# shuwang127/SRCNN_Cpp

Measured on AMD Instinct MI355X. Metric: SRCNN Y-channel Mpixels/sec, higher is better.
Workload: dtype f32; 1 GPU; 1 x 3840x2160 luma plane per GPU per step (1920x1080 x2.0, BASELINE configs[1]), fused conv path, mfma arithmetic, inputs resident in HBM; frames_per_gpu=1, width=3840, height=2160, mode=mfma, seam_deferral=True, output_checksum=584152

## Files before the change

### include/srcnn_amd.h

```cpp
#ifndef SRCNN_AMD_H
#define SRCNN_AMD_H

#include <stddef.h>
#include <stdint.h>

#ifdef __cplusplus
extern "C" {
#endif

#define SRCNN_CONV1_FILTERS 64
#define SRCNN_CONV2_FILTERS 32

enum {
    SRCNN_OK = 0,
    SRCNN_ERR_INVALID = -1,
    SRCNN_ERR_HIP = -2,
    SRCNN_ERR_NOMEM = -3,
    SRCNN_ERR_NODEVICE = -4,
    SRCNN_ERR_STATE = -5
};

enum { SRCNN_MODE_MFMA = 0, SRCNN_MODE_EXACT = 1, SRCNN_MODE_SPLIT16 = 2, SRCNN_MODE_REFBYTES = 3, SRCNN_MODE_REFBYTES16 = 4,
       SRCNN_MODE_BANDED16 = 5 };

// ... 142 lines not shown
enum { SRCNN_METRIC_SSE = 1, SRCNN_METRIC_SSIM = 2 };
int srcnn_metrics_image_dev(srcnn_ctx *ctx, const srcnn_image *a, const srcnn_image *b, int width, int height, int channels,
                            int n_frames, int border, const float *luma , double data_range, int flags,
                            double *d_out );
double srcnn_metric_psnr(double sse, double n_px, double data_range);

int srcnn_forward_y(srcnn_ctx *ctx, const uint8_t *src, size_t src_stride,
                    uint8_t *dst, size_t dst_stride, int width, int height,
                    float *preclamp, size_t preclamp_stride);

int srcnn_forward_y_frames(srcnn_ctx *ctx, const uint8_t *const *src, size_t src_stride,
                           uint8_t *const *dst, size_t dst_stride, int width, int height, int n_frames);


int srcnn_stripe_rows(int height, int n_parts, int index, int *row_begin, int *row_end);

int srcnn_forward_y_frames_multi(srcnn_ctx *const *ctxs, int n_ctx,
                                 const uint8_t *const *src, size_t src_stride,
                                 uint8_t *const *dst, size_t dst_stride,
                                 int width, int height, int n_frames);

int srcnn_forward_y_lanes_dev(srcnn_ctx *const *ctxs, int n_ctx,
                              const uint8_t *const *d_src, size_t src_stride,
                              uint8_t *const *d_dst, size_t dst_stride,
                              int width, int height, int n_planes);

int srcnn_forward_y_striped(srcnn_ctx *const *ctxs, int n_ctx,
                            const uint8_t *src, size_t src_stride,
                            uint8_t *dst, size_t dst_stride, int width, int height);

int srcnn_forward_y_striped_frames(srcnn_ctx *const *ctxs, int n_ctx,
                                   const uint8_t *const *src, size_t src_stride,
                                   uint8_t *const *dst, size_t dst_stride,
                                   int width, int height, int n_planes);

int srcnn_forward_y_striped_dev(srcnn_ctx *const *ctxs, int n_ctx,
                                const uint8_t *const *d_stripes, size_t stripe_stride,
                                uint8_t *const *d_out, size_t out_stride, int width, int height);

int srcnn_halo_transport(const srcnn_ctx *ctx);


int srcnn_forward_y_dev(srcnn_ctx *ctx,
                        const uint8_t *d_src, size_t src_stride, size_t src_frame_pitch,
                        uint8_t *d_dst, size_t dst_stride, size_t dst_frame_pitch,
                        int width, int height, int n_frames,
                        float *d_preclamp );

int srcnn_forward_y_rows_dev(srcnn_ctx *ctx,
                             const uint8_t *d_src, size_t src_stride, int src_row0,
                             uint8_t *d_dst, size_t dst_stride, int dst_row0,
                             int width, int height, int row_begin, int row_end);

int srcnn_forward_y_rows_halo_dev(srcnn_ctx *ctx,
                                  const uint8_t *d_src, size_t src_stride, int src_row0, int src_rows,
                                  const uint8_t *d_halo_top, const uint8_t *d_halo_bot, size_t halo_stride,
                                  uint8_t *d_dst, size_t dst_stride, int dst_row0,
                                  int width, int height, int row_begin, int row_end);


int srcnn_model_halo_rows(const srcnn_ctx *ctx);

int srcnn_model_rows_dev(srcnn_ctx *ctx,
                         const uint8_t *d_src, size_t src_stride, int src_row0,
                         uint8_t *d_dst, size_t dst_stride, int dst_row0,
                         int width, int height, int row_begin, int row_end,
                         float *d_preclamp );

int srcnn_model_rows_halo_dev(srcnn_ctx *ctx,
                              const uint8_t *d_src, size_t src_stride, int src_row0, int src_rows,
                              const uint8_t *d_halo_top, const uint8_t *d_halo_bot, size_t halo_stride,
                              uint8_t *d_dst, size_t dst_stride, int dst_row0,
                              int width, int height, int row_begin, int row_end,
                              float *d_preclamp );

int srcnn_model_striped_dev(srcnn_ctx *const *ctxs, int n_ctx,
                            const uint8_t *const *d_stripes, size_t stripe_stride,
                            uint8_t *const *d_out, size_t out_stride, int width, int height);

int srcnn_model_striped(srcnn_ctx *const *ctxs, int n_ctx,
                        const uint8_t *src, size_t src_stride,
                        uint8_t *dst, size_t dst_stride, int width, int height);

int srcnn_model_color_rows_dev(srcnn_ctx *ctx,
                               const uint8_t *d_src, size_t src_stride, int src_row0,
                               uint8_t *d_dst, size_t dst_stride, int dst_row0,
                               int width, int height, int row_begin, int row_end,
                               float *d_preclamp );
int srcnn_model_color_rows_halo_dev(srcnn_ctx *ctx,
                                    const uint8_t *d_src, size_t src_stride, int src_row0, int src_rows,
                                    const uint8_t *d_halo_top, const uint8_t *d_halo_bot, size_t halo_stride,
                                    uint8_t *d_dst, size_t dst_stride, int dst_row0,
                                    int width, int height, int row_begin, int row_end,
                                    float *d_preclamp );
int srcnn_model_color_striped_dev(srcnn_ctx *const *ctxs, int n_ctx,
                                  const uint8_t *const *d_stripes, size_t stripe_stride,
                                  uint8_t *const *d_out, size_t out_stride, int width, int height);
int srcnn_model_color_striped(srcnn_ctx *const *ctxs, int n_ctx,
                              const uint8_t *src, size_t src_stride,
                              uint8_t *dst, size_t dst_stride, int width, int height);

int srcnn_model_rows_f32_dev(srcnn_ctx *ctx,
                             const float *d_src, size_t src_stride, size_t src_ch_pitch, int src_row0,
                             float *d_dst, size_t dst_stride, size_t dst_ch_pitch, int dst_row0,
                             int width, int height, int row_begin, int row_end);
int srcnn_model_rows_halo_f32_dev(srcnn_ctx *ctx,
                                  const float *d_src, size_t src_stride, size_t src_ch_pitch, int src_row0, int src_rows,
                                  const float *d_halo_top, const float *d_halo_bot, size_t halo_stride, size_t halo_ch_pitch,
                                  float *d_dst, size_t dst_stride, size_t dst_ch_pitch, int dst_row0,
                                  int width, int height, int row_begin, int row_end);
int srcnn_model_striped_f32_dev(srcnn_ctx *const *ctxs, int n_ctx,
                                const float *const *d_stripes, size_t stripe_stride, size_t stripe_ch_pitch,
                                float *const *d_out, size_t out_stride, size_t out_ch_pitch, int width, int height);
int srcnn_model_striped_f32(srcnn_ctx *const *ctxs, int n_ctx,
                            const float *src, size_t src_stride, size_t src_ch_pitch,
                            float *dst, size_t dst_stride, size_t dst_ch_pitch, int width, int height);

int srcnn_forward_y_unfused_dev(srcnn_ctx *ctx,
                                const uint8_t *d_src, size_t src_stride, size_t src_frame_pitch,
                                uint8_t *d_dst, size_t dst_stride, size_t dst_frame_pitch,
                                int width, int height, int n_frames, float *d_work);

int srcnn_conv99x11_dev(srcnn_ctx *ctx, const uint8_t *d_src, size_t src_stride,
                        float *d_planes, size_t plane_stride, size_t plane_pitch,
                        int width, int height);
int srcnn_conv55_dev(srcnn_ctx *ctx, const float *d_planes, size_t plane_stride, size_t plane_pitch,
                     uint8_t *d_dst, size_t dst_stride, int width, int height,
                     float *d_preclamp );


int srcnn_scaled_size(int width, int height, float scale, int *out_w, int *out_h);

int srcnn_bgr2ycrcb(srcnn_ctx *ctx, const uint8_t *bgr, size_t stride, int width, int height,
                    uint8_t *y, uint8_t *cr, uint8_t *cb, size_t plane_stride);
int srcnn_ycrcb2bgr(srcnn_ctx *ctx, const uint8_t *y, const uint8_t *cr, const uint8_t *cb,
                    size_t plane_stride, int width, int height, uint8_t *bgr, size_t stride);
int srcnn_resize_cubic(srcnn_ctx *ctx, const uint8_t *src, size_t src_stride, int src_w, int src_h,
                       uint8_t *dst, size_t dst_stride, int dst_w, int dst_h);

int srcnn_process_bgr(srcnn_ctx *ctx, const uint8_t *bgr, size_t stride, int width, int height,
                      float scale, uint8_t *out, size_t out_stride);
int srcnn_process_bgr_dev(srcnn_ctx *ctx, const uint8_t *d_bgr, size_t stride, int width, int height,
                          float scale, uint8_t *d_out, size_t out_stride);


int srcnn_fixup_stats(srcnn_ctx *ctx, unsigned long long out[4], float *delta, float *max_dev);
int srcnn_set_fixup_strict(srcnn_ctx *ctx, int on);
int srcnn_set_fixup_margin(srcnn_ctx *ctx, float factor);
int srcnn_set_fixup_local(srcnn_ctx *ctx, float k_local);
int srcnn_fixup_local_stats(srcnn_ctx *ctx, float *k, float *max_ratio);

int srcnn_query_plan(srcnn_ctx *ctx, int width, int height, int n_frames, int out[6]);

#ifdef __cplusplus
}
#endif
#endif
```

### srcnn_cpp_amd/__init__.py

```python
from __future__ import annotations

import ctypes as C
from pathlib import Path
from typing import Optional, Sequence

import numpy as np

__all__ = [
    "Context", "SrcnnError", "forward_y_striped_frames", "load_library", "library_path", "tuning_library_path", "use_library", "load_weights", "split_weights",
    "load_model", "split_model", "model_from_state_dict", "model_from_module", "MODEL_SIZES", "COLOR_MODEL_SIZES", "PAD_REPLICATE",
    "PAD_ZERO",
    "Convolution99", "Convolution11", "Convolution55", "Convolution99x11", "default_context",
    "MODE_MFMA", "MODE_EXACT", "MODE_SPLIT16", "MODE_REFBYTES", "MODE_REFBYTES16", "MODE_BANDED16", "FLOP_PER_PIXEL",
    "ERR_INVALID", "ERR_HIP", "ERR_NOMEM", "ERR_NODEVICE", "ERR_STATE",
    "stripe_rows", "forward_y_frames_multi", "forward_y_lanes_dev", "forward_y_striped", "forward_y_striped_dev",
    "model_striped", "model_striped_dev",
    "model_color_striped", "model_color_striped_dev", "model_striped_f32", "model_striped_f32_dev",
    "cubic_f32_taps", "cubic_aa_f32_taps", "luma_gain", "luma_for_order", "luma_bt601_studio", "LUMA_BT601",
    "ELEM_F32", "ELEM_F16", "ELEM_BF16", "ELEM_U8", "ELEM_SIZE", "Image", "image_check",
]

_PKG = Path(__file__).resolve().parent
_LIB_PATH = _PKG / "libsrcnn_amd.so"
_WEIGHTS_PATH = _PKG / "data" / "srcnn915_weights.f32"

MODE_MFMA = 0
MODE_EXACT = 1
MODE_SPLIT16 = 2
MODE_REFBYTES = 3
MODE_REFBYTES16 = 4
MODE_BANDED16 = 5
N_WEIGHTS = 8129
MODEL_SIZES = {8129: 1, 24513: 3, 57281: 5}
COLOR_MODEL_SIZES = {20099: 1, 36483: 3, 69251: 5}
PAD_REPLICATE = 0
PAD_ZERO = 1
_PADDINGS = {"replicate": PAD_REPLICATE, "zero": PAD_ZERO}
FLOP_PER_PIXEL = 16064
LUMA_BT601 = (0.299, 0.587, 0.114, 0.0)

ELEM_F32, ELEM_F16, ELEM_BF16, ELEM_U8 = 0, 1, 2, 3
ELEM_SIZE = {ELEM_F32: 4, ELEM_F16: 2, ELEM_BF16: 2, ELEM_U8: 1}
METRIC_SSE, METRIC_SSIM = 1, 2
METRIC_FIELDS = ("sse", "n_px", "ssim_sum", "n_win")

ERR_INVALID, ERR_HIP, ERR_NOMEM, ERR_NODEVICE, ERR_STATE = -1, -2, -3, -4, -5
_ERR = {-1: "invalid argument", -2: "HIP runtime error", -3: "out of memory",
        -4: "no gfx950 device", -5: "bad state"}

_u8p = C.POINTER(C.c_uint8)
_f32p = C.POINTER(C.c_float)
_f32pp = C.POINTER(_f32p)
_lib = None


class _CImage(C.Structure):
    _fields_ = [("data", C.c_void_p), ("elem", C.c_int), ("scale", C.c_float), ("px_step", C.c_size_t), ("stride", C.c_size_t),
                ("ch_pitch", C.c_size_t), ("frame_pitch", C.c_size_t)]


class SrcnnError(RuntimeError):
    def __init__(self, code: int, msg: str = ""):
        self.code = code
        super().__init__(f"srcnn error {code} ({_ERR.get(code, '?')}): {msg}")


def library_path() -> Path:
    return _LIB_PATH


def tuning_library_path() -> Path:
    return _PKG / "libsrcnn_amd_tuning.so"


def use_library(path) -> None:
    global _LIB_PATH
    if _lib is not None:
        raise RuntimeError("the library is already loaded")
    _LIB_PATH = Path(path)


def load_library() -> C.CDLL:
    global _lib
    if _lib is not None:
        return _lib
    if not _LIB_PATH.exists():
        raise SrcnnError(-4, f"{_LIB_PATH} not built: run `python -m srcnn_cpp_amd.build` "
                             "(there is no CPU fallback)")
    import importlib.util
    import sys
    if "torch" not in sys.modules and importlib.util.find_spec("torch") is not None:
        import torch
    lib = C.CDLL(str(_LIB_PATH))
    sz, i, vp, imp = C.c_size_t, C.c_int, C.c_void_p, C.POINTER(_CImage)
    sigs = {
        "srcnn_abi_version": ([], i),
        "srcnn_create": ([C.POINTER(vp), i], i),
        "srcnn_destroy": ([vp], None),
        "srcnn_last_error": ([vp], C.c_char_p),
        "srcnn_set_mode": ([vp, i], i),
        "srcnn_get_mode": ([vp], i),
        "srcnn_set_stream": ([vp, vp], i),
        "srcnn_synchronize": ([vp], i),
        "srcnn_kernel_variant": ([vp], i),
        "srcnn_conv99": ([vp, _u8p, sz, _f32p, sz, i, i, _f32p, C.c_float], i),
        "srcnn_conv11": ([vp, _f32pp, sz, _f32p, sz, i, i, _f32p, C.c_float], i),
        "srcnn_conv55": ([vp, _f32pp, sz, _u8p, sz, i, i, _f32p, C.c_float], i),
        "srcnn_conv99x11": ([vp, _u8p, sz, _f32pp, sz, i, i, _f32p, _f32p, _f32p, _f32p], i),
        "srcnn_set_weights": ([vp, _f32p, _f32p, _f32p, _f32p, _f32p, C.c_float], i),
        "srcnn_set_model": ([vp, i, _f32p, _f32p, _f32p, _f32p, _f32p, C.c_float], i),
        "srcnn_get_model_f2": ([vp], i),
        "srcnn_set_padding": ([vp, i], i),
        "srcnn_get_padding": ([vp], i),
        "srcnn_set_model_color": ([vp, i, _f32p, _f32p, _f32p, _f32p, _f32p, _f32p], i),
        "srcnn_get_model_channels": ([vp], i),
        "srcnn_forward_color": ([vp, _u8p, sz, _u8p, sz, i, i, _f32p, sz], i),
        "srcnn_forward_color_dev": ([vp, vp, sz, sz, vp, sz, sz, i, i, i, vp], i),
        "srcnn_forward_f32": ([vp, _f32p, sz, sz, _f32p, sz, sz, i, i], i),
        "srcnn_forward_f32_dev": ([vp, vp, sz, sz, sz, vp, sz, sz, sz, i, i, i], i),
        "srcnn_cubic_f32_taps": ([i, i, C.POINTER(i), _f32p], i),
        "srcnn_resize_cubic_f32": ([vp, _f32p, sz, sz, i, i, _f32p, sz, sz, i, i, i], i),
        "srcnn_resize_cubic_f32_dev": ([vp, vp, sz, sz, sz, i, i, vp, sz, sz, sz, i, i, i, i], i),
        "srcnn_cubic_aa_f32_taps": ([i, i, C.POINTER(i), C.POINTER(i), _f32p, i], i),
        "srcnn_resize_cubic_aa_f32": ([vp, _f32p, sz, sz, i, i, _f32p, sz, sz, i, i, i], i),
        "srcnn_resize_cubic_aa_f32_dev": ([vp, vp, sz, sz, sz, i, i, vp, sz, sz, sz, i, i, i, i], i),
        "srcnn_resize_cubic_aa_image_dev": ([vp, imp, i, i, imp, i, i, i, i], i),
        "srcnn_metrics_image_dev": ([vp, imp, imp, i, i, i, i, i, _f32p, C.c_double, i, vp], i),
        "srcnn_metric_psnr": ([C.c_double, C.c_double, C.c_double], C.c_double),
        "srcnn_process_f32": ([vp, _f32p, sz, sz, i, i, _f32p, sz, sz, i, i], i),
        "srcnn_process_f32_dev": ([vp, vp, sz, sz, sz, i, i, vp, sz, sz, sz, i, i, i], i),
        "srcnn_luma_gain": ([_f32p, _f32p], i),
        "srcnn_process_rgb_f32": ([vp, _f32p, sz, sz, i, i, _f32p, sz, sz, i, i, _f32p, _f32p], i),
        "srcnn_process_rgb_f32_dev": ([vp, vp, sz, sz, sz, i, i, vp, sz, sz, sz, i, i, _f32p, _f32p, i], i),
        "srcnn_image_check": ([imp, i, i, i, i, i], i),
        "srcnn_forward_image_dev": ([vp, imp, imp, i, i, i], i),
        "srcnn_resize_cubic_image_dev": ([vp, imp, i, i, imp, i, i, i, i], i),
        "srcnn_process_image_dev": ([vp, imp, i, i, imp, i, i, i], i),
        "srcnn_process_rgb_image_dev": ([vp, imp, i, i, imp, i, i, _f32p, _f32p, i], i),
        "srcnn_set_input_range": ([vp, C.c_float], i),
        "srcnn_get_input_range": ([vp], C.c_float),
        "srcnn_forward_y": ([vp, _u8p, sz, _u8p, sz, i, i, _f32p, sz], i),
        "srcnn_forward_y_frames": ([vp, C.POINTER(_u8p), sz, C.POINTER(_u8p), sz, i, i, i], i),
        "srcnn_forward_y_dev": ([vp, vp, sz, sz, vp, sz, sz, i, i, i, vp], i),
        "srcnn_forward_y_rows_dev": ([vp, vp, sz, i, vp, sz, i, i, i, i, i], i),
        "srcnn_forward_y_rows_halo_dev": ([vp, vp, sz, i, i, vp, vp, sz, vp, sz, i, i, i, i, i], i),
        "srcnn_halo_transport": ([vp], i),
        "srcnn_forward_y_unfused_dev": ([vp, vp, sz, sz, vp, sz, sz, i, i, i, vp], i),
        "srcnn_conv99x11_dev": ([vp, vp, sz, vp, sz, sz, i, i], i),
        "srcnn_conv55_dev": ([vp, vp, sz, sz, vp, sz, i, i, vp], i),
        "srcnn_conv99x11_to_dev": ([vp, _u8p, sz, vp, sz, sz, i, i, _f32p, _f32p, _f32p, _f32p], i),
        "srcnn_conv55_from_dev": ([vp, vp, sz, sz, _u8p, sz, i, i, _f32p, C.c_float], i),
        "srcnn_dev_alloc": ([vp, sz, C.POINTER(vp)], i),
        "srcnn_dev_free": ([vp, vp], i),
        "srcnn_dev_download": ([vp, vp, vp, sz], i),
        "srcnn_dev_upload": ([vp, vp, vp, sz], i),
        "srcnn_ipc_export": ([vp, vp, C.POINTER(C.c_ubyte * 64)], i),
        "srcnn_ipc_open": ([vp, C.POINTER(C.c_ubyte * 64), C.POINTER(vp)], i),
        "srcnn_ipc_close": ([vp, vp], i),
        "srcnn_query_plan": ([vp, i, i, i, C.POINTER(i * 6)], i),
        "srcnn_fixup_stats": ([vp, C.POINTER(C.c_ulonglong * 4), C.POINTER(C.c_float), C.POINTER(C.c_float)], i),
        "srcnn_set_fixup_strict": ([vp, i], i),
        "srcnn_set_seam_deferral": ([vp, i], i),
        "srcnn_flush": ([vp], i),
        "srcnn_set_fixup_margin": ([vp, C.c_float], i),
        "srcnn_set_kernel_variant": ([vp, i], i),
        "srcnn_set_fixup_local": ([vp, C.c_float], i),
        "srcnn_fixup_local_stats": ([vp, C.POINTER(C.c_float), C.POINTER(C.c_float)], i),
        "srcnn_scaled_size": ([i, i, C.c_float, C.POINTER(i), C.POINTER(i)], i),
        "srcnn_bgr2ycrcb": ([vp, _u8p, sz, i, i, _u8p, _u8p, _u8p, sz], i),
        "srcnn_ycrcb2bgr": ([vp, _u8p, _u8p, _u8p, sz, i, i, _u8p, sz], i),
        "srcnn_resize_cubic": ([vp, _u8p, sz, i, i, _u8p, sz, i, i], i),
        "srcnn_process_bgr": ([vp, _u8p, sz, i, i, C.c_float, _u8p, sz], i),
        "srcnn_process_bgr_dev": ([vp, vp, sz, i, i, C.c_float, vp, sz], i),
        "srcnn_stripe_rows": ([i, i, i, C.POINTER(i), C.POINTER(i)], i),
        "srcnn_forward_y_frames_multi": ([C.POINTER(vp), i, C.POINTER(_u8p), sz, C.POINTER(_u8p), sz, i, i, i], i),
        "srcnn_forward_y_lanes_dev": ([C.POINTER(vp), i, C.POINTER(vp), sz, C.POINTER(vp), sz, i, i, i], i),
        "srcnn_forward_y_striped": ([C.POINTER(vp), i, _u8p, sz, _u8p, sz, i, i], i),
        "srcnn_forward_y_striped_frames": ([C.POINTER(vp), i, C.POINTER(_u8p), sz, C.POINTER(_u8p), sz, i, i, i], i),
        "srcnn_forward_y_striped_dev": ([C.POINTER(vp), i, C.POINTER(vp), sz, C.POINTER(vp), sz, i, i], i),
        "srcnn_model_halo_rows": ([vp], i),
        "srcnn_model_rows_dev": ([vp, vp, sz, i, vp, sz, i, i, i, i, i, vp], i),
        "srcnn_model_rows_halo_dev": ([vp, vp, sz, i, i, vp, vp, sz, vp, sz, i, i, i, i, i, vp], i),
        "srcnn_model_striped": ([C.POINTER(vp), i, _u8p, sz, _u8p, sz, i, i], i),
        "srcnn_model_striped_dev": ([C.POINTER(vp), i, C.POINTER(vp), sz, C.POINTER(vp), sz, i, i], i),
        "srcnn_model_color_rows_dev": ([vp, vp, sz, i, vp, sz, i, i, i, i, i, vp], i),
        "srcnn_model_color_rows_halo_dev": ([vp, vp, sz, i, i, vp, vp, sz, vp, sz, i, i, i, i, i, vp], i),
        "srcnn_model_color_striped": ([C.POINTER(vp), i, _u8p, sz, _u8p, sz, i, i], i),
        "srcnn_model_color_striped_dev": ([C.POINTER(vp), i, C.POINTER(vp), sz, C.POINTER(vp), sz, i, i], i),
        "srcnn_model_rows_f32_dev": ([vp, vp, sz, sz, i, vp, sz, sz, i, i, i, i, i], i),
        "srcnn_model_rows_halo_f32_dev": ([vp, vp, sz, sz, i, i, vp, vp, sz, sz, vp, sz, sz, i, i, i, i, i], i),
        "srcnn_model_striped_f32": ([C.POINTER(vp), i, _f32p, sz, sz, _f32p, sz, sz, i, i], i),
        "srcnn_model_striped_f32_dev": ([C.POINTER(vp), i, C.POINTER(vp), sz, sz, C.POINTER(vp), sz, sz, i, i], i),
    }
    for name, (args, res) in sigs.items():
        fn = getattr(lib, name)
        fn.argtypes = args
        fn.restype = res
    _lib = lib
    return lib


ABI_SYMBOLS = (
    "srcnn_abi_version", "srcnn_create", "srcnn_destroy", "srcnn_last_error", "srcnn_set_mode",
    "srcnn_get_mode", "srcnn_set_stream", "srcnn_synchronize", "srcnn_kernel_variant", "srcnn_set_kernel_variant", "srcnn_conv99", "srcnn_conv11",
    "srcnn_conv55", "srcnn_conv99x11", "srcnn_set_weights", "srcnn_forward_y", "srcnn_forward_y_frames",
    "srcnn_forward_y_dev",
    "srcnn_forward_y_rows_dev", "srcnn_forward_y_rows_halo_dev", "srcnn_halo_transport", "srcnn_forward_y_unfused_dev", "srcnn_conv99x11_dev",
    "srcnn_conv55_dev", "srcnn_conv99x11_to_dev", "srcnn_conv55_from_dev", "srcnn_dev_alloc", "srcnn_dev_free",
    "srcnn_dev_download", "srcnn_dev_upload", "srcnn_ipc_export", "srcnn_ipc_open", "srcnn_ipc_close", "srcnn_query_plan", "srcnn_fixup_stats", "srcnn_set_fixup_strict", "srcnn_set_fixup_margin", "srcnn_set_fixup_local", "srcnn_fixup_local_stats", "srcnn_set_seam_deferral", "srcnn_flush", "srcnn_scaled_size", "srcnn_bgr2ycrcb", "srcnn_ycrcb2bgr",
    "srcnn_resize_cubic", "srcnn_process_bgr", "srcnn_process_bgr_dev",
    "srcnn_stripe_rows", "srcnn_forward_y_frames_multi", "srcnn_forward_y_lanes_dev", "srcnn_forward_y_striped", "srcnn_forward_y_striped_frames", "srcnn_forward_y_striped_dev",
    "srcnn_set_model", "srcnn_get_model_f2", "srcnn_set_padding", "srcnn_get_padding",
    "srcnn_set_model_color", "srcnn_get_model_channels", "srcnn_forward_color", "srcnn_forward_color_dev",
    "srcnn_forward_f32", "srcnn_forward_f32_dev", "srcnn_set_input_range", "srcnn_get_input_range",
    "srcnn_cubic_f32_taps", "srcnn_resize_cubic_f32", "srcnn_resize_cubic_f32_dev", "srcnn_process_f32", "srcnn_process_f32_dev",
    "srcnn_luma_gain", "srcnn_process_rgb_f32", "srcnn_process_rgb_f32_dev",
    "srcnn_image_check", "srcnn_forward_image_dev", "srcnn_resize_cubic_image_dev", "srcnn_process_image_dev",
    "srcnn_process_rgb_image_dev",
    "srcnn_cubic_aa_f32_taps", "srcnn_resize_cubic_aa_f32", "srcnn_resize_cubic_aa_f32_dev", "srcnn_resize_cubic_aa_image_dev",
    "srcnn_metrics_image_dev", "srcnn_metric_psnr",
    "srcnn_model_halo_rows", "srcnn_model_rows_dev", "srcnn_model_rows_halo_dev", "srcnn_model_striped", "srcnn_model_striped_dev",
    "srcnn_model_color_rows_dev", "srcnn_model_color_rows_halo_dev", "srcnn_model_color_striped", "srcnn_model_color_striped_dev",
    "srcnn_model_rows_f32_dev", "srcnn_model_rows_halo_f32_dev", "srcnn_model_striped_f32", "srcnn_model_striped_f32_dev",
)


def load_weights(path: Optional[Path] = None) -> np.ndarray:
    blob = np.fromfile(str(path or _WEIGHTS_PATH), dtype="<f4")
    if blob.size != N_WEIGHTS:
        raise ValueError(f"weight blob has {blob.size} floats, expected {N_WEIGHTS}")
    return blob


def split_weights(blob: np.ndarray):
    blob = np.ascontiguousarray(blob, dtype=np.float32)
    return (blob[64:5248].reshape(64, 9, 9), blob[0:64], blob[5280:7328].reshape(32, 64),
            blob[5248:5280], blob[7329:8129].reshape(32, 5, 5), float(blob[7328]))


def split_model(blob: np.ndarray):
    blob = np.ascontiguousarray(blob, dtype=np.float32).ravel()
    if blob.size in COLOR_MODEL_SIZES:
        f2 = COLOR_MODEL_SIZES[blob.size]
        o2 = 64 + 15552
        o3 = o2 + 32 + 2048 * f2 * f2
        return (blob[64:o2].reshape(64, 3, 9, 9), blob[0:64], blob[o2 + 32:o3].reshape(32, 64, f2, f2),
                blob[o2:o2 + 32], blob[o3 + 3:o3 + 2403].reshape(3, 32, 5, 5), blob[o3:o3 + 3].copy())
    f2 = MODEL_SIZES.get(blob.size)
    if f2 is None:
        raise ValueError(f"model blob has {blob.size} floats, expected one of {sorted(MODEL_SIZES)} "
                         f"(colour: {sorted(COLOR_MODEL_SIZES)})")
    if f2 == 1:
        return split_weights(blob)
    n2 = 2048 * f2 * f2
    o3 = 5280 + n2
    return (blob[64:5248].reshape(64, 9, 9), blob[0:64], blob[5280:o3].reshape(32, 64, f2, f2),
            blob[5248:5280], blob[o3 + 1:o3 + 801].reshape(32, 5, 5), float(blob[o3]))


def load_model(path) -> np.ndarray:
    blob = np.fromfile(str(path), dtype="<f4")
    if blob.size not in MODEL_SIZES and blob.size not in COLOR_MODEL_SIZES:
        raise ValueError(f"model blob has {blob.size} floats, expected one of {sorted(MODEL_SIZES)} "
                         f"(colour: {sorted(COLOR_MODEL_SIZES)})")
    return blob


def model_from_state_dict(sd, input_scale: float = 255.0, image_order: Optional[str] = None):
    def arr(key, shape=None):
        if key not in sd:
            raise KeyError(f"state dict has no {key!r}")
        v = sd[key]
        v = v.detach().cpu().numpy() if hasattr(v, "detach") else np.asarray(v)
        v = np.asarray(v, dtype=np.float64)
        if shape is not None and v.shape != shape:
            raise ValueError(f"{key}: shape {v.shape}, expected {shape}")
        return v
    w2 = arr("conv2.weight")
    if w2.ndim != 4 or w2.shape[:2] != (32, 64) or w2.shape[2] != w2.shape[3] or w2.shape[2] not in (1, 3, 5):
        raise ValueError(f"conv2.weight: shape {w2.shape}, expected (32, 64, f2, f2) with f2 in 1, 3, 5")
    s = float(input_scale)
    f32 = lambda a: np.ascontiguousarray(a, dtype=np.float32)
    c_in, c_out = arr("conv1.weight").shape[1:2], arr("conv3.weight").shape[:1]
    if c_in == (3,) or c_out == (3,):
        if c_in != c_out:
            raise ValueError(f"conv1 reads {c_in[0] if c_in else '?'} channels and conv3 writes {c_out[0] if c_out else '?'}: "
                             "a model has 1 channel in and out, or 3")
        if image_order not in ("rgb", "bgr"):
            raise ValueError(f"image_order={image_order!r}: a 3-channel model needs image_order='rgb' or 'bgr' (the channel "
                             "order of the images it will run on)")
        w1, w3, b3 = arr("conv1.weight", (64, 3, 9, 9)), arr("conv3.weight", (3, 32, 5, 5)), arr("conv3.bias", (3,))
        if image_order == "bgr":
            w1, w3, b3 = w1[:, ::-1], w3[::-1], b3[::-1]
        return (f32(w1), f32(arr("conv1.bias", (64,)) * s), f32(w2.reshape(32, 64, w2.shape[2], w2.shape[2])),
                f32(arr("conv2.bias", (32,)) * s), f32(w3), f32(b3 * s))
    return (f32(arr("conv1.weight", (64, 1, 9, 9)).reshape(64, 9, 9)), f32(arr("conv1.bias", (64,)) * s),
            f32(w2 if w2.shape[2] > 1 else w2.reshape(32, 64)), f32(arr("conv2.bias", (32,)) * s),
            f32(arr("conv3.weight", (1, 32, 5, 5)).reshape(32, 5, 5)), float(arr("conv3.bias", (1,))[0] * s))


def model_from_module(module, input_scale: float = 255.0, image_order: Optional[str] = None):
    modes = set()
    for name in ("conv1", "conv2", "conv3"):
        conv = getattr(module, name, None)
        if conv is None:
            raise ValueError(f"module has no {name}")
        k = tuple(conv.kernel_size)
        pad = conv.padding
        if isinstance(pad, str):
            if pad == "valid":
                raise ValueError(f"{name}: padding='valid' (unpadded layers are not supported)")
            pad = tuple(kk // 2 for kk in k)
        pad = tuple(pad) if isinstance(pad, (tuple, list)) else (pad, pad)
        if pad != tuple(kk // 2 for kk in k):
            raise ValueError(f"{name}: padding {pad} for kernel {k}, expected {tuple(kk // 2 for kk in k)}"
                             + (" (unpadded layers are not supported)" if pad == (0, 0) else ""))
        mode = conv.padding_mode
        if mode == "zeros":
            modes.add("zero")
        elif mode == "replicate":
            modes.add("replicate")
        else:
            raise ValueError(f"{name}: padding_mode={mode!r} (only 'zeros' and 'replicate' are supported)")
    if len(modes) != 1:
        raise ValueError(f"the layers mix padding modes {sorted(modes)}: one mode for all three layers is supported")
    return model_from_state_dict(module.state_dict(), input_scale, image_order), modes.pop()


def _plane(a, dtype, name, writable=False):
    if not isinstance(a, np.ndarray) or a.ndim != 2 or a.dtype != dtype:
        raise TypeError(f"{name}: expected a 2-D numpy array of {np.dtype(dtype).name}")
    if a.strides[1] != a.itemsize or a.strides[0] % a.itemsize or a.strides[0] < a.shape[1] * a.itemsize:
        raise ValueError(f"{name}: rows must be contiguous (row stride may be padded)")
    if writable and not a.flags.writeable:
        raise ValueError(f"{name}: output plane is read-only")
    return a, a.strides[0] // a.itemsize


def _f32_planes(a, name, writable=False):
    if not isinstance(a, np.ndarray) or a.dtype != np.float32 or a.ndim not in (2, 3, 4):
        raise TypeError(f"{name}: expected a float32 numpy array of shape (H, W), (C, H, W) or (N, C, H, W)")
    if 0 in a.shape:
        raise ValueError(f"{name}: empty array of shape {tuple(a.shape)}")
    a4 = a[(None,) * (4 - a.ndim)]
    w = a4.shape[3]
    if a4.strides[3] != 4 or (a4.shape[2] > 1 and (a4.strides[2] % 4 or a4.strides[2] < 4 * w)):
        raise ValueError(f"{name}: rows must be contiguous (row, channel and frame strides may be padded)")
    if any(a4.shape[d] > 1 and (a4.strides[d] % 4 or a4.strides[d] <= 0) for d in (0, 1)):
        raise ValueError(f"{name}: channel and frame strides must be positive multiples of 4 bytes")
    if writable and not a.flags.writeable:
        raise ValueError(f"{name}: output array is read-only")
    return a4


def _f32_image(a, name, dst_w, dst_h):
    if not isinstance(a, np.ndarray) or a.dtype != np.float32 or a.ndim not in (2, 3):
        raise TypeError(f"{name}: expected a float32 numpy array of shape (H, W) or (C, H, W)")
    a3 = _f32_planes(a, name)[0]
    for what, v in (("dst_w", dst_w), ("dst_h", dst_h)):
        if isinstance(v, bool) or not isinstance(v, (int, np.integer)) or v <= 0:
            raise ValueError(f"{what}: expected a positive integer, got {v!r}")
    return a3, int(dst_w), int(dst_h)
# ... 139 lines not shown
        self._check(self._lib.srcnn_forward_color(self._h, img.ctypes.data_as(_u8p), ss, dst.ctypes.data_as(_u8p), ds, w, h,
                                                  pp, ps))
        return dst

    def forward_color_dev(self, d_src, src_stride, src_frame_pitch, d_dst, dst_stride, dst_frame_pitch,
                          width, height, n_frames=1, d_preclamp=0):
        self._check(self._lib.srcnn_forward_color_dev(self._h, d_src, src_stride, src_frame_pitch, d_dst, dst_stride,
                                                      dst_frame_pitch, width, height, n_frames, d_preclamp or None))

    def forward_f32(self, x, out=None):
        x4 = _f32_planes(x, "x")
        if out is None:
            out = np.empty(x.shape, np.float32)
        o4 = _f32_planes(out, "out", True)
        _same_shape("out", out.shape, x.shape)
        n, c, h, w = x4.shape
        if c not in (1, 3):
            raise ValueError(f"x: shape {tuple(x.shape)}: a model has 1 channel or 3")
        channels = self.model_channels()
        if c != channels:
            raise ValueError(f"x: shape {tuple(x.shape)} for a model of {channels} channel(s): expected (N, {channels}, H, W), "
                             f"({channels}, H, W)" + (" or (H, W)" if channels == 1 else ""))
        stride = lambda a4: a4.strides[2] // 4 if h > 1 else w
        for k in range(n):
            self._check(self._lib.srcnn_forward_f32(self._h, _fp(x4[k]), stride(x4), x4.strides[1] // 4 if c > 1 else 0, _fp(o4[k]),
                                                    stride(o4), o4.strides[1] // 4 if c > 1 else 0, w, h))
        return out

    def forward_f32_dev(self, d_src, src_stride, src_ch_pitch, src_frame_pitch, d_dst, dst_stride, dst_ch_pitch,
                        dst_frame_pitch, width, height, n_frames=1):
        self._check(self._lib.srcnn_forward_f32_dev(self._h, d_src, src_stride, src_ch_pitch, src_frame_pitch, d_dst, dst_stride,
                                                    dst_ch_pitch, dst_frame_pitch, width, height, n_frames))

    def resize_cubic_f32(self, x, dst_w, dst_h):
        x3, dst_w, dst_h = _f32_image(x, "x", dst_w, dst_h)
        c, h, w = x3.shape
        out = np.empty((c, dst_h, dst_w), np.float32)
        self._check(self._lib.srcnn_resize_cubic_f32(self._h, _fp(x3), x3.strides[1] // 4 if h > 1 else w,
                                                     x3.strides[0] // 4 if c > 1 else 0, w, h, _fp(out), dst_w, dst_w * dst_h,
                                                     dst_w, dst_h, c))
        return out if x.ndim == 3 else out[0]

    def resize_cubic_f32_dev(self, d_src, src_stride, src_ch_pitch, src_frame_pitch, src_w, src_h, d_dst, dst_stride,
                             dst_ch_pitch, dst_frame_pitch, dst_w, dst_h, channels=1, n_frames=1):
        self._check(self._lib.srcnn_resize_cubic_f32_dev(self._h, d_src, src_stride, src_ch_pitch, src_frame_pitch, src_w, src_h,
                                                         d_dst, dst_stride, dst_ch_pitch, dst_frame_pitch, dst_w, dst_h, channels,
                                                         n_frames))

    def resize_cubic_aa_f32(self, x, dst_w, dst_h):
        x3, dst_w, dst_h = _f32_image(x, "x", dst_w, dst_h)
        c, h, w = x3.shape
        out = np.empty((c, dst_h, dst_w), np.float32)
        self._check(self._lib.srcnn_resize_cubic_aa_f32(self._h, _fp(x3), x3.strides[1] // 4 if h > 1 else w,
                                                        x3.strides[0] // 4 if c > 1 else 0, w, h, _fp(out), dst_w, dst_w * dst_h,
                                                        dst_w, dst_h, c))
        return out if x.ndim == 3 else out[0]

    def resize_cubic_aa_f32_dev(self, d_src, src_stride, src_ch_pitch, src_frame_pitch, src_w, src_h, d_dst, dst_stride,
                                dst_ch_pitch, dst_frame_pitch, dst_w, dst_h, channels=1, n_frames=1):
        self._check(self._lib.srcnn_resize_cubic_aa_f32_dev(self._h, d_src, src_stride, src_ch_pitch, src_frame_pitch, src_w, src_h,
                                                            d_dst, dst_stride, dst_ch_pitch, dst_frame_pitch, dst_w, dst_h, channels,
                                                            n_frames))

    def process_f32(self, x, dst_w, dst_h):
        x3, dst_w, dst_h = _f32_image(x, "x", dst_w, dst_h)
        c, h, w = x3.shape
        channels = self.model_channels()
        if c != channels:
            raise ValueError(f"x: shape {tuple(x.shape)} for a model of {channels} channel(s): expected ({channels}, H, W)"
                             + (" or (H, W)" if channels == 1 else ""))
        out = np.empty((c, dst_h, dst_w), np.float32)
        self._check(self._lib.srcnn_process_f32(self._h, _fp(x3), x3.strides[1] // 4 if h > 1 else w,
                                                x3.strides[0] // 4 if c > 1 else 0, w, h, _fp(out), dst_w, dst_w * dst_h, dst_w,
                                                dst_h))
        return out if x.ndim == 3 else out[0]

    def process_f32_dev(self, d_src, src_stride, src_ch_pitch, src_frame_pitch, src_w, src_h, d_dst, dst_stride, dst_ch_pitch,
                        dst_frame_pitch, dst_w, dst_h, n_frames=1):
        self._check(self._lib.srcnn_process_f32_dev(self._h, d_src, src_stride, src_ch_pitch, src_frame_pitch, src_w, src_h, d_dst,
                                                    dst_stride, dst_ch_pitch, dst_frame_pitch, dst_w, dst_h, n_frames))

    def process_rgb_f32(self, x, dst_w, dst_h, luma=LUMA_BT601, clamp=None):
        x3, dst_w, dst_h = _f32_image(x, "x", dst_w, dst_h)
        if x.ndim != 3 or x3.shape[0] != 3:
            raise ValueError(f"x: shape {tuple(x.shape)}: expected (3, H, W)")
        _, h, w = x3.shape
        _not_shrinking(w, h, dst_w, dst_h)
        luma4, clamp2 = _luma4(luma), _clamp2(clamp)
        out = np.empty((3, dst_h, dst_w), np.float32)
        self._check(self._lib.srcnn_process_rgb_f32(self._h, _fp(x3), x3.strides[1] // 4 if h > 1 else w, x3.strides[0] // 4, w, h,
                                                    _fp(out), dst_w, dst_w * dst_h, dst_w, dst_h, luma4, clamp2))
        return out

    def process_rgb_f32_dev(self, d_src, src_stride, src_ch_pitch, src_frame_pitch, src_w, src_h, d_dst, dst_stride, dst_ch_pitch,
                            dst_frame_pitch, dst_w, dst_h, luma=LUMA_BT601, clamp=None, n_frames=1):
        _not_shrinking(src_w, src_h, dst_w, dst_h)
        luma4, clamp2 = _luma4(luma), _clamp2(clamp)
        self._check(self._lib.srcnn_process_rgb_f32_dev(self._h, d_src, src_stride, src_ch_pitch, src_frame_pitch, src_w, src_h, d_dst,
                                                        dst_stride, dst_ch_pitch, dst_frame_pitch, dst_w, dst_h, luma4, clamp2,
                                                        n_frames))

    def forward_image_dev(self, src: "Image", dst: "Image", width, height, n_frames=1):
        self._check(self._lib.srcnn_forward_image_dev(self._h, C.byref(src.c()), C.byref(dst.c()), width, height, n_frames))

    def resize_cubic_image_dev(self, src: "Image", src_w, src_h, dst: "Image", dst_w, dst_h, channels, n_frames=1):
        self._check(self._lib.srcnn_resize_cubic_image_dev(self._h, C.byref(src.c()), src_w, src_h, C.byref(dst.c()), dst_w, dst_h,
                                                           channels, n_frames))

    def resize_cubic_aa_image_dev(self, src: "Image", src_w, src_h, dst: "Image", dst_w, dst_h, channels, n_frames=1):
        self._check(self._lib.srcnn_resize_cubic_aa_image_dev(self._h, C.byref(src.c()), src_w, src_h, C.byref(dst.c()), dst_w,
                                                              dst_h, channels, n_frames))

    def metrics_image_dev(self, a: "Image", b: "Image", width, height, channels, n_frames, border, luma, data_range, flags, d_out):
        luma4, ca, cb = _metric_luma4(luma), a.c(), b.c()
        self._check(self._lib.srcnn_metrics_image_dev(self._h, C.byref(ca), C.byref(cb), int(width), int(height), int(channels),
                                                      int(n_frames), int(border), luma4, float(data_range), int(flags), d_out))

    def process_image_dev(self, src: "Image", src_w, src_h, dst: "Image", dst_w, dst_h, n_frames=1):
        self._check(self._lib.srcnn_process_image_dev(self._h, C.byref(src.c()), src_w, src_h, C.byref(dst.c()), dst_w, dst_h,
                                                      n_frames))

    def process_rgb_image_dev(self, src: "Image", src_w, src_h, dst: "Image", dst_w, dst_h, luma=LUMA_BT601, clamp=None, n_frames=1):
        _not_shrinking(src_w, src_h, dst_w, dst_h)
        luma4, clamp2 = _luma4(luma), _clamp2(clamp)
        self._check(self._lib.srcnn_process_rgb_image_dev(self._h, C.byref(src.c()), src_w, src_h, C.byref(dst.c()), dst_w, dst_h,
                                                          luma4, clamp2, n_frames))

    def set_input_range(self, r: float):
        self._check(self._lib.srcnn_set_input_range(self._h, float(r)))

    def input_range(self) -> float:
        return float(self._lib.srcnn_get_input_range(self._h))

    def model_f2(self) -> int:
        return int(self._lib.srcnn_get_model_f2(self._h))

    def set_padding(self, padding):
        if isinstance(padding, str):
            if padding not in _PADDINGS:
                raise ValueError(f"padding {padding!r}: expected 'zero' or 'replicate'")
            padding = _PADDINGS[padding]
        self._check(self._lib.srcnn_set_padding(self._h, int(padding)))

    def padding(self) -> str:
        v = int(self._lib.srcnn_get_padding(self._h))
        return {PAD_REPLICATE: "replicate", PAD_ZERO: "zero"}[v]

    def query_plan(self, width, height, n_frames=1):
        out = (C.c_int * 6)()
        self._check(self._lib.srcnn_query_plan(self._h, width, height, n_frames, C.byref(out)))
        return dict(workgroups=out[0], seg_rows=out[1], strips=out[2], segments=out[3],
                    lds_bytes=out[4], threads=out[5])

    def conv99(self, src, dst, kernel, bias):
        src, ss = _plane(src, np.uint8, "src")
        dst, ds = _plane(dst, np.float32, "dst", True)
        k = _wt(kernel, 81, "kernel")
        h, w = dst.shape
        _same_shape("src", src.shape, dst.shape)
        self._check(self._lib.srcnn_conv99(self._h, src.ctypes.data_as(_u8p), ss, _fp(dst), ds, w, h,
                                           _fp(k), float(bias)))

    def conv11(self, src, dst, kernel, bias):
        arr, ss, shape = _ptr_array(src, 64, "src")
        dst, ds = _plane(dst, np.float32, "dst", True)
        k = _wt(kernel, 64, "kernel")
        h, w = dst.shape
        _same_shape("src planes", shape, dst.shape)
        self._check(self._lib.srcnn_conv11(self._h, arr, ss, _fp(dst), ds, w, h, _fp(k), float(bias)))

    def conv55(self, src, dst, kernel, bias):
        arr, ss, shape = _ptr_array(src, 32, "src")
        dst, ds = _plane(dst, np.uint8, "dst", True)
        k = _wt(kernel, 800, "kernel")
        h, w = dst.shape
        _same_shape("src planes", shape, dst.shape)
        self._check(self._lib.srcnn_conv55(self._h, arr, ss, dst.ctypes.data_as(_u8p), ds, w, h,
                                           _fp(k), float(bias)))

    def conv99x11(self, src, dst, k99, b99, k11, b11):
        src, ss = _plane(src, np.uint8, "src")
        arr, ds, shape = _ptr_array(dst, 32, "dst", True)
        k99, b99 = _wt(k99, 5184, "kernel99"), _wt(b99, 64, "bias99")
        k11, b11 = _wt(k11, 2048, "kernel11"), _wt(b11, 32, "bias11")
        h, w = src.shape
        _same_shape("dst planes", shape, src.shape)
        self._check(self._lib.srcnn_conv99x11(self._h, src.ctypes.data_as(_u8p), ss, arr, ds, w, h,
                                              _fp(k99), _fp(b99), _fp(k11), _fp(b11)))

    def fixup_stats(self):
        out, delta, dev = (C.c_ulonglong * 4)(), C.c_float(), C.c_float()
        self._check(self._lib.srcnn_fixup_stats(self._h, C.byref(out), C.byref(delta), C.byref(dev)))
        return {"scattered_pixels": int(out[0]), "dense_tiles": int(out[1]), "bytes_changed": int(out[2]),
                "exact_reruns": int(out[3]), "delta": float(delta.value), "max_dev": float(dev.value)}

    def set_fixup_strict(self, on: bool = True):
        self._check(self._lib.srcnn_set_fixup_strict(self._h, int(bool(on))))

    def set_seam_deferral(self, on: bool = True):
        self._check(self._lib.srcnn_set_seam_deferral(self._h, int(bool(on))))

    def flush(self):
        self._check(self._lib.srcnn_flush(self._h))

    def set_fixup_margin(self, factor: float):
        self._check(self._lib.srcnn_set_fixup_margin(self._h, float(factor)))

    def set_fixup_local(self, k_local: float):
        self._check(self._lib.srcnn_set_fixup_local(self._h, float(k_local)))

    def fixup_local_stats(self):
        k, r = C.c_float(), C.c_float()
        self._check(self._lib.srcnn_fixup_local_stats(self._h, C.byref(k), C.byref(r)))
        return float(k.value), float(r.value)

    def dev_alloc(self, nbytes: int) -> int:
        p = C.c_void_p()
        self._check(self._lib.srcnn_dev_alloc(self._h, nbytes, C.byref(p)))
        return p.value

    def dev_free(self, d_ptr: int):
        self._check(self._lib.srcnn_dev_free(self._h, d_ptr))

    def dev_download(self, dst: np.ndarray, d_src: int):
        if not (isinstance(dst, np.ndarray) and dst.flags.c_contiguous and dst.flags.writeable):
            raise ValueError("dst: expected a writeable C-contiguous numpy array")
        self._check(self._lib.srcnn_dev_download(self._h, dst.ctypes.data_as(C.c_void_p), d_src, dst.nbytes))
        return dst

    def dev_upload(self, d_dst: int, src: np.ndarray):
        src = np.ascontiguousarray(src)
        self._check(self._lib.srcnn_dev_upload(self._h, d_dst, src.ctypes.data_as(C.c_void_p), src.nbytes))

    def ipc_export(self, d_ptr: int) -> bytes:
        h = (C.c_ubyte * 64)()
        self._check(self._lib.srcnn_ipc_export(self._h, d_ptr, C.byref(h)))
        return bytes(h)

    def ipc_open(self, handle: bytes) -> int:
        if len(handle) != 64:
            raise ValueError("an IPC handle is 64 bytes")
        h = (C.c_ubyte * 64).from_buffer_copy(handle)
        p = C.c_void_p()
        self._check(self._lib.srcnn_ipc_open(self._h, C.byref(h), C.byref(p)))
        return p.value

    def ipc_close(self, d_ptr: int):
        self._check(self._lib.srcnn_ipc_close(self._h, d_ptr))

    def conv99x11_to_dev(self, src, d_planes, plane_stride, plane_pitch, k99, b99, k11, b11):
        src, ss = _plane(src, np.uint8, "src")
        k99, b99 = _wt(k99, 5184, "kernel99"), _wt(b99, 64, "bias99")
        k11, b11 = _wt(k11, 2048, "kernel11"), _wt(b11, 32, "bias11")
        h, w = src.shape
        self._check(self._lib.srcnn_conv99x11_to_dev(self._h, src.ctypes.data_as(_u8p), ss, d_planes, plane_stride, plane_pitch,
                                                     w, h, _fp(k99), _fp(b99), _fp(k11), _fp(b11)))

    def conv55_from_dev(self, d_planes, plane_stride, plane_pitch, dst, kernel, bias):
        dst, ds = _plane(dst, np.uint8, "dst", True)
        k = _wt(kernel, 800, "kernel")
        h, w = dst.shape
        self._check(self._lib.srcnn_conv55_from_dev(self._h, d_planes, plane_stride, plane_pitch, dst.ctypes.data_as(_u8p), ds,
                                                    w, h, _fp(k), float(bias)))

    def forward_y(self, src, dst=None, preclamp=None):
        src, ss = _plane(src, np.uint8, "src")
        h, w = src.shape
        if dst is None:
            dst = np.empty((h, w), np.uint8)
        dst, ds = _plane(dst, np.uint8, "dst", True)
        _same_shape("dst", dst.shape, src.shape)
        pp, ps = None, 0
        if preclamp is not None:
            preclamp, ps = _plane(preclamp, np.float32, "preclamp", True)
            _same_shape("preclamp", preclamp.shape, src.shape)
            pp = _fp(preclamp)
        self._check(self._lib.srcnn_forward_y(self._h, src.ctypes.data_as(_u8p), ss,
                                              dst.ctypes.data_as(_u8p), ds, w, h, pp, ps))
        return dst

    def forward_y_frames(self, frames, out=None):
        frames = np.ascontiguousarray(frames, dtype=np.uint8)
        if frames.ndim != 3 or 0 in frames.shape:
            raise ValueError("frames: expected a non-empty [n, h, w] uint8 array")
        n, h, w = frames.shape
        if out is None:
            out = np.empty_like(frames)
        if not isinstance(out, np.ndarray) or out.dtype != np.uint8:
            raise TypeError("out: expected a uint8 numpy array")
        _same_shape("out", out.shape, frames.shape)
        if not out.flags.c_contiguous or not out.flags.writeable:
            raise ValueError("out: must be C-contiguous and writeable")
        srcs = (_u8p * n)(*[frames[k].ctypes.data_as(_u8p) for k in range(n)])
        dsts = (_u8p * n)(*[out[k].ctypes.data_as(_u8p) for k in range(n)])
        self._check(self._lib.srcnn_forward_y_frames(self._h, srcs, w, dsts, w, w, h, n))
        return out

    def forward_y_dev(self, d_src, src_stride, src_frame_pitch, d_dst, dst_stride, dst_frame_pitch,
                      width, height, n_frames=1, d_preclamp=0):
        self._check(self._lib.srcnn_forward_y_dev(self._h, d_src, src_stride, src_frame_pitch, d_dst,
                                                  dst_stride, dst_frame_pitch, width, height, n_frames,
                                                  d_preclamp or None))

    def forward_y_rows_dev(self, d_src, src_stride, src_row0, d_dst, dst_stride, dst_row0,
                           width, height, row_begin, row_end):
        self._check(self._lib.srcnn_forward_y_rows_dev(self._h, d_src, src_stride, src_row0, d_dst,
# ... 478 lines not shown
```

### srcnn_cpp_amd/csrc/srcnn_api.cpp

```cpp
#include "srcnn_ctx.h"

using namespace srcnn;
using namespace srcnn::host;

namespace srcnn {
namespace host {

int fail(srcnn_ctx *c, int code, const char *fmt, ...)
{
    if (c) {
        va_list ap;
        va_start(ap, fmt);
        vsnprintf(c->err, sizeof(c->err), fmt, ap);
        va_end(ap);
    }
    return code;
}

int reserve(srcnn_ctx *c, DevBuf &b, size_t bytes)
{
    if (bytes <= b.cap) return SRCNN_OK;
    if (b.p) {
        if (int rc = flush_seams(c)) return rc;
        HIP_TRY(c, hipDeviceSynchronize());
        HIP_TRY(c, hipFree(b.p));
        b.p = nullptr;
        b.cap = 0;
    }
    HIP_TRY(c, hipMalloc(&b.p, bytes));
    b.cap = bytes;
    return SRCNN_OK;
}

void release(DevBuf &b)
{
    if (b.p) (void)hipFree(b.p);
    b.p = nullptr;
    b.cap = 0;
}

}
}

static long probe_verdict(int device, int n_devices, hipStream_t stream)
{
    static std::mutex probe_mutex;
    static std::vector<long> probe_result;
    std::lock_guard<std::mutex> lk(probe_mutex);
    if ((int)probe_result.size() < n_devices) probe_result.resize((size_t)n_devices, -2);
    if (device < 0 || device >= (int)probe_result.size()) return -1;
    if (probe_result[(size_t)device] == -2) probe_result[(size_t)device] = srcnn::interlock_probe_mismatches(device, stream);
    return probe_result[(size_t)device];
}

extern "C" {

int srcnn_abi_version(void) { return 1; }

int srcnn_create(srcnn_ctx **out, int device)
{
    if (!out) return SRCNN_ERR_INVALID;
    *out = nullptr;
    int n = 0;
    if (hipGetDeviceCount(&n) != hipSuccess || n <= 0 || device < 0 || device >= n) return SRCNN_ERR_NODEVICE;
    hipDeviceProp_t prop;
    if (hipGetDeviceProperties(&prop, device) != hipSuccess) return SRCNN_ERR_NODEVICE;
    if (std::strncmp(prop.gcnArchName, "gfx950", 6) != 0) return SRCNN_ERR_NODEVICE;
    srcnn_ctx *c = new (std::nothrow) srcnn_ctx();
    if (!c) return SRCNN_ERR_NOMEM;
    c->device = device;
    c->n_cu = prop.multiProcessorCount > 0 ? prop.multiProcessorCount : 256;
    DeviceScope dev_scope_(c);
    if (dev_scope_.rc != SRCNN_OK || hipStreamCreateWithFlags(&c->own_stream, hipStreamNonBlocking) != hipSuccess) {
        delete c;
        return SRCNN_ERR_HIP;
    }
    c->stream = c->own_stream;
    long bad = probe_verdict(device, n, c->own_stream);
    const char *force = SRCNN_DEBUG_ENV("SRCNN_DEBUG_FORCE_SAFE");
    if (force && std::atoi(force)) bad = 1;
    if (bad != 0) {
        c->safe_hazards = true;
        (void)fail(c, SRCNN_OK, "the MFMA interlock probe %s on device %d: this context launches the hazard-safe strip kernels",
                   bad < 0 ? "could not run" : "found differing results", device);
    }
    *out = c;
    return SRCNN_OK;
}

int srcnn_kernel_variant(const srcnn_ctx *c) { return c ? (c->safe_hazards ? 1 : 0) : SRCNN_ERR_INVALID; }

int srcnn_set_kernel_variant(srcnn_ctx *c, int variant)
{
    BIND(c);
    if (variant != 0 && variant != 1) return fail(c, SRCNN_ERR_INVALID, "set_kernel_variant: 0 (what the interlock probe allows) or 1 (hazard-safe)");
    if (variant == 1) {
        c->safe_hazards = true;
        return SRCNN_OK;
    }
    int n = 0;
    HIP_TRY(c, hipGetDeviceCount(&n));
    c->safe_hazards = probe_verdict(c->device, n, c->own_stream) != 0;
    return SRCNN_OK;
}

void srcnn_destroy(srcnn_ctx *c)
{
    if (!c) return;
    c->pool.reset();
    DeviceScope dev_scope_(c);
    (void)flush_seams(c);
    (void)hipStreamSynchronize(c->stream);
    (void)hipDeviceSynchronize();
    for (DevBuf *b : {&c->wfrag, &c->wraw, &c->in_u8, &c->out_u8, &c->pre_f32, &c->planes, &c->plane1, &c->kern, &c->sink,
                      &c->bgr_in, &c->bgr_out, &c->ycc_lo, &c->ycc_hi, &c->y_sr, &c->tables, &c->wfrag16,
                      &c->band_top, &c->band_bot, &c->stripe_ext, &c->sp_table, &c->sp16_table, &c->sp_map64, &c->sp_map32,
                      &c->f32_tables, &c->f32_lo, &c->f32_hi, &c->f32_work, &c->aa_tables, &c->aa_work, &c->metric_work})
        release(*b);
    if (c->sp_done) (void)hipEventDestroy(c->sp_done);
    for (int k = 0; k < srcnn_ctx::kHaloSets; ++k) {
        release(c->halo_top[k]);
        release(c->halo_bot[k]);
        if (c->halo_free[k]) (void)hipEventDestroy(c->halo_free[k]);
    }
    for (int k = 0; k < 2; ++k)
        if (c->pin_plane[k]) (void)hipHostFree(c->pin_plane[k]);
    if (c->halo_ready) (void)hipEventDestroy(c->halo_ready);
    if (c->bands_done) (void)hipEventDestroy(c->bands_done);
    if (c->halo_stream) (void)hipStreamDestroy(c->halo_stream);
    for (auto &sc : c->seam_scratch) {
        release(sc.buf);
        release(sc.cbuf);
        release(sc.buf2);
        release(sc.cbuf2);
        release(sc.flag);
        release(sc.fix_lists);
        release(sc.fix_counters);
    }
    release(c->fix_totals);
    for (auto &t : c->item_tables) {
        release(t.dev);
        release(t.dev_seams);
        release(t.dev_winmap);
    }
    for (int k = 0; k < 2; ++k) {
        for (hipEvent_t e : {c->sf_up[k], c->sf_k[k], c->sf_down[k]})
            if (e) (void)hipEventDestroy(e);
        release(c->lane_in[k]);
        release(c->lane_out[k]);
        if (c->pin_in[k]) (void)hipHostFree(c->pin_in[k]);
        if (c->pin_out[k]) (void)hipHostFree(c->pin_out[k]);
        if (c->lane_stream[k]) (void)hipStreamDestroy(c->lane_stream[k]);
    }
    if (c->own_stream) (void)hipStreamDestroy(c->own_stream);
    delete c;
}

const char *srcnn_last_error(const srcnn_ctx *c) { return c ? c->err : "null context"; }

int srcnn_set_mode(srcnn_ctx *c, int mode)
{
    if (!c || (mode != SRCNN_MODE_MFMA && mode != SRCNN_MODE_EXACT && mode != SRCNN_MODE_SPLIT16 && mode != SRCNN_MODE_REFBYTES &&
               mode != SRCNN_MODE_REFBYTES16 && mode != SRCNN_MODE_BANDED16))
        return SRCNN_ERR_INVALID;
    BIND(c);
    c->mode = mode;
    return SRCNN_OK;
}

int srcnn_get_mode(const srcnn_ctx *c) { return c ? c->mode : SRCNN_ERR_INVALID; }

int srcnn_set_stream(srcnn_ctx *c, void *hip_stream)
{
    BIND(c);
    c->stream = hip_stream ? static_cast<hipStream_t>(hip_stream) : c->own_stream;
    return SRCNN_OK;
}

int srcnn_set_seam_deferral(srcnn_ctx *c, int on)
{
    BIND(c);
    c->defer_seams = on != 0;
    return SRCNN_OK;
}

int srcnn_flush(srcnn_ctx *c)
{
    BIND(c);
    return SRCNN_OK;
}

int srcnn_synchronize(srcnn_ctx *c)
{
    BIND(c);
    int rc = SRCNN_OK;
    (void)rc;
    HIP_TRY(c, hipStreamSynchronize(c->stream));
    return SRCNN_OK;
}

int srcnn_fixup_stats(srcnn_ctx *c, unsigned long long out[4], float *delta, float *max_dev)
{
    BIND(c);
    if (!out) return fail(c, SRCNN_ERR_INVALID, "fixup_stats: null output");
    unsigned long long t[FIX_TOTALS] = {0, 0, 0, 0, 0, 0};
    if (c->fix_totals.p) {
        HIP_TRY(c, hipStreamSynchronize(c->stream));
        HIP_TRY(c, hipMemcpy(t, c->fix_totals.p, sizeof(t), hipMemcpyDeviceToHost));
    }
    out[0] = t[FIX_N_SCAT];
    out[1] = t[FIX_N_DENSE];
    out[2] = t[FIX_N_CHANGED];
    out[3] = t[FIX_N_RERUN];
    if (delta) *delta = c->mode == SRCNN_MODE_REFBYTES16 ? c->fix_delta * (8.f / 6.f) : c->fix_delta;
    if (max_dev) {
        const unsigned bits = (unsigned)t[FIX_MAX_DEV];
        std::memcpy(max_dev, &bits, sizeof(float));
    }
    return SRCNN_OK;
}

int srcnn_set_fixup_local(srcnn_ctx *c, float k_local)
{
    BIND(c);
    if (!(k_local >= 0.f && k_local <= 64.f)) return fail(c, SRCNN_ERR_INVALID, "set_fixup_local: the factor must lie in [0, 64]");
    c->fix_local = k_local;
    c->fix_local16 = k_local * (kFixLocal16 / kFixLocal);
    return SRCNN_OK;
}

int srcnn_fixup_local_stats(srcnn_ctx *c, float *k, float *max_ratio)
{
    BIND(c);
    if (k) *k = (c->mode == SRCNN_MODE_REFBYTES16 ? c->fix_local16 : c->fix_local) * c->fix_margin;
    if (max_ratio) {
        unsigned long long t[FIX_TOTALS] = {0, 0, 0, 0, 0, 0};
        if (c->fix_totals.p) {
            HIP_TRY(c, hipStreamSynchronize(c->stream));
            HIP_TRY(c, hipMemcpy(t, c->fix_totals.p, sizeof(t), hipMemcpyDeviceToHost));
        }
        const unsigned bits = (unsigned)t[FIX_MAX_RATIO];
        std::memcpy(max_ratio, &bits, sizeof(float));
    }
    return SRCNN_OK;
}

int srcnn_set_fixup_margin(srcnn_ctx *c, float factor)
{
    BIND(c);
    if (!(factor >= 0.25f && factor <= 64.f)) return fail(c, SRCNN_ERR_INVALID, "set_fixup_margin: factor must lie in [0.25, 64]");
    c->fix_margin = factor;
    if (c->has_l12 || c->has_l3) {
        const float *hr = c->host_raw.data();
        c->fix_delta = fixup_delta(hr + 64, hr, hr + 5280, hr + 5248, hr + 7329, factor);
    }
    return SRCNN_OK;
}

int srcnn_set_fixup_strict(srcnn_ctx *c, int on)
{
    if (!c) return SRCNN_ERR_INVALID;
    c->fix_strict = on != 0;
    return SRCNN_OK;
}

int srcnn_dev_alloc(srcnn_ctx *c, size_t bytes, void **out)
{
    BIND(c);
    if (!out || bytes == 0) return fail(c, SRCNN_ERR_INVALID, "dev_alloc: bad arguments");
    *out = nullptr;
    HIP_TRY(c, hipMalloc(out, bytes));
    return SRCNN_OK;
}

int srcnn_dev_free(srcnn_ctx *c, void *p)
{
    BIND(c);
    if (!p) return SRCNN_OK;
    HIP_TRY(c, hipDeviceSynchronize());
    HIP_TRY(c, hipFree(p));
    return SRCNN_OK;
}

int srcnn_dev_download(srcnn_ctx *c, void *dst, const void *d_src, size_t bytes)
{
    BIND(c);
    if (!dst || !d_src) return fail(c, SRCNN_ERR_INVALID, "dev_download: null pointer");
    HIP_TRY(c, hipStreamSynchronize(c->stream));
    HIP_TRY(c, hipMemcpy(dst, d_src, bytes, hipMemcpyDeviceToHost));
    return SRCNN_OK;
}

int srcnn_dev_upload(srcnn_ctx *c, void *d_dst, const void *src, size_t bytes)
{
    BIND(c);
    if (!d_dst || !src) return fail(c, SRCNN_ERR_INVALID, "dev_upload: null pointer");
    HIP_TRY(c, hipStreamSynchronize(c->stream));
    HIP_TRY(c, hipMemcpy(d_dst, src, bytes, hipMemcpyHostToDevice));
    return SRCNN_OK;
}

int srcnn_ipc_export(srcnn_ctx *c, void *d_ptr, unsigned char handle[64])
{
    BIND(c);
    if (!d_ptr || !handle) return fail(c, SRCNN_ERR_INVALID, "ipc_export: null pointer");
    static_assert(sizeof(hipIpcMemHandle_t) == 64, "the ABI carries the handle as 64 bytes");
    hipIpcMemHandle_t h;
    HIP_TRY(c, hipIpcGetMemHandle(&h, d_ptr));
    std::memcpy(handle, &h, sizeof(h));
    return SRCNN_OK;
}

int srcnn_ipc_open(srcnn_ctx *c, const unsigned char handle[64], void **d_ptr)
{
    BIND(c);
    if (!d_ptr || !handle) return fail(c, SRCNN_ERR_INVALID, "ipc_open: null pointer");
    *d_ptr = nullptr;
    hipIpcMemHandle_t h;
    std::memcpy(&h, handle, sizeof(h));
    HIP_TRY(c, hipIpcOpenMemHandle(d_ptr, h, hipIpcMemLazyEnablePeerAccess));
    return SRCNN_OK;
}

int srcnn_ipc_close(srcnn_ctx *c, void *d_ptr)
{
    BIND(c);
    if (!d_ptr) return SRCNN_OK;
    HIP_TRY(c, hipDeviceSynchronize());
    HIP_TRY(c, hipIpcCloseMemHandle(d_ptr));
    return SRCNN_OK;
}

#ifdef SRCNN_TUNING_BUILD

int srcnn_debug_read_sink(srcnn_ctx *c, void *dst, size_t bytes)
{
    BIND(c);
    int rc = SRCNN_OK;
    (void)rc;
    if (!dst || bytes > c->sink.cap) return SRCNN_ERR_INVALID;
    HIP_TRY(c, hipStreamSynchronize(c->stream));
    HIP_TRY(c, hipMemcpy(dst, c->sink.p, bytes, hipMemcpyDeviceToHost));
    return SRCNN_OK;
}

int srcnn_debug_pack_fragments(const float *blob8129, float *frag , uint8_t *frag16 ,
                               int *frag_floats, int *frag16_bytes)
{
    if (frag_floats) *frag_floats = NFRAG * 64;
    if (frag16_bytes) *frag16_bytes = (int)S16_TABLE_BYTES;
    if (!blob8129) return SRCNN_ERR_INVALID;
    const float *b1 = blob8129, *w1 = blob8129 + 64, *b2 = blob8129 + 5248, *w2 = blob8129 + 5280, *w3 = blob8129 + 7329;
    if (frag) pack_fragments(w1, b1, w2, b2, w3, frag);
    if (frag16) pack_fragments16(w1, b1, w2, b2, w3, frag16);
    return split16_range_ok(w1, b1, w2, b2, w3) ? 1 : 0;
}

int srcnn_debug_worker_pool(int n, int rounds)
{
    if (n < 1 || n > 64 || rounds < 1) return SRCNN_ERR_INVALID;
    WorkerPool pool;
    std::vector<long> hits((size_t)n, 0);
    for (int r = 0; r < rounds; ++r) {
        const int m = 1 + r % n;
        const int fail_at = (r % 7 == 3 && m > 1) ? m - 1 : -1;
        const int rc = pool.run(m, [&](int k) -> int {
            ++hits[(size_t)k];
            return k == fail_at ? -100 - k : 0;
        });
        if (rc != (fail_at >= 0 ? -100 - fail_at : 0)) return -1;
    }
    for (int k = 0; k < n; ++k) {
        long want = 0;
        for (int r = 0; r < rounds; ++r) want += (1 + r % n) > k;
        if (hits[(size_t)k] != want) return -2;
    }
    return pool.size() == n - 1 ? 0 : -3;
}

int srcnn_debug_cubic_table(int n_src, int n_dst, int *ofs, short *coef)
{
    if (n_src <= 0 || n_dst <= 0 || !ofs || !coef) return SRCNN_ERR_INVALID;
    cubic_table(n_src, n_dst, ofs, coef);
    return SRCNN_OK;
}

int srcnn_debug_resize_variant(int sw, int sh, int dw, int dh, int dword_ok)
{
    if (sw <= 0 || sh <= 0 || dw <= 0 || dh <= 0) return SRCNN_ERR_INVALID;
    return resize_variant(sw, sh, dw, dh, dword_ok != 0);
}

int srcnn_debug_resize_f32_variant(int sw, int sh, int dw, int dh)
{
    if (sw <= 0 || sh <= 0 || dw <= 0 || dh <= 0) return SRCNN_ERR_INVALID;
    return resize_f32_variant(sw, sh, dw, dh);
}

int srcnn_debug_resize_f32_limits(int *out4)
{
    if (!out4) return SRCNN_ERR_INVALID;
    const int v[4] = {F32_RT, F32_RMAX, F32_SMAX, 256};
    for (int k = 0; k < 4; ++k) out4[k] = v[k];
    return SRCNN_OK;
}

int srcnn_debug_resize_limits(int *out6)
{
    if (!out6) return SRCNN_ERR_INVALID;
    const int v[6] = {RT, RMAX, RT4, RMAX4, SMAX, 256};
    for (int k = 0; k < 6; ++k) out6[k] = v[k];
    return SRCNN_OK;
}
#endif

}
```

### srcnn_cpp_amd/csrc/srcnn_ctx.h

```cpp
#pragma once
#include "../../include/srcnn_amd.h"
#include "srcnn_kernels.h"

#include <algorithm>
#include <atomic>
#include <cstdarg>
#include <cstdio>
#include <cstdlib>
#include <cmath>
#include <condition_variable>
#include <cstring>
#include <functional>
#include <memory>
#include <mutex>
#include <new>
#include <thread>
#include <vector>

#ifdef SRCNN_TUNING_BUILD
#define SRCNN_DEBUG_ENV(name) std::getenv(name)
#else
#define SRCNN_DEBUG_ENV(name) static_cast<const char *>(nullptr)
#endif

namespace srcnn {
namespace host {

struct DevBuf {
    void *p = nullptr;
    size_t cap = 0;
};

class WorkerPool {
    struct Worker {
        std::thread th;
        std::mutex m;
        std::condition_variable cv;
        std::function<int()> task;
        bool has_task = false, done = false, stop = false;
        int rc = 0;
    };
    std::vector<std::unique_ptr<Worker>> workers_;

    static void loop(Worker *w)
    {
        std::unique_lock<std::mutex> lk(w->m);
        for (;;) {
            w->cv.wait(lk, [w] { return w->has_task || w->stop; });
            if (w->stop) return;
            std::function<int()> t = std::move(w->task);
            w->has_task = false;
            lk.unlock();
            const int rc = t();
            lk.lock();
            w->rc = rc;
            w->done = true;
            w->cv.notify_all();
        }
    }

public:
    WorkerPool() = default;
    WorkerPool(const WorkerPool &) = delete;
    WorkerPool &operator=(const WorkerPool &) = delete;
    ~WorkerPool()
    {
        for (auto &w : workers_) {
            { std::lock_guard<std::mutex> lk(w->m); w->stop = true; }
            w->cv.notify_all();
            if (w->th.joinable()) w->th.join();
        }
    }
    template <typename Fn>
    int run(int n, Fn fn, int nomem = SRCNN_ERR_NOMEM) { return run(n, fn, nomem, [] {}); }
    template <typename Fn, typename Abort>
    int run(int n, Fn fn, int nomem, Abort on_incomplete)
    {
        try {
            while ((int)workers_.size() < n - 1) {
                std::unique_ptr<Worker> w(new Worker());
                w->th = std::thread(loop, w.get());
                workers_.push_back(std::move(w));
            }
        } catch (...) {
            return nomem;
        }
        int posted = 0, first = 0;
        try {
            for (int k = 1; k < n; ++k) {
                Worker *w = workers_[(size_t)k - 1].get();
                { std::lock_guard<std::mutex> lk(w->m); w->task = [&fn, k] { return fn(k); }; w->has_task = true; w->done = false; }
                w->cv.notify_all();
                posted = k;
            }
            first = fn(0);
        } catch (...) {
            first = nomem;
            on_incomplete();
        }
        for (int k = 1; k <= posted; ++k) {
            Worker *w = workers_[(size_t)k - 1].get();
            std::unique_lock<std::mutex> lk(w->m);
            w->cv.wait(lk, [w] { return w->done; });
            if (!first && w->rc) first = w->rc;
        }
        return first;
    }
    int size() const { return (int)workers_.size(); }
};

}
}

constexpr float kFixMargin = 4.f;
constexpr float kFixAbsTerm = 4.f * 256.f / 16777216.f;
constexpr float kFixAbsLocal = 16.f * 256.f / 16777216.f;
constexpr float kFixLocal = 0.4f;
constexpr float kFixLocal16 = 0.5375f;

struct srcnn_ctx {
    int device = 0;
    int n_cu = 256;
    int mode = SRCNN_MODE_MFMA;
    bool safe_hazards = false;
    hipStream_t own_stream = nullptr;
    hipStream_t stream = nullptr;
    char err[512] = "no error";
    bool has_l12 = false, has_l3 = false;
    float b3 = 0.f;
    srcnn::host::DevBuf wfrag;
    srcnn::host::DevBuf wfrag16;
    bool split16_ok = false;
    srcnn::host::DevBuf wraw;
    int channels = 1;
    int f2 = 1;
    srcnn::host::DevBuf sp_table, sp_map64, sp_map32;
    float sp_b3[3] = {0.f, 0.f, 0.f};
    int sp_f2 = 0;
    std::vector<float> sp_w2;
    double sp_l1_bound = 0.0;
    srcnn::host::DevBuf sp16_table;
    int sp16_f2 = 0;
    float sp16_scale1 = 1.f, sp16_unscale = 1.f;
    float input_range = 255.f;
    double sp_l1_sum[64] = {}, sp_l1_absb[64] = {};
    int sp16_e2 = 0;
    hipEvent_t sp_done = nullptr;
    hipStream_t sp_stream = nullptr;
    int padding = SRCNN_PAD_REPLICATE;
    bool whole_model = false;
    bool per_filter = false;
    srcnn::host::DevBuf in_u8, out_u8, pre_f32, planes, plane1, kern, sink;
    struct SeamScratch {
        hipStream_t stream = nullptr;
        bool used = false;
        srcnn::host::DevBuf buf, cbuf;
        srcnn::host::DevBuf buf2, cbuf2;
        int flip = 0;
        srcnn::host::DevBuf flag, fix_lists, fix_counters;
    };
    SeamScratch seam_scratch[4];
    srcnn::host::DevBuf bgr_in, bgr_out, ycc_lo, ycc_hi, y_sr, tables;
    int tab_sw = 0, tab_sh = 0, tab_dw = 0, tab_dh = 0;
    srcnn::host::DevBuf f32_tables, f32_lo, f32_hi, f32_work;
    int ftab_sw = 0, ftab_sh = 0, ftab_dw = 0, ftab_dh = 0;
    hipStream_t ftab_stream = nullptr;
    srcnn::host::DevBuf aa_tables, aa_work;
    int atab_sw = 0, atab_sh = 0, atab_dw = 0, atab_dh = 0, atab_kx = 0, atab_ky = 0;
    hipStream_t aa_stream = nullptr;
    srcnn::host::DevBuf metric_work;
    hipStream_t metric_stream = nullptr;
    struct ItemTable {
        int key[8] = {0, 0, 0, 0, 0, 0, 0, 0};
        int count = 0;
        int n_seams = 0;
        srcnn::host::DevBuf dev, dev_seams;
        srcnn::host::DevBuf dev_winmap;
        bool separated = false;
        unsigned long stamp = 0;
    };
    static constexpr int kItemTables = 32;
    ItemTable item_tables[kItemTables];
    unsigned long item_clock = 0;
    std::vector<float> host_raw = std::vector<float>(8129, 0.f);
    void *pin_plane[2] = {nullptr, nullptr};
    size_t pin_plane_cap = 0;
    hipStream_t halo_stream = nullptr;
    hipEvent_t halo_ready = nullptr, bands_done = nullptr;
    bool bands_pending = false;
    srcnn::host::DevBuf band_top, band_bot, stripe_ext;
    static constexpr int kHaloSets = 4;
    srcnn::host::DevBuf halo_top[kHaloSets], halo_bot[kHaloSets];
    hipEvent_t halo_free[kHaloSets] = {nullptr, nullptr, nullptr, nullptr};
    bool halo_free_set[kHaloSets] = {false, false, false, false};
    unsigned long stripe_steps = 0;
    int halo_transport = 0;
    std::vector<int> peer_state;
    hipEvent_t sf_up[2] = {nullptr, nullptr}, sf_k[2] = {nullptr, nullptr}, sf_down[2] = {nullptr, nullptr};
    std::atomic<int> sf_gen_up{0}, sf_gen_k{0}, sf_abort{0};
    hipStream_t lane_stream[2] = {nullptr, nullptr};
    srcnn::host::DevBuf lane_in[2], lane_out[2];
    void *pin_in[2] = {nullptr, nullptr}, *pin_out[2] = {nullptr, nullptr};
    size_t pin_cap = 0;
    bool defer_seams = false;
    int defer_block = 0;
    struct PendingSeams {
        bool valid = false;
        hipStream_t stream = nullptr;
        srcnn::FoldParams f{};
    } pending;
    float fix_delta = 0.f;
    float fix_margin = kFixMargin;
    float fix_local = kFixLocal;
    float fix_local16 = kFixLocal16;
    bool fix_strict = true;
    srcnn::host::DevBuf fix_totals;
    std::unique_ptr<srcnn::host::WorkerPool> pool;
};

namespace srcnn {
namespace host {

int fail(srcnn_ctx *c, int code, const char *fmt, ...);

#define HIP_TRY(ctx, expr)                                                                      \
    do {                                                                                        \
        hipError_t e_ = (expr);                                                                 \
        if (e_ != hipSuccess)                                                                   \
            return fail((ctx), e_ == hipErrorOutOfMemory ? SRCNN_ERR_NOMEM : SRCNN_ERR_HIP,     \
                        "%s failed: %s", #expr, hipGetErrorString(e_));                         \
    } while (0)

struct DeviceScope {
    int prev = -1, rc = SRCNN_OK;
    explicit DeviceScope(srcnn_ctx *c)
    {
        if (!c) { rc = SRCNN_ERR_INVALID; return; }
        if (hipGetDevice(&prev) != hipSuccess) prev = -1;
        if (prev != c->device) {
            const hipError_t e = hipSetDevice(c->device);
            if (e != hipSuccess) {
                rc = fail(c, SRCNN_ERR_HIP, "hipSetDevice(%d) failed: %s", c->device, hipGetErrorString(e));
                prev = -1;
            }
        } else {
            prev = -1;
        }
    }
    ~DeviceScope() { if (prev >= 0) (void)hipSetDevice(prev); }
    DeviceScope(const DeviceScope &) = delete;
    DeviceScope &operator=(const DeviceScope &) = delete;
};
struct DeferBlock {
    srcnn_ctx *c;
    explicit DeferBlock(srcnn_ctx *ctx) : c(ctx) { ++c->defer_block; }
    ~DeferBlock() { --c->defer_block; }
    DeferBlock(const DeferBlock &) = delete;
    DeferBlock &operator=(const DeferBlock &) = delete;
};
#define BIND_KEEP(c)            \
    DeviceScope dev_scope_(c);  \
    if (dev_scope_.rc) return dev_scope_.rc
#define BIND(c)                                                        \
    BIND_KEEP(c);                                                      \
    if (int flush_rc_ = srcnn::host::flush_seams(c)) return flush_rc_; \
    srcnn::host::DeferBlock defer_block_(c)

int reserve(srcnn_ctx *c, DevBuf &b, size_t bytes);
void release(DevBuf &b);

constexpr int kHaloRows = 6;

float fixup_delta(const float *w1, const float *b1, const float *w2, const float *b2, const float *w3, double margin = kFixMargin);
void pack_fragments(const float *w1, const float *b1, const float *w2, const float *b2, const float *w3, float *out);
void pack_fragments16(const float *w1, const float *b1, const float *w2, const float *b2, const float *w3, uint8_t *out);
void split16(float w, float scale, uint16_t *hi, uint16_t *lo);
double banded16_l1_bound(int C, const float *w1, const float *b1, double range = 255.0);
bool banded16_exponent(double bound, int *e);
bool banded16_pack_w2(int f2, const float *w2, uint16_t *table, int *e2);
bool split16_range_ok(const float *w1, const float *b1, const float *w2, const float *b2, const float *w3);
int upload_weights(srcnn_ctx *c, const float *k99, const float *b99, const float *k11, const float *b11, const float *k55, float b55);
int use_layers12(srcnn_ctx *c, const float *kernel99, const float *bias99, const float *kernel11, const float *bias11);
int use_layer3(srcnn_ctx *c, const float *kernel, float bias);
inline bool has_model(const srcnn_ctx *c) { return c->has_l12 && c->has_l3; }
inline bool luma_path_ok(const srcnn_ctx *c)
{
    return c->channels == 1 && c->f2 == 1 && c->padding != SRCNN_PAD_ZERO && (c->mode != SRCNN_MODE_BANDED16 || c->per_filter);
}
void drop_spatial_model(srcnn_ctx *c);

int refuse_spatial(srcnn_ctx *c, const char *what, bool banded_entry = false);
struct BandedPlanes {
    bool f32 = false;
    const void *src = nullptr;
    size_t src_stride = 0, ch_step = 0, src_frame_pitch = 0;
    int px_step = 1;
    void *dst = nullptr;
    size_t dst_stride = 0, dst_ch_pitch = 0, dst_frame_pitch = 0;
    float *pre = nullptr;
    bool rows = false;
    int row_begin = 0, row_end = 0, src_row0 = 0, src_rows = 0, dst_row0 = 0;
    const void *halo_top = nullptr, *halo_bot = nullptr;
    size_t halo_stride = 0, halo_ch_pitch = 0;
};
int forward_banded(srcnn_ctx *c, const BandedPlanes &io, int width, int height, int n_frames);
int forward_banded(srcnn_ctx *c, const uint8_t *src, size_t src_stride, int px_step, size_t ch_step, size_t src_frame_pitch,
                   uint8_t *dst, size_t dst_stride, size_t dst_frame_pitch, int width, int height, int n_frames, float *pre);
enum StripeKind { STRIPE_Y = 0, STRIPE_COLOR = 1, STRIPE_F32 = 2 };
int model_rows_refusal(srcnn_ctx *c, StripeKind kind = STRIPE_Y);
size_t f32_span(int C, size_t stride, size_t ch_pitch, size_t frame_pitch, int width, int height, int n_frames);
bool f32_planes_disjoint(int C, size_t stride, size_t ch_pitch, size_t frame_pitch, int width, int height, int n_frames);
int forward_f32_refusal(srcnn_ctx *c);
constexpr size_t kSpatialWorkBytes = (size_t)512 << 20;
extern const char *const kNoModel;

struct Plan {
    int seg_rows, n_strips, n_segs;
};
Plan make_plan(const srcnn_ctx *c, int width, int rows, int n_frames, int halo, int wgs_per_cu = 2, int col_halo = -1);
struct ItemPlan {
    std::vector<int> items, seams;
    bool separated = false;
    int count() const { return (int)items.size() / ITEM_INTS; }
    int n_seams() const { return (int)seams.size() / 2; }
};
ItemPlan plan_items(int n_cu, int n_strips, int row_begin, int row_end, int skew_pct, int wgs_per_cu = 2, bool want_seams = false,
                    int extra_top = 0, int extra_bot = 0);
int skew_percent();
int build_items(srcnn_ctx *c, int n_strips, int row_begin, int row_end, int height, int wgs_per_cu, bool want_seams,
                const srcnn_ctx::ItemTable **table);
int split16_wgs_per_cu(bool split16, int tune);
int seam_scratch_for_stream(srcnn_ctx *c, srcnn_ctx::SeamScratch **out);
bool cseam_pays(int width);
constexpr int kItemBatchMax = 32, kItemBatchChunk = 8, kGridBatchChunk = 64;
bool f32_mfma(const srcnn_ctx *c);
int frames_per_launch(const srcnn_ctx *c, int width, int height, int n_frames);

bool ranges_overlap(const void *a, size_t a_bytes, const void *b, size_t b_bytes);
size_t span_elems(size_t stride, size_t frame_pitch, int width, int height, int n_frames);
bool bad_plane(const void *p, size_t stride, int w, int h);
bool bad_pitch(size_t plane_pitch);
int run_strip(srcnn_ctx *c, int mode, StripParams p, int n_frames, int fix_frame = 0, int fix_frames = 1, bool may_defer = false);
int flush_seams(srcnn_ctx *c);

void cubic_f32_taps(int n_src, int n_dst, int *first, float *coef);
struct ResizeTablesF32 {
    const int *xfirst, *yfirst;
    const float *xcoef, *ycoef;
};
int ensure_tables_f32(srcnn_ctx *c, int sw, int sh, int dw, int dh, ResizeTablesF32 *t);
int cubic_aa_f32_taps(int n_src, int n_dst, int *first, int *count, float *coef, int max_taps);

void cubic_table(int n_src, int n_dst, int *ofs, short *coef);
int ensure_lanes(srcnn_ctx *c, size_t bytes);

template <typename T>
void copy_rows_mt(T *dst, size_t dst_stride, const T *src, size_t src_stride, int width, int height)
{
    static const int n_thr = [] {
        const char *e = SRCNN_DEBUG_ENV("SRCNN_HOST_COPY_THREADS");
        const int hw = (int)std::thread::hardware_concurrency();
        return std::max(1, e ? std::atoi(e) : std::min(8, hw > 0 ? hw / 2 : 4));
    }();
    auto part = [=](int y0, int y1) {
        if (dst_stride == (size_t)width && src_stride == (size_t)width)
            std::memcpy(dst + (size_t)y0 * width, src + (size_t)y0 * width, (size_t)(y1 - y0) * width * sizeof(T));
        else
            for (int y = y0; y < y1; ++y) std::memcpy(dst + (size_t)y * dst_stride, src + (size_t)y * src_stride, (size_t)width * sizeof(T));
    };
    const int nt = (int)std::min<size_t>((size_t)n_thr, std::max<size_t>(1, (size_t)width * height * sizeof(T) >> 20));
    if (nt <= 1) { part(0, height); return; }
    std::vector<std::thread> pool;
    for (int t = 1; t < nt; ++t) pool.emplace_back(part, (int)((long)height * t / nt), (int)((long)height * (t + 1) / nt));
    part(0, height / nt);
    for (auto &th : pool) th.join();
}

}
}
```

### srcnn_cpp_amd/csrc/srcnn_kernels.h

```cpp
#pragma once
#include <hip/hip_runtime.h>
#include <stddef.h>
#include <stdint.h>

namespace srcnn {

constexpr int FW = 128;
constexpr int YP = FW + 8;
constexpr int YR = 16;
constexpr int NWAVES = FW / 32;
constexpr int NTHREADS = NWAVES * 64;

enum StripMode { MODE_FUSED = 0, MODE_L12 = 1, MODE_L3 = 2 };

constexpr int NFRAG_L1 = 82;
constexpr int NFRAG_L2 = 32;
constexpr int NFRAG_L3 = 16;
constexpr int NFRAG_B2 = 16;
constexpr int NFRAG_L2U = 32;
constexpr int NFRAG_B2U = 16;
constexpr int NFRAG_L3U = 16;
constexpr int FRAG_L2 = NFRAG_L1, FRAG_L3 = FRAG_L2 + NFRAG_L2, FRAG_B2 = FRAG_L3 + NFRAG_L3,
              FRAG_L2U = FRAG_B2 + NFRAG_B2, FRAG_B2U = FRAG_L2U + NFRAG_L2U, FRAG_L3U = FRAG_B2U + NFRAG_B2U;
constexpr int NFRAG = FRAG_L3U + NFRAG_L3U;

__host__ __device__ constexpr int acc_row(int r, int h) { return (r & 3) + 8 * (r >> 2) + 4 * h; }
__host__ __device__ constexpr int row_chan(int i) { return 2 * ((i & 3) + 4 * (i >> 3)) + ((i >> 2) & 1); }

__host__ __device__ constexpr int l3_row_tap(int i)
{
    const int r = (i & 3) + 4 * (i >> 3), h = (i >> 2) & 1, s = r / 5, m = r % 5, n = h ? 3 + s : s;
    return (r < 15 && n < 5) ? 5 * m + n : -1;
}
__host__ __device__ constexpr bool l3_row_is_scale(int i)
{
    const int r = (i & 3) + 4 * (i >> 3), h = (i >> 2) & 1;
    return h == 1 && r >= 10 && r < 15;
}

constexpr int S16_FRAG_L2 = 24, S16_FRAG_L3 = 32, S16_NFRAG = 36;
constexpr size_t S16_TABLE_BYTES = (size_t)S16_NFRAG * 64 * 16 + 2 * 16 * sizeof(float);
__host__ __device__ constexpr int l1s_tap(int b, int h, int e)
{
    const int n = 4 * b + e / 2, u = e & 1;
    if (n < 20) return (2 * (n % 5) + u < 9) ? 9 * (n / 5 + 5 * h) + 2 * (n % 5) + u : -1;
    if (n < 23) {
        const int jj = 4 * h + 2 * (n - 20) + u;
        return (h == 0 ? jj <= 3 : (jj >= 4 && jj <= 8)) ? 36 + jj : -1;
    }
    return (u == 0 && h == 0) ? 81 : -1;
}

struct StripParams {
    const uint8_t *src;
    long src_stride, src_frame_pitch;
    int src_row0;
    const uint8_t *src_top, *src_bot;
    long halo_stride;
    int src_row1;
    const float *planes_in;
    float *planes_out;
    long pl_stride, pl_pitch, pl_frame_pitch;
    uint8_t *dst;
    float *pre;
    long dst_stride, dst_frame_pitch;
    int dst_row0;
    const float *wfrag;
    const uint32_t *wfrag16;
    float *sink;
    float b3;
    int width, height;
    int row_begin, row_end;
    int seg_rows, n_strips, n_segs;
    const int *items;
    int items_per_frame;
    int seams_per_frame;
    float *seam;
    float *cseam;
    int strips_total;
    int tune;
    uint8_t *flag;
    float fix_delta, fix_scale;
    float fix_kl, fix_abs;
    unsigned *fix_counters;
};

enum { FIX_N_SCAT = 0, FIX_N_DENSE = 1, FIX_N_CHANGED = 2, FIX_MAX_DEV = 3, FIX_N_RERUN = 4,
       FIX_MAX_RATIO = 5,
       FIX_TOTALS = 6,
       FIX_WORD_STRIDE = 64,
       FIX_NEXT_ITEM = 6,
       FIX_NEXT_RERUN = 7,
       FIX_REGIONS = 8, FIX_REGION0 = 8 * FIX_WORD_STRIDE,
       FIX_COUNTERS = FIX_REGION0 + FIX_REGIONS * FIX_WORD_STRIDE };
struct FixParams {
    const uint8_t *src;
    long src_stride;
    int src_row0;
    const uint8_t *src_top, *src_bot;
    long halo_stride;
    int src_row1;
    uint8_t *dst;
    const uint8_t *flag;
    long dst_stride;
    int dst_row0;
    int width, height, row_begin, row_end;
    const float *wraw;
    unsigned *counters;
    unsigned long long *totals;
    unsigned *scat, *dense;
    float delta, code_step;
    float kl, abs_term;
    float rerun_above;
    int n_frames;
    long src_frame_pitch, dst_frame_pitch, flag_frame_pitch;
};
__device__ __forceinline__ float fix_threshold(float s1, float delta, float kl, float abs_term)
{
    return __builtin_fminf(delta, __builtin_fmaf(s1, kl, abs_term));
}
__device__ __forceinline__ uint8_t fix_code(float v, float thr, float delta, float scale)
{
    const float dist = v - __builtin_rintf(v);
    const bool live = (__builtin_fabsf(dist) <= thr) & ((__builtin_bit_cast(unsigned, v) - 0x3f000000u) < (0x437f8000u - 0x3f000000u));
    const unsigned code = (unsigned)((dist + delta) * scale + 1.5f);
    return live ? (uint8_t)code : (uint8_t)0;
}

__device__ __forceinline__ uint8_t fix_src_at(const FixParams &p, int frame, int yy, int xx)
{
    if (p.src_top && yy < p.src_row0) return p.src_top[(long)(yy - (p.src_row0 - 6)) * p.halo_stride + xx];
    if (p.src_bot && yy >= p.src_row1) return p.src_bot[(long)(yy - p.src_row1) * p.halo_stride + xx];
    return p.src[(long)frame * p.src_frame_pitch + (long)(yy - p.src_row0) * p.src_stride + xx];
}

hipError_t launch_fixup(const FixParams &p, int n_cu, bool with_rerun, bool lds_weights, hipStream_t st);
constexpr int FIX_BATCH_FRAMES = 16;
size_t fixup_list_entries(int width, int rows, int n_frames, size_t *dense_entries);

constexpr int ITEM_INTS = 5;
constexpr int SEAM_R = 12, SEAM_ROWS = 4;
__host__ __device__ constexpr int seam_t_off(int r) { return SEAM_R + 3 * (r * 4 - r * (r - 1) / 2); }
constexpr int SEAM_FLOATS = SEAM_R + 3 * (4 + 3 + 2 + 1);

size_t strip_lds_bytes(int mode);
hipError_t launch_seams(const StripParams &p, int n_seams, const int *d_seams, hipStream_t stream);

constexpr int CSEAM_FLOATS = 16;
hipError_t launch_cseams(const StripParams &p, int n_frames, hipStream_t stream);
hipError_t launch_seams_merged(const StripParams &p, int n_seams, const int *d_seams, const unsigned char *d_winmap, int n_frames,
                               hipStream_t stream);
hipError_t launch_strip(int mode, const StripParams &p, int n_frames, hipStream_t stream, size_t lds_pad = 0);
struct FoldParams {
    StripParams prev;
    const int *seams;
    const unsigned char *winmap;
    int n_seams, cblocks, first_block;
};
hipError_t launch_strip_fold(const StripParams &p, const FoldParams &f, hipStream_t stream, size_t lds_pad = 0);
hipError_t launch_strip_safe(int mode, const StripParams &p, int n_frames, hipStream_t stream, size_t lds_pad = 0);
long interlock_probe_mismatches(int device, hipStream_t stream);

size_t split16_lds_bytes();
hipError_t launch_split16(const StripParams &p, int n_frames, hipStream_t stream, size_t lds_pad = 0);

hipError_t launch_conv99_exact(const uint8_t *src, long sstride, float *dst, long dstride,
                               int w, int h, const float *d_kernel81, float bias, hipStream_t st);
hipError_t launch_conv11_exact(const float *planes, long stride, long pitch, float *dst, long dstride,
                               int w, int h, const float *d_kernel64, float bias, hipStream_t st);
hipError_t launch_conv99x11_exact(const uint8_t *src, long sstride, long src_frame_pitch,
                                  float *planes, long stride, long pitch, long frame_pitch,
                                  int w, int h, int n_frames, const float *d_weights, hipStream_t st);
hipError_t launch_conv55_exact(const float *planes, long stride, long pitch, long frame_pitch,
                               uint8_t *dst, float *pre, long dstride, long dst_frame_pitch,
                               int w, int h, int n_frames, const float *d_kernel800, float bias,
                               hipStream_t st);

constexpr int SPATIAL_NFRAG_L1 = 82, SPATIAL_NFRAG_L3 = 16;
__host__ __device__ constexpr size_t spatial_l2_offset(int C) { return (size_t)C * SPATIAL_NFRAG_L1 * 64; }
__host__ __device__ constexpr size_t spatial_l3_offset(int C, int f2) { return spatial_l2_offset(C) + (size_t)f2 * f2 * 2048 + 32; }
__host__ __device__ constexpr size_t spatial_table_floats(int C, int f2) { return spatial_l3_offset(C, f2) + (size_t)C * SPATIAL_NFRAG_L3 * 64; }
size_t spatial_l2_lds_bytes(int f2);
__host__ __device__ constexpr int spatial_l2h_channel(int step, int h, int e) { return 32 * (step >> 1) + acc_row(8 * (step & 1) + e, h); }
__host__ __device__ constexpr size_t spatial_l2h_table_bytes(int f2) { return (size_t)4 * f2 * f2 * 2 * 64 * 16; }
struct L1Input {
    const void *src;
    bool f32;
    int channels;
    long sstride;
    int px_step;
    long ch_step;
    bool rows;
    const void *top, *bot;
    long halo_stride, halo_ch_pitch;
    int src_row0, src_row1, halo_rows;
};
hipError_t launch_spatial_l1(const L1Input &in, bool zero, bool split, float scale, int W, int H, int m0, int m1, const float *frag,
                             void *map, long mpitch, hipStream_t st);
hipError_t launch_spatial_l2(int f2, bool zero, bool split, const void *map, long mpitch, int m0, int m1, int W, int H, int o0, int o1,
                             const void *frag, const float *bias, float unscale, float *out, long opitch, hipStream_t st);
struct L3Output {
    void *dst;
    bool f32;
    long dstride, ch_pitch;
    float *pre;
};
hipError_t launch_spatial_l3(int channels, bool zero, const float *map, long mpitch, int o0, int o1, int W, int H, int b0, int b1,
                             const float *frag, const float *b3, const L3Output &out, hipStream_t st);
hipError_t launch_split3(const uint8_t *src, long sstride, int W, int H, uint8_t *planes, long ppitch, hipStream_t st);

constexpr int RT = 8;
constexpr int RMAX = 16;
constexpr int SMAX = 288;
#ifndef SRCNN_RT4
#define SRCNN_RT4 32
#endif
constexpr int RT4 = SRCNN_RT4;
constexpr int RPT = RT4 / 4;
constexpr int RMAX4 = RT4 == 32 ? 28 : 20;
enum { RESIZE_DIRECT = 0, RESIZE_TILED = 1, RESIZE_TILED4 = 2 };
inline int resize_variant(int sw, int sh, int dw, int dh, bool dword_ok)
{
    const long span = ((long)RT * sh + dh - 1) / dh + 4;
    const long cspan = (256L * sw + dw - 1) / dw + 5;
    const long span4 = ((long)RT4 * sh + dh - 1) / dh + 4;
    if (span4 <= RMAX4 && cspan <= SMAX && dword_ok) return RESIZE_TILED4;
    if (span <= RMAX && cspan <= SMAX) return RESIZE_TILED;
    return RESIZE_DIRECT;
}
constexpr int kMaxGridYZ = 65535;
inline long resize_grid_rows(int variant, int dh)
{
    return variant == RESIZE_TILED4 ? ((long)dh + RT4 - 1) / RT4 : variant == RESIZE_TILED ? ((long)dh + RT - 1) / RT : (long)dh;
}

constexpr int F32_RT = 16;
constexpr int F32_RPT = F32_RT / 4;
constexpr int F32_RMAX = 20;
// ... 39 lines not shown
```

### srcnn_cpp_amd/csrc/srcnn_launch.cpp

```cpp
#include "srcnn_ctx.h"

using namespace srcnn;
using namespace srcnn::host;

namespace srcnn {
namespace host {

bool ranges_overlap(const void *a, size_t a_bytes, const void *b, size_t b_bytes)
{
    const uintptr_t a0 = (uintptr_t)a, b0 = (uintptr_t)b;
    return a0 < b0 + b_bytes && b0 < a0 + a_bytes;
}
size_t span_elems(size_t stride, size_t frame_pitch, int width, int height, int n_frames)
{
    return (size_t)(n_frames - 1) * frame_pitch + (size_t)(height - 1) * stride + (size_t)width;
}

bool bad_plane(const void *p, size_t stride, int w, int h)
{
    return !p || w <= 0 || h <= 0 || stride < (size_t)w || stride >= ((size_t)1 << 30);
}
bool bad_pitch(size_t plane_pitch) { return plane_pitch >= ((size_t)1 << 29); }

int flush_seams(srcnn_ctx *c)
{
    if (!c || !c->pending.valid) return SRCNN_OK;
    c->pending.valid = false;
    const FoldParams &f = c->pending.f;
    if (f.winmap) HIP_TRY(c, launch_seams_merged(f.prev, f.n_seams, f.seams, f.winmap, 1, c->pending.stream));
    else HIP_TRY(c, launch_seams(f.prev, f.n_seams, f.seams, c->pending.stream));
    return SRCNN_OK;
}

static bool fold_is_safe(const StripParams &a, const StripParams &b)
{
    auto span = [](const StripParams &q, const uint8_t **lo, size_t *bytes) {
        *lo = q.dst + (long)(q.row_begin - q.dst_row0) * q.dst_stride;
        *bytes = (size_t)(q.row_end - q.row_begin - 1) * (size_t)q.dst_stride + (size_t)q.width;
    };
    const uint8_t *alo, *blo;
    size_t ab, bb;
    span(a, &alo, &ab);
    span(b, &blo, &bb);
    {
        const int r0 = std::max(0, b.row_begin - kHaloRows), r1 = std::min(b.height, b.row_end + kHaloRows);
        const int s0 = b.src_top ? std::max(r0, b.src_row0) : r0, s1 = b.src_bot ? std::min(r1, b.src_row1) : r1;
        if (s1 > s0 && ranges_overlap(alo, ab, b.src + (long)(s0 - b.src_row0) * b.src_stride,
                                      (size_t)(s1 - s0 - 1) * (size_t)b.src_stride + (size_t)b.width))
            return false;
        const size_t halo_bytes = (size_t)(kHaloRows - 1) * (size_t)b.halo_stride + (size_t)b.width;
        if (b.src_top && ranges_overlap(alo, ab, b.src_top, halo_bytes)) return false;
        if (b.src_bot && ranges_overlap(alo, ab, b.src_bot, halo_bytes)) return false;
    }
    if (!ranges_overlap(alo, ab, blo, bb)) return true;
    return a.dst == b.dst && a.dst_stride == b.dst_stride && a.dst_row0 == b.dst_row0 && a.width == b.width && a.height == b.height &&
           a.row_begin == b.row_begin && a.row_end == b.row_end && a.items == b.items && a.strips_total == b.strips_total;
}

static float r16_kl(const srcnn_ctx *c, float strip_kl) { return c->mode == SRCNN_MODE_REFBYTES16 ? strip_kl * 1024.f : strip_kl; }

int run_strip(srcnn_ctx *c, int mode, StripParams p, int n_frames, int fix_frame, int fix_frames, bool may_defer)
{
    const int halo = (mode == MODE_L12) ? 0 : 2;
    static const char *env_tune = SRCNN_DEBUG_ENV("SRCNN_DEBUG_TUNE");
    static const char *env_pad = SRCNN_DEBUG_ENV("SRCNN_DEBUG_LDS_PAD");
    constexpr int kTuneHarmless = 2 | 8 | 16 | 128;
    p.tune = (env_tune ? std::atoi(env_tune) : 0) & kTuneHarmless;
    const size_t pad = env_pad ? (size_t)std::atol(env_pad) : 0;
    const bool split16 = mode == MODE_FUSED && (c->mode == SRCNN_MODE_SPLIT16 || c->mode == SRCNN_MODE_REFBYTES16);
    const int wgs_per_cu = split16_wgs_per_cu(split16, p.tune);
    Plan pl = make_plan(c, p.width, p.row_end - p.row_begin, n_frames, halo, wgs_per_cu);
    static const char *env_segs = SRCNN_DEBUG_ENV("SRCNN_DEBUG_SEGS");
    if (env_segs && std::atoi(env_segs) > 0) {
        const int rows = p.row_end - p.row_begin, ns = std::min(rows, std::atoi(env_segs));
        pl.seg_rows = (rows + ns - 1) / ns;
        pl.n_segs = (rows + pl.seg_rows - 1) / pl.seg_rows;
    }
    p.seg_rows = pl.seg_rows;
    p.n_strips = pl.n_strips;
    p.n_segs = pl.n_segs;
    p.items = nullptr;
    p.seam = nullptr;
    p.cseam = nullptr;
    p.strips_total = pl.n_strips;
    int grid_items = 0;
    bool defer = false;
    const srcnn_ctx::ItemTable *table = nullptr;
    static const char *env_l3 = SRCNN_DEBUG_ENV("SRCNN_DEBUG_L3");
    const int ns_l3 = (p.width + FW - 1) / FW;
    const bool l3_aligned = mode == MODE_L3 && !(env_l3 && std::atoi(env_l3) == 0) &&
                            (p.width - (ns_l3 - 1) * FW >= 4 || ns_l3 == 1);
    if (l3_aligned) {
        pl = make_plan(c, p.width, p.row_end - p.row_begin, n_frames, halo, 4, 0);
        p.seg_rows = pl.seg_rows;
        p.n_strips = pl.n_strips;
        p.n_segs = pl.n_segs;
        p.strips_total = pl.n_strips;
        srcnn_ctx::SeamScratch *sc = nullptr;
        int rc;
        if ((rc = seam_scratch_for_stream(c, &sc))) return rc;
        const size_t n = (size_t)n_frames * p.strips_total * (p.row_end - p.row_begin) * CSEAM_FLOATS * sizeof(float);
        if ((rc = reserve(c, sc->cbuf, n))) return rc;
        p.cseam = static_cast<float *>(sc->cbuf.p);
    }
    const bool fused32 = mode == MODE_FUSED && !split16;
    if (mode != MODE_L12 && (n_frames == 1 || (fused32 && n_frames < kItemBatchMax && !(p.tune & 128))) && !l3_aligned) {
        static const char *env_seams = SRCNN_DEBUG_ENV("SRCNN_DEBUG_SEAMS");
        const int seam_knob = env_seams ? std::atoi(env_seams) : 3;
        const bool want_seams = mode == MODE_FUSED && !split16 && (seam_knob & 1);
        int rc;
        auto items_for = [&](int n_strips_, bool seams_) -> int {
            int rc2 = build_items(c, n_strips_, p.row_begin, p.row_end, p.height, wgs_per_cu, seams_, &table);
            if (!rc2 && table->count == 0 && wgs_per_cu == 2 && seams_)
                rc2 = build_items(c, n_strips_, p.row_begin, p.row_end, p.height, 1, seams_, &table);
            return rc2;
        };
        bool col_seams = false;
        if (want_seams && (seam_knob & 2) && cseam_pays(p.width)) {
            const int ns_cs = (p.width + FW - 1) / FW;
            if ((rc = items_for(ns_cs, true))) return rc;
            if (table->count > 0) {
                p.strips_total = ns_cs;
                col_seams = true;
            } else {
                table = nullptr;
            }
        }
        if (!table && (rc = items_for(pl.n_strips, want_seams))) return rc;
        grid_items = table->count;
        if (grid_items > 0) {
            p.items = static_cast<const int *>(table->dev.p);
            if (table->n_seams > 0 || col_seams) {
                srcnn_ctx::SeamScratch *sc = nullptr;
                for (auto &e : c->seam_scratch)
                    if (e.used && e.stream == c->stream) sc = &e;
                for (auto &e : c->seam_scratch)
                    if (!sc && !e.used) sc = &e;
                if (!sc) {
                    HIP_TRY(c, hipDeviceSynchronize());
                    for (auto &e : c->seam_scratch) e.used = false;
                    sc = &c->seam_scratch[0];
                }
                sc->used = true;
                sc->stream = c->stream;
                defer = may_defer && c->defer_seams && c->defer_block == 0 && !c->safe_hazards && fused32 && n_frames == 1 && !p.pre && !(p.tune & 16) &&
                        table->n_seams > 0 && (col_seams ? table->separated : true) &&
                        !(c->mode == SRCNN_MODE_REFBYTES || c->mode == SRCNN_MODE_REFBYTES16);
                if (defer) sc->flip ^= 1;
                DevBuf &rbuf = defer && sc->flip ? sc->buf2 : sc->buf, &cbuf = defer && sc->flip ? sc->cbuf2 : sc->cbuf;
                if (table->n_seams > 0) {
                    if ((rc = reserve(c, rbuf, (size_t)n_frames * table->n_seams * SEAM_FLOATS * NTHREADS * sizeof(float)))) return rc;
                    p.seam = static_cast<float *>(rbuf.p);
                }
                if (col_seams) {
                    const size_t n = (size_t)n_frames * p.strips_total * (p.row_end - p.row_begin) * CSEAM_FLOATS * sizeof(float);
                    if ((rc = reserve(c, cbuf, n))) return rc;
                    p.cseam = static_cast<float *>(cbuf.p);
                }
            }
            p.n_strips = 1;
            p.n_segs = grid_items;
            p.items_per_frame = grid_items;
            p.seams_per_frame = std::max(1, table->n_seams);
        }
    }
    if (fused32 && n_frames > 1 && grid_items == 0) {
        static const char *env_seams = SRCNN_DEBUG_ENV("SRCNN_DEBUG_SEAMS");
        const int ns_cs = (p.width + FW - 1) / FW;
        (void)ns_cs;
        if ((!env_seams || (std::atoi(env_seams) & 2)) && cseam_pays(p.width)) {
            pl = make_plan(c, p.width, p.row_end - p.row_begin, n_frames, halo, wgs_per_cu, 0);
            p.seg_rows = pl.seg_rows;
            p.n_strips = pl.n_strips;
            p.n_segs = pl.n_segs;
            p.strips_total = pl.n_strips;
            srcnn_ctx::SeamScratch *sc = nullptr;
            for (auto &e : c->seam_scratch)
                if (e.used && e.stream == c->stream) sc = &e;
            for (auto &e : c->seam_scratch)
                if (!sc && !e.used) sc = &e;
            if (!sc) {
                HIP_TRY(c, hipDeviceSynchronize());
                for (auto &e : c->seam_scratch) e.used = false;
                sc = &c->seam_scratch[0];
            }
            sc->used = true;
            sc->stream = c->stream;
            const size_t n = (size_t)n_frames * p.strips_total * (p.row_end - p.row_begin) * CSEAM_FLOATS * sizeof(float);
            int rc;
            if ((rc = reserve(c, sc->cbuf, n))) return rc;
            p.cseam = static_cast<float *>(sc->cbuf.p);
        }
    }
    const bool fix = mode == MODE_FUSED && (c->mode == SRCNN_MODE_REFBYTES || c->mode == SRCNN_MODE_REFBYTES16) && !p.pre;
    srcnn_ctx::SeamScratch *fsc = nullptr;
    size_t fix_scat_cap = 0, fix_dense_cap = 0, fix_flag_pitch = 0;
    float fix_delta_used = 0.f;
    if (fix) {
        if (n_frames != 1 || fix_frame < 0 || fix_frame >= fix_frames || fix_frames > FIX_BATCH_FRAMES)
            return fail(c, SRCNN_ERR_STATE, "REFBYTES strip launches hold one frame");
        int rc;
        if ((rc = seam_scratch_for_stream(c, &fsc))) return rc;
        const int rows = p.row_end - p.row_begin;
        fix_scat_cap = fixup_list_entries(p.width, rows, fix_frames, &fix_dense_cap);
        fix_flag_pitch = (size_t)rows * (size_t)p.dst_stride;
        if ((rc = reserve(c, fsc->flag, fix_flag_pitch * (size_t)fix_frames))) return rc;
        if ((rc = reserve(c, fsc->fix_lists, (fix_scat_cap + fix_dense_cap) * sizeof(unsigned)))) return rc;
        if ((rc = reserve(c, fsc->fix_counters, FIX_COUNTERS * sizeof(unsigned)))) return rc;
        if (!c->fix_totals.p) {
            if ((rc = reserve(c, c->fix_totals, FIX_TOTALS * sizeof(unsigned long long)))) return rc;
            HIP_TRY(c, hipMemsetAsync(c->fix_totals.p, 0, FIX_TOTALS * sizeof(unsigned long long), c->stream));
        }
        p.flag = static_cast<uint8_t *>(fsc->flag.p) + (size_t)fix_frame * fix_flag_pitch - (long)(p.row_begin - p.dst_row0) * p.dst_stride;
        fix_delta_used = c->mode == SRCNN_MODE_REFBYTES16 ? c->fix_delta * (8.f / 6.f) : c->fix_delta;
        p.fix_delta = fix_delta_used;
        p.fix_scale = 253.f / (2.f * fix_delta_used);
        const bool r16 = c->mode == SRCNN_MODE_REFBYTES16;
        const bool local = (r16 ? c->fix_local16 : c->fix_local) > 0.f;
        p.fix_kl = local ? (r16 ? c->fix_local16 * std::ldexp(1.f, -10) : c->fix_local) * c->fix_margin * std::ldexp(1.f, -24) : 0.f;
        p.fix_abs = local ? kFixAbsLocal : fix_delta_used;
        p.fix_counters = static_cast<unsigned *>(fsc->fix_counters.p);
    }
    p.wfrag = static_cast<const float *>(c->wfrag.p);
    p.wfrag16 = static_cast<const uint32_t *>(c->wfrag16.p);
    p.sink = static_cast<float *>(c->sink.p);
    p.b3 = c->b3;
    if (split16) {
        if (!c->split16_ok)
            return fail(c, SRCNN_ERR_STATE, "SRCNN_MODE_SPLIT16: these weights exceed the f16 ranges of the mode "
                                            "(layer maps must stay below 8192 / 16384 for 8-bit input); use SRCNN_MODE_MFMA");
        int rc;
        if ((rc = flush_seams(c))) return rc;
        HIP_TRY(c, launch_split16(p, n_frames, c->stream, pad));
    }
    else if (c->pending.valid && defer && c->pending.stream == c->stream && grid_items > 0 && fold_is_safe(c->pending.f.prev, p)) {
        c->pending.f.first_block = grid_items;
        c->pending.valid = false;
        HIP_TRY(c, launch_strip_fold(p, c->pending.f, c->stream, pad));
    } else {
        int rc;
        if ((rc = flush_seams(c))) return rc;
        HIP_TRY(c, (c->safe_hazards ? launch_strip_safe : launch_strip)(mode, p, n_frames, c->stream, pad));
    }
    static const char *env_merge = SRCNN_DEBUG_ENV("SRCNN_DEBUG_SEAM_MERGE");
    if (defer && !(env_merge && std::atoi(env_merge) == 0)) {
        FoldParams &f = c->pending.f;
        f.prev = p;
        f.seams = static_cast<const int *>(table->dev_seams.p);
        f.winmap = p.cseam ? static_cast<const unsigned char *>(table->dev_winmap.p) : nullptr;
        f.n_seams = table->n_seams;
        f.cblocks = p.cseam ? (int)(((long)(p.strips_total - 1) * (p.row_end - p.row_begin) + 255) / 256) : 0;
        f.first_block = 0;
        c->pending.stream = c->stream;
        c->pending.valid = true;
    } else if (p.seam && p.cseam && table->separated && !(env_merge && std::atoi(env_merge) == 0)) {
        HIP_TRY(c, launch_seams_merged(p, table->n_seams * n_frames, static_cast<const int *>(table->dev_seams.p),
                                       static_cast<const unsigned char *>(table->dev_winmap.p), n_frames, c->stream));
    } else {
        if (p.seam) HIP_TRY(c, launch_seams(p, table->n_seams * n_frames, static_cast<const int *>(table->dev_seams.p), c->stream));
        if (p.cseam) HIP_TRY(c, launch_cseams(p, n_frames, c->stream));
    }
    if (fix && fix_frame == fix_frames - 1) {
        FixParams f{};
        f.n_frames = fix_frames;
        f.src_frame_pitch = p.src_frame_pitch;
        f.dst_frame_pitch = p.dst_frame_pitch;
        f.flag_frame_pitch = (long)fix_flag_pitch;
        f.src = p.src - (long)fix_frame * p.src_frame_pitch;
        f.src_stride = p.src_stride;
        f.src_row0 = p.src_row0;
        f.src_top = p.src_top;
        f.src_bot = p.src_bot;
        f.halo_stride = p.halo_stride;
        f.src_row1 = p.src_row1;
        f.dst = p.dst - (long)fix_frame * p.dst_frame_pitch;
        f.flag = p.flag - (long)fix_frame * (long)fix_flag_pitch;
        f.dst_stride = p.dst_stride;
        f.dst_row0 = p.dst_row0;
        f.width = p.width;
        f.height = p.height;
        f.row_begin = p.row_begin;
        f.row_end = p.row_end;
        f.wraw = static_cast<const float *>(c->wraw.p);
        f.counters = p.fix_counters;
        f.totals = static_cast<unsigned long long *>(c->fix_totals.p);
        f.scat = static_cast<unsigned *>(fsc->fix_lists.p);
        f.dense = f.scat + fix_scat_cap;
        f.delta = fix_delta_used;
        f.code_step = 2.f * fix_delta_used / 253.f;
        f.kl = r16_kl(c, p.fix_kl);
        f.abs_term = p.fix_abs;
        static const char *env_rerun = SRCNN_DEBUG_ENV("SRCNN_DEBUG_FORCE_RERUN");
        f.rerun_above = (env_rerun && std::atoi(env_rerun)) ? -1.f : c->fix_strict ? 0.5f : INFINITY;
        static const char *env_lds = SRCNN_DEBUG_ENV("SRCNN_DEBUG_FIX_LDS");
        const bool lds_weights = env_lds ? std::atoi(env_lds) == 1
                                         : (long)p.width * (p.row_end - p.row_begin) * fix_frames <= 2400000L;
        HIP_TRY(c, launch_fixup(f, c->n_cu, c->fix_strict, lds_weights, c->stream));
    }
    return SRCNN_OK;
}

}
}

extern "C" {


int srcnn_conv99x11_dev(srcnn_ctx *c, const uint8_t *d_src, size_t src_stride, float *d_planes,
                        size_t plane_stride, size_t plane_pitch, int width, int height)
{
    BIND(c);
    int rc = SRCNN_OK;
    (void)rc;
    if (!luma_path_ok(c)) return refuse_spatial(c, "srcnn_conv99x11_dev");
    if (!c->has_l12) return fail(c, SRCNN_ERR_STATE, "layers 1-2 not loaded (srcnn_set_weights / srcnn_conv99x11)");
    if (bad_plane(d_src, src_stride, width, height) || bad_plane(d_planes, plane_stride, width, height) ||
        plane_pitch < plane_stride * (size_t)height || bad_pitch(plane_pitch))
        return fail(c, SRCNN_ERR_INVALID, "conv99x11_dev: bad plane geometry");
    if (c->mode == SRCNN_MODE_EXACT) {
        HIP_TRY(c, launch_conv99x11_exact(d_src, (long)src_stride, 0, d_planes, (long)plane_stride,
                                          (long)plane_pitch, 0, width, height, 1,
                                          static_cast<const float *>(c->wraw.p), c->stream));
        return SRCNN_OK;
    }
    StripParams p{};
    p.src = d_src;
    p.src_stride = (long)src_stride;
    p.planes_out = d_planes;
    p.pl_stride = (long)plane_stride;
    p.pl_pitch = (long)plane_pitch;
    p.width = width;
    p.height = height;
    p.row_begin = 0;
    p.row_end = height;
    return run_strip(c, MODE_L12, p, 1);
}

int srcnn_conv55_dev(srcnn_ctx *c, const float *d_planes, size_t plane_stride, size_t plane_pitch,
                     uint8_t *d_dst, size_t dst_stride, int width, int height, float *d_preclamp)
{
    BIND(c);
    int rc = SRCNN_OK;
    (void)rc;
    if (!luma_path_ok(c)) return refuse_spatial(c, "srcnn_conv55_dev");
    if (!c->has_l3) return fail(c, SRCNN_ERR_STATE, "layer 3 not loaded (srcnn_set_weights / srcnn_conv55)");
    if (bad_plane(d_planes, plane_stride, width, height) || bad_plane(d_dst, dst_stride, width, height) ||
        plane_pitch < plane_stride * (size_t)height || bad_pitch(plane_pitch))
        return fail(c, SRCNN_ERR_INVALID, "conv55_dev: bad plane geometry");
    if (c->mode == SRCNN_MODE_EXACT) {
        HIP_TRY(c, launch_conv55_exact(d_planes, (long)plane_stride, (long)plane_pitch, 0, d_dst, d_preclamp,
                                       (long)dst_stride, 0, width, height, 1,
                                       static_cast<const float *>(c->wraw.p) + 7329, c->b3, c->stream));
        return SRCNN_OK;
    }
    StripParams p{};
    p.planes_in = d_planes;
    p.pl_stride = (long)plane_stride;
    p.pl_pitch = (long)plane_pitch;
    p.dst = d_dst;
    p.pre = d_preclamp;
    p.dst_stride = (long)dst_stride;
    p.width = width;
    p.height = height;
    p.row_begin = 0;
    p.row_end = height;
    return run_strip(c, MODE_L3, p, 1);
}

int srcnn_forward_y_unfused_dev(srcnn_ctx *c, const uint8_t *d_src, size_t src_stride, size_t src_frame_pitch,
                                uint8_t *d_dst, size_t dst_stride, size_t dst_frame_pitch, int width,
                                int height, int n_frames, float *d_work)
{
    BIND(c);
    int rc = SRCNN_OK;
    (void)rc;
    if (!luma_path_ok(c)) return refuse_spatial(c, "srcnn_forward_y_unfused_dev");
    if (!has_model(c)) return fail(c, SRCNN_ERR_STATE, "%s", kNoModel);
    if (bad_plane(d_src, src_stride, width, height) || bad_plane(d_dst, dst_stride, width, height) || !d_work ||
        n_frames <= 0)
        return fail(c, SRCNN_ERR_INVALID, "forward_y_unfused_dev: bad arguments");
    static const char *env_plpad = SRCNN_DEBUG_ENV("SRCNN_DEBUG_PLPAD");
    const long pitch = (long)width * height + (env_plpad ? std::atol(env_plpad) : 0);
    if (bad_pitch((size_t)pitch)) return fail(c, SRCNN_ERR_INVALID, "forward_y_unfused_dev: plane too large");
    if (c->mode == SRCNN_MODE_EXACT) {
        HIP_TRY(c, launch_conv99x11_exact(d_src, (long)src_stride, (long)src_frame_pitch, d_work, width, pitch,
                                          32 * pitch, width, height, n_frames,
                                          static_cast<const float *>(c->wraw.p), c->stream));
        HIP_TRY(c, launch_conv55_exact(d_work, width, pitch, 32 * pitch, d_dst, nullptr, (long)dst_stride,
                                       (long)dst_frame_pitch, width, height, n_frames,
                                       static_cast<const float *>(c->wraw.p) + 7329, c->b3, c->stream));
        return SRCNN_OK;
    }
    StripParams p{};
    p.src = d_src;
    p.src_stride = (long)src_stride;
// ... 173 lines not shown
```

### srcnn_cpp_amd/csrc/srcnn_mfma.hip

```cpp
#include "srcnn_kernels.h"

#include <type_traits>

#ifndef SRCNN_SAFE_HAZARDS
#define SRCNN_SAFE_HAZARDS 0
#endif
#if SRCNN_SAFE_HAZARDS
#define SRCNN_KNS safe
#else
#define SRCNN_KNS fast
#endif

namespace srcnn {
namespace SRCNN_KNS {

typedef float f32x16 __attribute__((ext_vector_type(16)));
typedef float f32x2 __attribute__((ext_vector_type(2)));

#define MFMA(a, b, c) __builtin_amdgcn_mfma_f32_32x32x2f32((a), (b), (c), 0, 0, 0)

__device__ __forceinline__ f32x16 mfma_first(float a, float b, const f32x16 &c)
{
#if SRCNN_SAFE_HAZARDS
    return MFMA(a, b, c);
#endif
    f32x16 d;
    asm volatile("v_mfma_f32_32x32x2_f32 %0, %1, %2, %3" : "=&v"(d) : "v"(a), "v"(b), "v"(c));
    return d;
}
__device__ __forceinline__ f32x16 mfma_first0(float a, float b)
{
#if SRCNN_SAFE_HAZARDS
    const f32x16 z = {0};
    return MFMA(a, b, z);
#endif
    f32x16 d;
    asm volatile("v_mfma_f32_32x32x2_f32 %0, %1, %2, 0" : "=&v"(d) : "v"(a), "v"(b));
    return d;
}


__device__ __forceinline__ int clampi(int v, int lo, int hi) { return min(max(v, lo), hi); }

__device__ __forceinline__ unsigned lane_off(unsigned x)
{
    asm volatile("" : "+v"(x));
    return x;
}
template <typename T>
__device__ __forceinline__ __attribute__((address_space(1))) T *scalar_base(T *p)
{
    __attribute__((address_space(1))) T *g = (__attribute__((address_space(1))) T *)p;
    asm volatile("" : "+s"(g));
    return g;
}

template <typename T>
__device__ __forceinline__ T *uniform_ptr(T *p)
{
    const unsigned long long a = (unsigned long long)p;
    const unsigned lo = __builtin_amdgcn_readfirstlane((unsigned)a), hi = __builtin_amdgcn_readfirstlane((unsigned)(a >> 32));
    return (T *)(((unsigned long long)hi << 32) | lo);
}

__device__ __forceinline__ void lds_barrier()
{
    asm volatile("s_waitcnt lgkmcnt(0)\n\ts_barrier" ::: "memory");
}

__device__ __forceinline__ float relu(float x)
{
    float r;
    asm("v_max_f32 %0, 0, %1" : "=v"(r) : "v"(x));
    return r;
}

__device__ const signed char CSEAM_TERMS[15][9] = {
    {4, 0, 124, 1, 125, 2, 126, 3, 127}, {3, 0, 125, 1, 126, 2, 127, 0, 0}, {1, 0, 126, 0, 0, 0, 0, 0, 0},
    {1, 0, 127, 0, 0, 0, 0, 0, 0},       {1, 1, 127, 0, 0, 0, 0, 0, 0},     {1, 2, 0, 0, 0, 0, 0, 0, 0},
    {1, 3, 1, 0, 0, 0, 0, 0, 0},         {1, 4, 2, 0, 0, 0, 0, 0, 0},       {1, 1, 0, 0, 0, 0, 0, 0, 0},
    {1, 2, 1, 0, 0, 0, 0, 0, 0},         {1, 3, 2, 0, 0, 0, 0, 0, 0},       {1, 4, 3, 0, 0, 0, 0, 0, 0},
    {1, 3, 0, 0, 0, 0, 0, 0, 0},         {1, 4, 0, 0, 0, 0, 0, 0, 0},       {1, 4, 1, 0, 0, 0, 0, 0, 0}};

struct CseamLane {
    int cnt, off[4];
};
__device__ __forceinline__ CseamLane cseam_lane(int e)
{
    CseamLane cl = {0, {0, 0, 0, 0}};
    if (e < 15) {
        const signed char *t = CSEAM_TERMS[e];
        cl.cnt = t[0];
#pragma unroll
        for (int i = 0; i < 4; ++i) cl.off[i] = i < t[0] ? t[1 + 2 * i] * FW + t[2 + 2 * i] : 0;
    }
    return cl;
}
__device__ __forceinline__ void cseam_export(const float *tile, float *dst, int e, const CseamLane &cl)
{
    const float a = tile[cl.off[0]], b = tile[cl.off[1]], c = tile[cl.off[2]], d = tile[cl.off[3]];
    float v = a;
    v = cl.cnt > 1 ? v + b : v;
    v = cl.cnt > 2 ? v + c : v;
    v = cl.cnt > 3 ? v + d : v;
    if (cl.cnt > 0) dst[(unsigned)e] = v;
}

__device__ __forceinline__ void relu_pairs(f32x16 &a, const f32x2 ones)
{
#if SRCNN_SAFE_HAZARDS
#pragma unroll
    for (int q = 0; q < 16; ++q) a[q] = __builtin_fmaxf(a[q], 0.f);
    return;
#endif
#pragma unroll
    for (int q = 0; q < 8; ++q) {
        f32x2 pr = {a[2 * q], a[2 * q + 1]};
        asm("v_pk_mul_f32 %0, %0, %1 clamp" : "+v"(pr) : "s"(ones));
        a[2 * q] = pr.x;
        a[2 * q + 1] = pr.y;
    }
}

constexpr bool fast_kernel(int mode, bool pre, int diag)
{
    (void)diag;
    return mode == MODE_FUSED && !pre;
}

template <int MODE, bool PRE, int DIAG = 0, bool FIX = false, bool HALO3 = false>
__device__ __forceinline__ void strip_body(const StripParams &p)
{
    static_assert(!FIX || (MODE == MODE_FUSED && !PRE && DIAG == 0), "flags belong to the production fused kernel");
    static_assert(!HALO3 || (MODE == MODE_FUSED && !PRE && DIAG == 0), "halo buffers belong to the production fused kernel");
    if constexpr (FIX) {
        if (blockIdx.x == 0)
            for (int i = threadIdx.x; i < FIX_COUNTERS; i += 256) p.fix_counters[i] = 0u;
    }
    unsigned long long lt[4] = {0, 0, 0, 0};
    if constexpr (DIAG == 2) lt[0] = __builtin_amdgcn_s_memrealtime();
    extern __shared__ __attribute__((aligned(16))) char smem[];
    float *ylds = reinterpret_cast<float *>(smem);
    float *fbuf = (MODE == MODE_L3) ? ylds : ylds + 2 * YR * YP;

    const int tid = threadIdx.x;
    const int lane = tid & 63;
    const int wave = __builtin_amdgcn_readfirstlane(tid >> 6);
    const int j = lane & 31;
    const int half = lane >> 5;

    constexpr int HALO = (MODE == MODE_L12) ? 0 : 2;

    const int W = p.width, H = p.height;
    int bid = blockIdx.x;
    int strip, frame = 0, ys, ye, seam_up = -1, seam_dn = -1;
    if (p.items) {
        frame = bid / p.items_per_frame;
        const int *it = p.items + ITEM_INTS * (bid - frame * p.items_per_frame);
        strip = it[0];
        ys = it[1];
        ye = it[2];
        if constexpr (MODE == MODE_FUSED) {
            seam_up = it[3] >= 0 ? it[3] + frame * p.seams_per_frame : -1;
            seam_dn = it[4] >= 0 ? it[4] + frame * p.seams_per_frame : -1;
        }
        if (ys >= ye) return;
    } else {
        if (!(p.tune & 8)) {
            const int nwg = gridDim.x, q = nwg >> 3, r = nwg & 7, xcd = bid & 7;
            bid = (xcd < r ? xcd * (q + 1) : r * (q + 1) + (xcd - r) * q) + (bid >> 3);
        }
        strip = bid % p.n_strips;
        bid /= p.n_strips;
        const int seg = bid % p.n_segs;
        frame = bid / p.n_segs;
        ys = p.row_begin + seg * p.seg_rows;
        ye = min(ys + p.seg_rows, p.row_end);
    }

    const bool cs = (MODE != MODE_L12) && p.cseam != nullptr;
    const CseamLane cl = cseam_lane((cs && threadIdx.x < 64 && (threadIdx.x & 31) < 15 &&
                                     (threadIdx.x < 32 || fast_kernel(MODE, PRE, DIAG)))
                                        ? (int)(threadIdx.x & 31) : 15);
    const int halo_c = cs ? 0 : HALO;
    const int xs = strip * (FW - 2 * halo_c);
    const int gx0 = xs - halo_c;
    float *cs_row0 = (cs && wave == 0)
                         ? p.cseam + (((long)frame * p.strips_total + strip) * (p.row_end - p.row_begin) - p.row_begin) * CSEAM_FLOATS
                         : nullptr;
    const bool top_open = seam_up >= 0, bot_open = seam_dn >= 0;
    const int f_lo = top_open ? ys : max(ys - HALO, 0);
    const int f_hi = bot_open ? ye : min(ye + HALO, H);
    const int out_lo = top_open ? ys + 2 : ys, out_hi = bot_open ? ye - 2 : ye;

    const float *wf = p.wfrag + lane;
    float w1f[2][41], w2f[32], w3f[16];
    f32x16 b2v = {0};
    if constexpr (MODE != MODE_L3) {
#pragma unroll
        for (int t = 0; t < 2; ++t)
#pragma unroll
            for (int s = 0; s < 41; ++s) w1f[t][s] = wf[(t * 41 + s) * 64];
        constexpr int L2 = (MODE == MODE_L12) ? FRAG_L2U : FRAG_L2, B2 = (MODE == MODE_L12) ? FRAG_B2U : FRAG_B2;
#pragma unroll
        for (int q = 0; q < 32; ++q) w2f[q] = wf[(L2 + q) * 64];
#pragma unroll
        for (int q = 0; q < 16; ++q) b2v[q] = wf[(B2 + q) * 64];
    }
    if constexpr (MODE != MODE_L12) {
        constexpr int L3 = (MODE == MODE_L3) ? FRAG_L3U : FRAG_L3;
#pragma unroll
        for (int q = 0; q < 16; ++q) w3f[q] = wf[(L3 + q) * 64];
    }
    const f32x2 ones = {1.0f, 1.0f};

    const uint8_t *srcf = nullptr;
    int ycol = 0;
    if constexpr (MODE != MODE_L3) {
        srcf = p.src + (long)frame * p.src_frame_pitch;
        ycol = clampi(gx0 - 4 + tid, 0, W - 1);
    }
    const int y_last = min(H - 1, f_hi + 3);
    auto y_row = [&](int r) -> const uint8_t * {
        if constexpr (HALO3) {
            if (r < p.src_row0) return p.src_top + (long)(r - (p.src_row0 - 6)) * p.halo_stride;
            if (r >= p.src_row1) return p.src_bot + (long)(r - p.src_row1) * p.halo_stride;
        }
        return srcf + (long)(r - p.src_row0) * p.src_stride;
    };
    auto load_y = [&](int r) -> uint8_t {
        const uint8_t *row = y_row(clampi(r, 0, y_last));
        return row[(unsigned)ycol];
    };
    auto stage_y = [&](int r, uint8_t v) {
        const int slot = r & (YR - 1);
        const float fv = (float)v;
        ylds[slot * YP + tid] = fv;
        ylds[(slot + YR) * YP + tid] = fv;
    };
    if constexpr (MODE != MODE_L3) {
        if (tid < YP) {
            uint8_t v[9];
#pragma unroll
            for (int q = 0; q < 9; ++q) v[q] = load_y(f_lo - 4 + q);
#pragma unroll
            for (int q = 0; q < 9; ++q) stage_y(f_lo - 4 + q, v[q]);
        }
        __syncthreads();
    }
    asm volatile("s_waitcnt vmcnt(0)" ::: "memory");
    if constexpr (MODE != MODE_L3) {
#pragma unroll
        for (int t = 0; t < 2; ++t)
#pragma unroll
            for (int k = 0; k < 41; ++k) asm volatile("" : "+v"(w1f[t][k]));
#pragma unroll
        for (int q = 0; q < 32; ++q) asm volatile("" : "+v"(w2f[q]));
        asm volatile("" : "+v"(b2v));
    }
    if constexpr (MODE != MODE_L12) {
#pragma unroll
        for (int q = 0; q < 16; ++q) asm volatile("" : "+v"(w3f[q]));
    }

    if constexpr (DIAG == 2) lt[1] = __builtin_amdgcn_s_memrealtime();

    const int xi = 32 * wave + j;
    const int gx = gx0 + xi;


    constexpr bool FASTK = fast_kernel(MODE, PRE, DIAG);
    static_assert(!FIX || FASTK, "the flag threshold reads plane 5 through the FAST kernels' column offsets");
    constexpr int FSLOT = 6 * FW;
    int xn[5] = {0, 0, 0, 0, 0};
    bool px_ok = false;
    if constexpr (MODE != MODE_L12) {
#pragma unroll
        for (int n = 0; n < 5; ++n) {
            xn[n] = clampi(clampi(gx + n - 2, 0, W - 1) - gx0, 0, FW - 1);
            if constexpr (FASTK) xn[n] += n * FW + half * FSLOT;
        }
        px_ok = cs ? (gx < W) && (xi >= 2 || strip == 0) && (xi < FW - 2 || strip == p.strips_total - 1)
                   : (xi >= HALO) && (xi < FW - HALO) && (gx < W);
    }
    CseamLane cl2 = cl;
    if constexpr (FASTK) {
#pragma unroll
        for (int i = 0; i < 4; ++i) cl2.off[i] += half * FSLOT;
    }
    float R[4][3] = {{0.f, 0.f, 0.f}, {0.f, 0.f, 0.f}, {0.f, 0.f, 0.f}, {0.f, 0.f, 0.f}};
    long o_out = (long)frame * p.dst_frame_pitch + (long)(f_lo - 3 - p.dst_row0) * p.dst_stride;
    long o_src = (long)(min(f_lo + 5, y_last) - p.src_row0) * p.src_stride;
    long o_pl = (long)frame * p.pl_frame_pitch + (long)(MODE == MODE_L3 ? min(f_lo + 1, H - 1) : f_lo) * p.pl_stride;
    auto scale_thr = [&](const float *fr) -> float {
        float s1 = fr[xn[0] + 5 * FW];
#pragma unroll
        for (int n = 1; n < 5; ++n) s1 += fr[xn[n] + (5 - n) * FW];
        return fix_threshold(s1, p.fix_delta, p.fix_kl, p.fix_abs);
    };
    auto finalize = [&](long o, float acc, bool ok, const float *fr) {
        const float v = acc + p.b3;
        auto row = scalar_base(p.dst + o);
        if (ok) row[lane_off((unsigned)gx)] = (uint8_t)clampi((int)v, 0, 255);
        if constexpr (FIX) {
            auto frow = scalar_base(p.flag + o);
            const float thr = scale_thr(fr);
            if (ok) frow[lane_off((unsigned)gx)] = fix_code(v, thr, p.fix_delta, p.fix_scale);
        }
        if constexpr (PRE) {
            float *prow = p.pre + o;
            if (ok) prow[(unsigned)gx] = v;
        }
    };
    auto ftile = [&](int g, int slot) -> float * {
        if constexpr (FASTK) return fbuf + ((4 - ((g + slot) & 3)) & 3) * FSLOT;
        else return fbuf + (((g & 1) * 3 + slot) * 6) * FW;
    };
    auto vertical = [&](int f, const f32x16 &t) {
        const int fplane = 3 * half * FW + xi;
        if (top_open && f < ys + SEAM_ROWS) {
            const int r = f - ys;
            float *o = p.seam + ((long)seam_up * SEAM_FLOATS + seam_t_off(r)) * NTHREADS + tid;
#pragma unroll
            for (int s = 0; s < 3; ++s)
#pragma unroll
                for (int m = 1; m < 5; ++m)
                    if (m > r) o[(s * (4 - r) + (m - r - 1)) * NTHREADS] = t[5 * s + m];
        }
        if (f > 0) {
            float *fo = ftile(f, 0) + fplane;
#pragma unroll
            for (int s = 0; s < 3; ++s) {
                fo[s * FW] = R[3][s] + t[5 * s + 4];
                R[3][s] = R[2][s] + t[5 * s + 3];
                R[2][s] = R[1][s] + t[5 * s + 2];
                R[1][s] = R[0][s] + t[5 * s + 1];
                R[0][s] = t[5 * s];
            }
        } else {
#pragma unroll
            for (int s = 0; s < 3; ++s) {
                R[0][s] = t[5 * s];
                R[1][s] = t[5 * s] + t[5 * s + 1];
                R[2][s] = R[1][s] + t[5 * s + 2];
                R[3][s] = 0.f;
            }
        }
        if (f == H - 1) {
            float *f1 = ftile(f, 1) + fplane, *f2 = ftile(f, 2) + fplane;
#pragma unroll
            for (int s = 0; s < 3; ++s) {
                f1[s * FW] = R[3][s] + t[5 * s + 4];
                f2[s * FW] = (R[2][s] + t[5 * s + 3]) + t[5 * s + 4];
            }
        }
    };
    float hv[5];
    auto hp_load = [&](int g, int slot) {
        const float *fr = ftile(g, slot);
#pragma unroll
        for (int n = 0; n < 5; ++n) hv[n] = FASTK ? fr[xn[n]] : fr[n * FW + xn[n]];
    };
    auto hp_use = [&](int g, int slot) {
        float acc = hv[0];
#pragma unroll
        for (int n = 1; n < 5; ++n) acc += hv[n];
        const int y = g - 2 + slot;
// ... 525 lines not shown
```

### srcnn_cpp_amd/csrc/srcnn_plan.cpp

```cpp
#include "srcnn_ctx.h"

using namespace srcnn;
using namespace srcnn::host;

namespace srcnn {
namespace host {

Plan make_plan(const srcnn_ctx *c, int width, int rows, int n_frames, int halo, int wgs_per_cu, int col_halo)
{
    const int ow = FW - 2 * (col_halo < 0 ? halo : col_halo);
    Plan best{rows, (width + ow - 1) / ow, 1};
    const long slots = (long)wgs_per_cu * c->n_cu;
    double best_eff = -1.0;
    const int max_segs = std::min(rows, 4096);
    for (int ns = 1; ns <= max_segs; ++ns) {
        const int seg = (rows + ns - 1) / ns;
        const int real_ns = (rows + seg - 1) / seg;
        if (real_ns != ns) continue;
        const long wgs = (long)best.n_strips * ns * n_frames;
        const long rounds = (wgs + slots - 1) / slots;
        const double fill = (double)wgs / (double)(rounds * slots);
        constexpr int STARTUP_ROWS = 3;
        const double useful = (double)rows / ((double)ns * (seg + 2 * halo + STARTUP_ROWS));
        const double eff = fill * useful;
        if (eff > best_eff + 1e-9) {
            best_eff = eff;
            best.seg_rows = seg;
            best.n_segs = ns;
        }
    }
    return best;
}

double kPairFast = 6.40, kPairSlow = 8.40, kAlone = 3.76, kStartFast = 3.63, kStartSlow = 5.44;

double cu_finish_estimate(int fast_rows, int slow_rows, double speed)
{
    static const bool once = [] {
        if (const char *e = SRCNN_DEBUG_ENV("SRCNN_DEBUG_RATES"))
            std::sscanf(e, "%lf,%lf,%lf,%lf,%lf", &kPairFast, &kPairSlow, &kAlone, &kStartFast, &kStartSlow);
        return true;
    }();
    (void)once;
    const double tf = kStartFast + fast_rows * kPairFast, ts = kStartSlow + slow_rows * kPairSlow;
    double t;
    if (tf <= ts) t = tf + std::max(0.0, slow_rows - (tf - kStartSlow) / kPairSlow) * kAlone;
    else t = ts + std::max(0.0, fast_rows - (ts - kStartFast) / kPairFast) * kAlone;
    return t / speed;
}

ItemPlan plan_items_balanced(int n_cu, int n_strips, int row_begin, int row_end, int skew_pct, int extra_top, int extra_bot,
                             const double *cu_speed = nullptr)
{
    const ItemPlan none;
    constexpr int kMinRows = 10;
    constexpr int kSepMinRows = 12;
    constexpr double kLaunchSaved = 8.0;
    const int hs = row_end - row_begin;
    const int slots = 2 * n_cu;
    if (n_cu <= 0 || n_strips <= 0 || n_strips > n_cu || hs <= 0 || slots / n_strips < 2 || hs / (slots / n_strips + 1) < kMinRows + 2)
        return none;
    const int kbase = slots / n_strips, kextra = slots % n_strips;
    std::vector<int> k((size_t)n_strips), a((size_t)n_strips);
    int fast_total = 0;
    for (int s = 0; s < n_strips; ++s) {
        k[(size_t)s] = kbase + (s < kextra ? 1 : 0);
        a[(size_t)s] = k[(size_t)s] / 2;
        fast_total += a[(size_t)s];
    }
    for (int pass = 0; pass < 2 && fast_total < n_cu; ++pass)
        for (int s = 0; s < n_strips && fast_total < n_cu; ++s)
            if ((pass == 1 || k[(size_t)s] % 2 == 1) && a[(size_t)s] < k[(size_t)s] - 1) { ++a[(size_t)s]; ++fast_total; }
    if (fast_total != n_cu) return none;
    struct Item { int strip, rows, cu; bool fast; int extra = 0; };
    std::vector<Item> items;
    const double d = std::min(std::max(skew_pct, 0), 60) / 100.0;
    for (int s = 0; s < n_strips; ++s) {
        const int na = a[(size_t)s], nb = k[(size_t)s] - na;
        const double u = hs / (na * (1.0 + d) + nb * (1.0 - d));
        double acc = 0.0;
        int used = 0;
        for (int j = 0; j < k[(size_t)s]; ++j) {
            const bool fast = (j % 2 == 0) ? (j / 2 < na) : !((j / 2) < nb);
            acc += fast ? (1.0 + d) * u : (1.0 - d) * u;
            const int upto = (j == k[(size_t)s] - 1) ? hs : (int)std::lround(acc);
            items.push_back({s, upto - used, -1, fast, (j == 0 ? extra_top : 0) + (j == k[(size_t)s] - 1 ? extra_bot : 0)});
            used = upto;
        }
        constexpr int kStagger = 16;
        if ((s & 1) && k[(size_t)s] >= 3) {
            Item &first = items[items.size() - (size_t)k[(size_t)s]], &last = items.back();
            const int x = std::min(kStagger, first.rows - kMinRows);
            if (x > 0) {
                first.rows -= x;
                last.rows += x;
            }
        }
    }
    for (int s = 0; s < n_strips; ++s) {
        int have = 0;
        for (auto &it : items) if (it.strip == s && it.fast) ++have;
        for (auto &it : items) if (it.strip == s && have > a[(size_t)s] && it.fast) { it.fast = false; --have; }
        for (auto &it : items) if (it.strip == s && have < a[(size_t)s] && !it.fast) { it.fast = true; ++have; }
    }
    std::vector<int> fi, si;
    for (int i = 0; i < (int)items.size(); ++i) (items[(size_t)i].fast ? fi : si).push_back(i);
    if ((int)fi.size() != n_cu || (int)si.size() != n_cu) return none;
    std::stable_sort(fi.begin(), fi.end(), [&](int x, int y) { return items[(size_t)x].rows + items[(size_t)x].extra > items[(size_t)y].rows + items[(size_t)y].extra; });
    std::stable_sort(si.begin(), si.end(), [&](int x, int y) { return items[(size_t)x].rows + items[(size_t)x].extra < items[(size_t)y].rows + items[(size_t)y].extra; });
    for (int c = 0; c < n_cu; ++c) items[(size_t)fi[(size_t)c]].cu = items[(size_t)si[(size_t)c]].cu = c;
    auto speed = [&](int c) { return cu_speed && cu_speed[c] > 0.5 && cu_speed[c] < 2.0 ? cu_speed[c] : 1.0; };
    auto work = [&](int i) { return items[(size_t)i].rows + items[(size_t)i].extra; };
    auto finish = [&](int c) { return cu_finish_estimate(work(fi[(size_t)c]), work(si[(size_t)c]), speed(c)); };
    std::vector<std::vector<int>> in_strip((size_t)n_strips);
    for (int i = 0; i < (int)items.size(); ++i) in_strip[(size_t)items[(size_t)i].strip].push_back(i);
    std::vector<double> fin((size_t)n_cu);
    for (int c = 0; c < n_cu; ++c) fin[(size_t)c] = finish(c);
    std::vector<int> by_time((size_t)n_cu);
    auto bounds = [&](int s_) {
        std::vector<int> b;
        int y = 0;
        for (size_t q = 0; q + 1 < in_strip[(size_t)s_].size(); ++q) b.push_back(y += items[(size_t)in_strip[(size_t)s_][q]].rows);
        return b;
    };
    auto apart = [&](const std::vector<int> &x, const std::vector<int> &y) {
        for (int u : x)
            for (int v : y)
                if (std::abs(u - v) < SEAM_ROWS) return false;
        return true;
    };
    auto strip_apart = [&](int s_) {
        const std::vector<int> b = bounds(s_);
        return (s_ == 0 || apart(b, bounds(s_ - 1))) && (s_ + 1 >= n_strips || apart(b, bounds(s_ + 1)));
    };
    std::vector<std::vector<int>> cur((size_t)n_strips);
    std::vector<int> pos(items.size());
    for (int s_ = 0; s_ < n_strips; ++s_)
        for (size_t q = 0; q < in_strip[(size_t)s_].size(); ++q) pos[(size_t)in_strip[(size_t)s_][q]] = (int)q;
    auto clear_of = [&](const std::vector<int> &nbr, int b) {
        const auto it = std::lower_bound(nbr.begin(), nbr.end(), b);
        return (it == nbr.end() || *it - b >= SEAM_ROWS) && (it == nbr.begin() || b - *(it - 1) >= SEAM_ROWS);
    };
    auto move_ok = [&](int from, int to) {
        const int s_ = items[(size_t)from].strip, pa = pos[(size_t)from], pb = pos[(size_t)to];
        const int lo = std::min(pa, pb), hi = std::max(pa, pb) - 1, delta = pa < pb ? -1 : 1;
        for (int q = lo; q <= hi; ++q) {
            const int b = cur[(size_t)s_][(size_t)q] + delta;
            if (s_ > 0 && !clear_of(cur[(size_t)s_ - 1], b)) return false;
            if (s_ + 1 < n_strips && !clear_of(cur[(size_t)s_ + 1], b)) return false;
        }
        return true;
    };
    auto move_apply = [&](int from, int to) {
        const int s_ = items[(size_t)from].strip, pa = pos[(size_t)from], pb = pos[(size_t)to];
        const int lo = std::min(pa, pb), hi = std::max(pa, pb) - 1, delta = pa < pb ? -1 : 1;
        for (int q = lo; q <= hi; ++q) cur[(size_t)s_][(size_t)q] += delta;
    };
    auto search = [&](bool keep_apart) {
        for (int iter = 0; iter < 40 * n_cu; ++iter) {
            for (int c = 0; c < n_cu; ++c) by_time[(size_t)c] = c;
            std::sort(by_time.begin(), by_time.end(), [&](int x, int y) { return fin[(size_t)x] > fin[(size_t)y]; });
            bool moved = false;
            for (int rank = 0; rank < n_cu && !moved; ++rank) {
                const int c = by_time[(size_t)rank];
                double best_gain = 1e-6;
                int best_from = -1, best_to = -1;
                for (int from : {fi[(size_t)c], si[(size_t)c]}) {
                    if (items[(size_t)from].rows <= kMinRows) continue;
                    items[(size_t)from].rows -= 1;
                    const double mine = finish(c);
                    for (int to : in_strip[(size_t)items[(size_t)from].strip]) {
                        const int c2 = items[(size_t)to].cu;
                        if (c2 == c) continue;
                        items[(size_t)to].rows += 1;
                        const double theirs = finish(c2);
                        const double gain = fin[(size_t)c] - std::max(mine, theirs);
                        if (theirs < fin[(size_t)c] && gain > best_gain && (!keep_apart || move_ok(from, to))) {
                            best_gain = gain;
                            best_from = from;
                            best_to = to;
                        }
                        items[(size_t)to].rows -= 1;
                    }
                    items[(size_t)from].rows += 1;
                }
                if (best_from >= 0) {
                    if (keep_apart) move_apply(best_from, best_to);
                    items[(size_t)best_from].rows -= 1;
                    items[(size_t)best_to].rows += 1;
                    fin[(size_t)c] = finish(c);
                    fin[(size_t)items[(size_t)best_to].cu] = finish(items[(size_t)best_to].cu);
                    moved = true;
                }
            }
            if (!moved) break;
        }
    };
    const std::vector<Item> start = items;
    static const char *env_sep = SRCNN_DEBUG_ENV("SRCNN_DEBUG_SEPARATE");
    static const char *env_sep_rows = SRCNN_DEBUG_ENV("SRCNN_DEBUG_SEP_MINROWS"), *env_sep_saved = SRCNN_DEBUG_ENV("SRCNN_DEBUG_SEP_SAVED");
    const int sep_min_rows = env_sep_rows ? std::atoi(env_sep_rows) : kSepMinRows;
    bool separated = !(env_sep && std::atoi(env_sep) == 0) && n_strips >= 2 && hs / (kbase + 1) >= sep_min_rows;
    constexpr int kSlack = 4;
    for (int s_ = 1; s_ < n_strips && separated; ++s_) {
        const std::vector<int> left = bounds(s_ - 1);
        const std::vector<int> &mine = in_strip[(size_t)s_];
        for (size_t q = 0; q + 1 < mine.size() && separated; ++q) {
            int y = 0;
            for (size_t r = 0; r <= q; ++r) y += items[(size_t)mine[r]].rows;
            auto dist = [&](int b) {
                int dmin = 1 << 30;
                for (int v : left) dmin = std::min(dmin, std::abs(v - b));
                return dmin;
            };
            if (dist(y) >= SEAM_ROWS + kSlack) continue;
            Item &up = items[(size_t)mine[q]], &dn = items[(size_t)mine[q + 1]];
            int best_d = 0;
            double best_t = 1e30;
            for (int d = -3 * SEAM_ROWS; d <= 3 * SEAM_ROWS; ++d) {
                if (dist(y + d) < SEAM_ROWS || up.rows + d < kMinRows || dn.rows - d < kMinRows) continue;
                up.rows += d;
                dn.rows -= d;
                const double t = std::max(finish(up.cu), finish(dn.cu)) + 0.5 * std::abs(d) +
                                 4.0 * std::max(0, SEAM_ROWS + kSlack - dist(y + d));
                up.rows -= d;
                dn.rows += d;
                if (t < best_t) { best_t = t; best_d = d; }
            }
            if (best_t >= 1e30) { separated = false; break; }
            up.rows += best_d;
            dn.rows -= best_d;
        }
    }
    for (int s_ = 0; s_ < n_strips && separated; ++s_) separated = strip_apart(s_);
    auto slowest = [&] {
        double mx = 0.0;
        for (int c = 0; c < n_cu; ++c) mx = std::max(mx, fin[(size_t)c]);
        return mx;
    };
    if (separated) {
        for (int c = 0; c < n_cu; ++c) fin[(size_t)c] = finish(c);
        for (int s_ = 0; s_ < n_strips; ++s_) cur[(size_t)s_] = bounds(s_);
        search(true);
    }
    const std::vector<Item> apart_items = items;
    const double apart_t = separated ? slowest() : 1e30;
    items = start;
    for (int c = 0; c < n_cu; ++c) fin[(size_t)c] = finish(c);
    search(false);
    const double launch_saved = env_sep_saved ? std::atof(env_sep_saved) : kLaunchSaved;
    if (separated && apart_t <= slowest() + launch_saved) {
        items = apart_items;
        for (int c = 0; c < n_cu; ++c) fin[(size_t)c] = finish(c);
    } else {
        separated = false;
    }
    if (SRCNN_DEBUG_ENV("SRCNN_DEBUG_PLANLOG")) {
        double mx = 0, mn = 1e30;
        for (int c = 0; c < n_cu; ++c) { mx = std::max(mx, fin[(size_t)c]); mn = std::min(mn, fin[(size_t)c]); }
        std::fprintf(stderr, "plan: separated=%d finish %.1f..%.1f\n", (int)separated, mn, mx);
    }
    ItemPlan plan;
    plan.separated = separated;
    std::vector<int> y0(items.size()), up(items.size(), -1), dn(items.size(), -1);
    for (int s = 0; s < n_strips; ++s) {
        int y = row_begin, prev = -1;
        for (int i : in_strip[(size_t)s]) {
            if (items[(size_t)i].rows < 2 * SEAM_ROWS) return none;
            y0[(size_t)i] = y;
            y += items[(size_t)i].rows;
            if (prev >= 0) {
                const int id = plan.n_seams();
                plan.seams.insert(plan.seams.end(), {s, y0[(size_t)i]});
                dn[(size_t)prev] = id;
                up[(size_t)i] = id;
            }
            prev = i;
        }
        if (y != row_end) return none;
    }
    auto emit = [&](int i) {
        plan.items.insert(plan.items.end(), {items[(size_t)i].strip, y0[(size_t)i], y0[(size_t)i] + items[(size_t)i].rows, up[(size_t)i], dn[(size_t)i]});
    };
    for (int c = 0; c < n_cu; ++c) emit(fi[(size_t)c]);
    for (int c = 0; c < n_cu; ++c) emit(si[(size_t)c]);
    return plan;
}

ItemPlan plan_items_raw(int n_cu, int n_strips, int row_begin, int row_end, int skew_pct, int wgs_per_cu = 2,
                        bool want_seams = false, int extra_top = 0, int extra_bot = 0)
{
    const ItemPlan none;
    static const char *env_plan = SRCNN_DEBUG_ENV("SRCNN_DEBUG_PLAN");
    if (wgs_per_cu == 2 && want_seams && skew_pct > 0 && !(env_plan && std::atoi(env_plan) == 1)) {
        const ItemPlan balanced = plan_items_balanced(n_cu, n_strips, row_begin, row_end, skew_pct, extra_top, extra_bot);
        if (balanced.count() > 0) return balanced;
    }
    const int rows = row_end - row_begin;
    int slots = wgs_per_cu * n_cu;
    const int min_rows = want_seams ? 10 : 24;
    if (skew_pct <= 0 || n_strips <= 0 || n_strips > n_cu) return none;
    bool underfilled = false;
    if (wgs_per_cu == 1 && want_seams && rows / min_rows < slots / n_strips + 1) {
        slots = n_strips * (rows / min_rows);
        underfilled = true;
    }
    if (slots / n_strips < 2 || (!underfilled && rows / (slots / n_strips + 1) < min_rows)) return none;
    if (wgs_per_cu == 1) skew_pct = 0;
    const int kbase = slots / n_strips, kextra = slots % n_strips;
    std::vector<int> k(n_strips), a(n_strips);
    int fast_total = 0;
    for (int s = 0; s < n_strips; ++s) {
        k[s] = kbase + (s < kextra ? 1 : 0);
        a[s] = wgs_per_cu == 1 ? k[s] : k[s] / 2;
        fast_total += a[s];
    }
    for (int s = 0; fast_total < n_cu && s < n_strips; ++s)
        if (k[s] % 2 == 1 && a[s] < k[s] - 1) { ++a[s]; ++fast_total; }
    for (int s = 0; fast_total < n_cu && s < n_strips; ++s)
        if (a[s] < k[s] - 1) { ++a[s]; ++fast_total; }
    if (wgs_per_cu == 2 && fast_total != n_cu) return none;
    const double d = skew_pct / 100.0;
    std::vector<std::vector<int>> bounds(n_strips);
    for (int s = 0; s < n_strips; ++s) {
        const int b = k[s] - a[s];
        const double u = rows / (a[s] * (1.0 + d) + b * (1.0 - d));
        bounds[s].resize(k[s] + 1);
        for (int j = 0; j <= k[s]; ++j) {
            const double y = j <= a[s] ? j * (1.0 + d) * u : a[s] * (1.0 + d) * u + (j - a[s]) * (1.0 - d) * u;
            bounds[s][j] = row_begin + std::min(rows, std::max(0, (int)std::lround(y)));
        }
        bounds[s][0] = row_begin;
        bounds[s][k[s]] = row_end;
        for (int j = 1; j <= k[s]; ++j)
            if (bounds[s][j] <= bounds[s][j - 1]) return none;
    }
    struct Item { int strip, y0, y1, up, dn; };
    ItemPlan plan;
    for (int s = 0; s < n_strips && want_seams; ++s)
        for (int j = 0; j < k[s]; ++j)
            if (bounds[s][j + 1] - bounds[s][j] < 2 * SEAM_ROWS) want_seams = false;
    std::vector<Item> fast, slow;
    for (int s = 0; s < n_strips; ++s)
        for (int j = 0; j < k[s]; ++j) {
            int up = -1, dn = -1;
            if (want_seams && j > 0) up = plan.n_seams() - 1;
            if (want_seams && j < k[s] - 1) {
                dn = plan.n_seams();
                plan.seams.insert(plan.seams.end(), {s, bounds[s][j + 1]});
            }
            (j < a[s] ? fast : slow).push_back({s, bounds[s][j], bounds[s][j + 1], up, dn});
        }
    std::stable_sort(fast.begin(), fast.end(), [](const Item &x, const Item &y) { return x.y1 - x.y0 > y.y1 - y.y0; });
    std::stable_sort(slow.begin(), slow.end(), [](const Item &x, const Item &y) { return x.y1 - x.y0 < y.y1 - y.y0; });
    plan.items.reserve(ITEM_INTS * (size_t)slots);
    for (const Item &it : fast) plan.items.insert(plan.items.end(), {it.strip, it.y0, it.y1, it.up, it.dn});
    for (const Item &it : slow) plan.items.insert(plan.items.end(), {it.strip, it.y0, it.y1, it.up, it.dn});
    return plan.count() == slots ? plan : none;
}

int skew_percent()
{
    static const char *env_skew = SRCNN_DEBUG_ENV("SRCNN_DEBUG_SKEW");
    return env_skew ? std::atoi(env_skew) : 10;
}

ItemPlan plan_items(int n_cu, int n_strips, int row_begin, int row_end, int skew_pct, int wgs_per_cu, bool want_seams, int extra_top,
                    int extra_bot)
{
    return plan_items_raw(n_cu, n_strips, row_begin, row_end, skew_pct, wgs_per_cu, want_seams, extra_top, extra_bot);
}

int build_items(srcnn_ctx *c, int n_strips, int row_begin, int row_end, int height, int wgs_per_cu, bool want_seams,
                const srcnn_ctx::ItemTable **table)
{
    *table = nullptr;
    static const char *env_edge = SRCNN_DEBUG_ENV("SRCNN_DEBUG_PLAN_EDGES");
    const bool edges = !(env_edge && std::atoi(env_edge) == 0);
    const int extra_top = edges && row_begin > 0 ? 2 : 0, extra_bot = edges && row_end < height ? 2 : 0;
    const int key[8] = {n_strips, row_begin, row_end, skew_percent(), c->n_cu, wgs_per_cu, want_seams ? 1 : 0, extra_top + 4 * extra_bot};
    srcnn_ctx::ItemTable *victim = &c->item_tables[0];
    for (auto &t : c->item_tables) {
        if (t.stamp && std::memcmp(key, t.key, sizeof(key)) == 0) {
            t.stamp = ++c->item_clock;
            *table = &t;
            return SRCNN_OK;
        }
        if (t.stamp < victim->stamp) victim = &t;
    }
    const ItemPlan plan = plan_items(c->n_cu, n_strips, row_begin, row_end, key[3], wgs_per_cu, want_seams, extra_top, extra_bot);
    if (victim->stamp) {
        if (int rc = flush_seams(c)) return rc;
        HIP_TRY(c, hipDeviceSynchronize());
    }
    if (plan.count() > 0) {
        int rc;
        if ((rc = reserve(c, victim->dev, plan.items.size() * sizeof(int)))) return rc;
        HIP_TRY(c, hipMemcpy(victim->dev.p, plan.items.data(), plan.items.size() * sizeof(int), hipMemcpyHostToDevice));
        if (plan.n_seams() > 0) {
            if ((rc = reserve(c, victim->dev_seams, plan.seams.size() * sizeof(int)))) return rc;
            HIP_TRY(c, hipMemcpy(victim->dev_seams.p, plan.seams.data(), plan.seams.size() * sizeof(int),
                                 hipMemcpyHostToDevice));
            if (plan.separated) {
                const int rows = row_end - row_begin;
                std::vector<unsigned char> win((size_t)n_strips * rows, 0);
                for (int id = 0; id < plan.n_seams(); ++id) {
                    const int s_ = plan.seams[2 * (size_t)id], b = plan.seams[2 * (size_t)id + 1];
                    for (int y = b - 2; y < b + 2; ++y)
                        if (y >= row_begin && y < row_end) win[(size_t)s_ * rows + (y - row_begin)] = 1;
                }
                if ((rc = reserve(c, victim->dev_winmap, win.size()))) return rc;
                HIP_TRY(c, hipMemcpy(victim->dev_winmap.p, win.data(), win.size(), hipMemcpyHostToDevice));
            }
        }
    }
    std::memcpy(victim->key, key, sizeof(key));
    victim->count = plan.count();
    victim->n_seams = plan.n_seams();
    victim->separated = plan.n_seams() > 0 && plan.separated;
    victim->stamp = ++c->item_clock;
    *table = victim;
    return SRCNN_OK;
}

int split16_wgs_per_cu(bool split16, int ) { return split16 ? 1 : 2; }

int seam_scratch_for_stream(srcnn_ctx *c, srcnn_ctx::SeamScratch **out)
{
    srcnn_ctx::SeamScratch *sc = nullptr;
    for (auto &e : c->seam_scratch)
        if (e.used && e.stream == c->stream) sc = &e;
    for (auto &e : c->seam_scratch)
        if (!sc && !e.used) sc = &e;
    if (!sc) {
        HIP_TRY(c, hipDeviceSynchronize());
        for (auto &e : c->seam_scratch) e.used = false;
        sc = &c->seam_scratch[0];
    }
    sc->used = true;
    sc->stream = c->stream;
    *out = sc;
    return SRCNN_OK;
}

bool cseam_pays(int width)
{
    const int ns_cs = (width + FW - 1) / FW, ns_halo = (width + FW - 5) / (FW - 4);
    return ns_cs < ns_halo && (width - (ns_cs - 1) * FW >= 4 || ns_cs == 1);
}

bool f32_mfma(const srcnn_ctx *c) { return c->mode == SRCNN_MODE_MFMA || c->mode == SRCNN_MODE_REFBYTES; }
int frames_per_launch(const srcnn_ctx *c, int width, int height, int n_frames)
{
    static const char *env_loop = SRCNN_DEBUG_ENV("SRCNN_DEBUG_FRAMELOOP");
    const size_t px = (size_t)width * height;
    if (c->mode == SRCNN_MODE_REFBYTES || c->mode == SRCNN_MODE_REFBYTES16) return 1;
    if (c->mode != SRCNN_MODE_MFMA || n_frames <= 1) return kGridBatchChunk;
    if (!(env_loop && std::atoi(env_loop) == 0) &&
        ((px >= ((size_t)4 << 20) && n_frames < kItemBatchMax) || (px >= ((size_t)3 << 19) && n_frames <= 8)))
        return 1;
    return n_frames < kItemBatchMax ? kItemBatchChunk : kGridBatchChunk;
}

}
}

extern "C" {

int srcnn_query_plan(srcnn_ctx *c, int width, int height, int n_frames, int out[6])
{
    if (!c || !out || width <= 0 || height <= 0 || n_frames <= 0) return SRCNN_ERR_INVALID;
    static const char *env_seams = SRCNN_DEBUG_ENV("SRCNN_DEBUG_SEAMS");
    const int wgs_per_cu = split16_wgs_per_cu(c->mode == SRCNN_MODE_SPLIT16 || c->mode == SRCNN_MODE_REFBYTES16, 0);
    const int nl = std::min(n_frames, frames_per_launch(c, width, height, n_frames));
    const int seam_knob = env_seams ? std::atoi(env_seams) : 3;
    const int ns_cs = (width + FW - 1) / FW;
    bool col_seams = f32_mfma(c) && (seam_knob & 2) && (nl > 1 || (seam_knob & 1)) && cseam_pays(width);
    int items_per_cu = wgs_per_cu;
    const bool row_seams = f32_mfma(c) && (seam_knob & 1);
    auto fits = [&](int n_strips_, int per_cu) { return !plan_items(c->n_cu, n_strips_, 0, height, skew_percent(), per_cu, row_seams).items.empty(); };
    if (col_seams && nl == 1 && !fits(ns_cs, wgs_per_cu)) {
        if (wgs_per_cu == 2 && fits(ns_cs, 1)) items_per_cu = 1;
        else col_seams = false;
    }
    if (!col_seams && nl == 1 && row_seams && wgs_per_cu == 2) {
        const int ns_halo = (width + FW - 5) / (FW - 4);
        if (!fits(ns_halo, 2) && fits(ns_halo, 1)) items_per_cu = 1;
    }
    const Plan pl = make_plan(c, width, height, nl, 2, wgs_per_cu, col_seams ? 0 : -1);
    out[0] = pl.n_strips * pl.n_segs * n_frames;
    out[1] = pl.seg_rows;
    out[2] = pl.n_strips;
    out[3] = pl.n_segs;
    if (nl == 1 || (f32_mfma(c) && n_frames < kItemBatchMax)) {
        const std::vector<int> items =
            plan_items(c->n_cu, pl.n_strips, 0, height, skew_percent(), items_per_cu,
                       f32_mfma(c) && (seam_knob & 1)).items;
        if (!items.empty()) {
            out[0] = (int)items.size() / ITEM_INTS * n_frames;
            out[1] = 0;
            for (size_t i = 0; i < items.size(); i += ITEM_INTS) out[1] = std::max(out[1], items[i + 2] - items[i + 1]);
            out[3] = ((int)items.size() / ITEM_INTS + pl.n_strips - 1) / pl.n_strips;
        }
    }
    out[4] = (int)strip_lds_bytes(MODE_FUSED);
    out[5] = NTHREADS;
    return SRCNN_OK;
}

#ifdef SRCNN_TUNING_BUILD
int srcnn_debug_plan_items(int n_cu, int n_strips, int row_begin, int row_end, int skew_pct, int wgs_per_cu,
                                      int want_seams, int *items, int max_items, int *seams, int max_seams,
                                      int *n_seams)
{
    const int extra_top = (wgs_per_cu >> 4) & 15, extra_bot = (wgs_per_cu >> 8) & 15;
    wgs_per_cu &= 15;
    const ItemPlan plan = plan_items(n_cu, n_strips, row_begin, row_end, skew_pct, wgs_per_cu, want_seams != 0, extra_top, extra_bot);
    if (plan.count() > max_items || plan.n_seams() > max_seams || !items || !seams || !n_seams) return SRCNN_ERR_INVALID;
    if (!plan.items.empty()) std::memcpy(items, plan.items.data(), plan.items.size() * sizeof(int));
    if (!plan.seams.empty()) std::memcpy(seams, plan.seams.data(), plan.seams.size() * sizeof(int));
    *n_seams = plan.n_seams();
    return plan.count();
}
#endif

}
```

Measured before the change: 8796 MPix/s.

## Claim work items per XCC via atomics and rate-weighted XCC item lists

Adds XCC-aware dynamic item claiming to the fused f32 MFMA strip kernel. Each workgroup reads its hardware XCC id and atomically claims an item from that XCC's list, stealing from other XCCs' lists when its own is empty. The planner splits items across XCCs using per-XCC rate estimates, with odd XCCs given a slightly lower default rate. Weight loading is moved ahead of the claim so the loads overlap the atomics. The aim is to balance load when dispatch order or XCC speed differs, at the cost of atomics, a double-buffered claim counter array cleared by block 0, and a per-block claim scan at kernel start.

```diff
diff --git a/include/srcnn_amd.h b/include/srcnn_amd.h
--- a/include/srcnn_amd.h
+++ b/include/srcnn_amd.h
@@ -318,6 +318,8 @@
 
 int srcnn_query_plan(srcnn_ctx *ctx, int width, int height, int n_frames, int out[6]);
 
+int srcnn_query_plan_xcc(srcnn_ctx *ctx, int width, int height, int out[8]);
+
 #ifdef __cplusplus
 }
 #endif
diff --git a/srcnn_cpp_amd/__init__.py b/srcnn_cpp_amd/__init__.py
--- a/srcnn_cpp_amd/__init__.py
+++ b/srcnn_cpp_amd/__init__.py
@@ -158,6 +158,7 @@
         "srcnn_ipc_open": ([vp, C.POINTER(C.c_ubyte * 64), C.POINTER(vp)], i),
         "srcnn_ipc_close": ([vp, vp], i),
         "srcnn_query_plan": ([vp, i, i, i, C.POINTER(i * 6)], i),
+        "srcnn_query_plan_xcc": ([vp, i, i, C.POINTER(i * 8)], i),
         "srcnn_fixup_stats": ([vp, C.POINTER(C.c_ulonglong * 4), C.POINTER(C.c_float), C.POINTER(C.c_float)], i),
         "srcnn_set_fixup_strict": ([vp, i], i),
         "srcnn_set_seam_deferral": ([vp, i], i),
@@ -207,7 +208,7 @@
     "srcnn_forward_y_dev",
     "srcnn_forward_y_rows_dev", "srcnn_forward_y_rows_halo_dev", "srcnn_halo_transport", "srcnn_forward_y_unfused_dev", "srcnn_conv99x11_dev",
     "srcnn_conv55_dev", "srcnn_conv99x11_to_dev", "srcnn_conv55_from_dev", "srcnn_dev_alloc", "srcnn_dev_free",
-    "srcnn_dev_download", "srcnn_dev_upload", "srcnn_ipc_export", "srcnn_ipc_open", "srcnn_ipc_close", "srcnn_query_plan", "srcnn_fixup_stats", "srcnn_set_fixup_strict", "srcnn_set_fixup_margin", "srcnn_set_fixup_local", "srcnn_fixup_local_stats", "srcnn_set_seam_deferral", "srcnn_flush", "srcnn_scaled_size", "srcnn_bgr2ycrcb", "srcnn_ycrcb2bgr",
+    "srcnn_dev_download", "srcnn_dev_upload", "srcnn_ipc_export", "srcnn_ipc_open", "srcnn_ipc_close", "srcnn_query_plan", "srcnn_query_plan_xcc", "srcnn_fixup_stats", "srcnn_set_fixup_strict", "srcnn_set_fixup_margin", "srcnn_set_fixup_local", "srcnn_fixup_local_stats", "srcnn_set_seam_deferral", "srcnn_flush", "srcnn_scaled_size", "srcnn_bgr2ycrcb", "srcnn_ycrcb2bgr",
     "srcnn_resize_cubic", "srcnn_process_bgr", "srcnn_process_bgr_dev",
     "srcnn_stripe_rows", "srcnn_forward_y_frames_multi", "srcnn_forward_y_lanes_dev", "srcnn_forward_y_striped", "srcnn_forward_y_striped_frames", "srcnn_forward_y_striped_dev",
     "srcnn_set_model", "srcnn_get_model_f2", "srcnn_set_padding", "srcnn_get_padding",
@@ -653,6 +654,11 @@
         return dict(workgroups=out[0], seg_rows=out[1], strips=out[2], segments=out[3],
                     lds_bytes=out[4], threads=out[5])
 
+    def query_plan_xcc(self, width, height):
+        out = (C.c_int * 8)()
+        self._check(self._lib.srcnn_query_plan_xcc(self._h, width, height, C.byref(out)))
+        return list(out)
+
     def conv99(self, src, dst, kernel, bias):
         src, ss = _plane(src, np.uint8, "src")
         dst, ds = _plane(dst, np.float32, "dst", True)
diff --git a/srcnn_cpp_amd/csrc/srcnn_api.cpp b/srcnn_cpp_amd/csrc/srcnn_api.cpp
--- a/srcnn_cpp_amd/csrc/srcnn_api.cpp
+++ b/srcnn_cpp_amd/csrc/srcnn_api.cpp
@@ -70,6 +70,7 @@
     if (!c) return SRCNN_ERR_NOMEM;
     c->device = device;
     c->n_cu = prop.multiProcessorCount > 0 ? prop.multiProcessorCount : 256;
+    std::memcpy(c->xcc_rates, kXccRates, sizeof(c->xcc_rates));
     DeviceScope dev_scope_(c);
     if (dev_scope_.rc != SRCNN_OK || hipStreamCreateWithFlags(&c->own_stream, hipStreamNonBlocking) != hipSuccess) {
         delete c;
@@ -136,12 +137,14 @@
         release(sc.flag);
         release(sc.fix_lists);
         release(sc.fix_counters);
+        release(sc.claim);
     }
     release(c->fix_totals);
     for (auto &t : c->item_tables) {
         release(t.dev);
         release(t.dev_seams);
         release(t.dev_winmap);
+        release(t.dev_claim);
     }
     for (int k = 0; k < 2; ++k) {
         for (hipEvent_t e : {c->sf_up[k], c->sf_k[k], c->sf_down[k]})
@@ -341,6 +344,34 @@
     if (!dst || bytes > c->sink.cap) return SRCNN_ERR_INVALID;
     HIP_TRY(c, hipStreamSynchronize(c->stream));
     HIP_TRY(c, hipMemcpy(dst, c->sink.p, bytes, hipMemcpyDeviceToHost));
+    return SRCNN_OK;
+}
+
+int srcnn_debug_set_xcc_rates(srcnn_ctx *c, const double *rates, int claim)
+{
+    BIND(c);
+    for (int x = 0; rates && x < kXccCount; ++x)
+        if (!(rates[x] > 0.25 && rates[x] < 4.0)) return fail(c, SRCNN_ERR_INVALID, "xcc rates must lie in (0.25, 4)");
+    std::memcpy(c->xcc_rates, rates ? rates : kXccRates, sizeof(c->xcc_rates));
+    c->xcc_claim = claim != 0;
+    return SRCNN_OK;
+}
+
+int srcnn_debug_claim_counts(srcnn_ctx *c, unsigned out[9])
+{
+    BIND(c);
+    if (!out) return SRCNN_ERR_INVALID;
+    const srcnn_ctx::SeamScratch *sc = c->last_claim;
+    if (!sc || !sc->claim.p || sc->claim_words <= 0) return fail(c, SRCNN_ERR_STATE, "no claiming launch yet");
+    HIP_TRY(c, hipDeviceSynchronize());
+    std::vector<unsigned> words((size_t)sc->claim_words);
+    HIP_TRY(c, hipMemcpy(words.data(), static_cast<const unsigned *>(sc->claim.p) + (size_t)sc->claim_flip * sc->claim_words,
+                         words.size() * sizeof(unsigned), hipMemcpyDeviceToHost));
+    for (int k = 0; k < 9; ++k) out[k] = 0u;
+    for (size_t i = 0; i < words.size(); ++i) {
+        if (words[i]) ++out[i % kXccCount];
+        out[8] = std::max(out[8], words[i]);
+    }
     return SRCNN_OK;
 }
 
diff --git a/srcnn_cpp_amd/csrc/srcnn_ctx.h b/srcnn_cpp_amd/csrc/srcnn_ctx.h
--- a/srcnn_cpp_amd/csrc/srcnn_ctx.h
+++ b/srcnn_cpp_amd/csrc/srcnn_ctx.h
@@ -158,6 +158,8 @@
         srcnn::host::DevBuf buf2, cbuf2;
         int flip = 0;
         srcnn::host::DevBuf flag, fix_lists, fix_counters;
+        srcnn::host::DevBuf claim;
+        int claim_words = 0, claim_flip = 0;
     };
     SeamScratch seam_scratch[4];
     srcnn::host::DevBuf bgr_in, bgr_out, ycc_lo, ycc_hi, y_sr, tables;
@@ -176,12 +178,19 @@
         int n_seams = 0;
         srcnn::host::DevBuf dev, dev_seams;
         srcnn::host::DevBuf dev_winmap;
+        double rates[8] = {0, 0, 0, 0, 0, 0, 0, 0};
+        srcnn::host::DevBuf dev_claim;
+        int xcc_len[8] = {0, 0, 0, 0, 0, 0, 0, 0};
+        int claim_slots = 0;
         bool separated = false;
         unsigned long stamp = 0;
     };
     static constexpr int kItemTables = 32;
     ItemTable item_tables[kItemTables];
     unsigned long item_clock = 0;
+    double xcc_rates[8] = {1, 1, 1, 1, 1, 1, 1, 1};
+    bool xcc_claim = true;
+    SeamScratch *last_claim = nullptr;
     std::vector<float> host_raw = std::vector<float>(8129, 0.f);
     void *pin_plane[2] = {nullptr, nullptr};
     size_t pin_plane_cap = 0;
@@ -318,14 +327,17 @@
     int seg_rows, n_strips, n_segs;
 };
 Plan make_plan(const srcnn_ctx *c, int width, int rows, int n_frames, int halo, int wgs_per_cu = 2, int col_halo = -1);
+constexpr int kXccCount = 8;
+extern const double kXccRates[kXccCount];
 struct ItemPlan {
     std::vector<int> items, seams;
+    std::vector<int> lists[kXccCount];
     bool separated = false;
     int count() const { return (int)items.size() / ITEM_INTS; }
     int n_seams() const { return (int)seams.size() / 2; }
 };
 ItemPlan plan_items(int n_cu, int n_strips, int row_begin, int row_end, int skew_pct, int wgs_per_cu = 2, bool want_seams = false,
-                    int extra_top = 0, int extra_bot = 0);
+                    int extra_top = 0, int extra_bot = 0, const double *xcc_rates = nullptr);
 int skew_percent();
 int build_items(srcnn_ctx *c, int n_strips, int row_begin, int row_end, int height, int wgs_per_cu, bool want_seams,
                 const srcnn_ctx::ItemTable **table);
diff --git a/srcnn_cpp_amd/csrc/srcnn_kernels.h b/srcnn_cpp_amd/csrc/srcnn_kernels.h
--- a/srcnn_cpp_amd/csrc/srcnn_kernels.h
+++ b/srcnn_cpp_amd/csrc/srcnn_kernels.h
@@ -83,7 +83,11 @@
     float fix_delta, fix_scale;
     float fix_kl, fix_abs;
     unsigned *fix_counters;
-};
+    unsigned *claim, *claim_zero;
+    const int *claim_items;
+    int claim_slots, claim_words;
+};
+constexpr int CLAIM_LEN_INTS = 8;
 
 enum { FIX_N_SCAT = 0, FIX_N_DENSE = 1, FIX_N_CHANGED = 2, FIX_MAX_DEV = 3, FIX_N_RERUN = 4,
        FIX_MAX_RATIO = 5,
diff --git a/srcnn_cpp_amd/csrc/srcnn_launch.cpp b/srcnn_cpp_amd/csrc/srcnn_launch.cpp
--- a/srcnn_cpp_amd/csrc/srcnn_launch.cpp
+++ b/srcnn_cpp_amd/csrc/srcnn_launch.cpp
@@ -80,6 +80,10 @@
     p.n_strips = pl.n_strips;
     p.n_segs = pl.n_segs;
     p.items = nullptr;
+    p.claim = p.claim_zero = nullptr;
+    p.claim_items = nullptr;
+    p.claim_slots = p.claim_words = 0;
+    srcnn_ctx::SeamScratch *claim_sc = nullptr;
     p.seam = nullptr;
     p.cseam = nullptr;
     p.strips_total = pl.n_strips;
@@ -162,6 +166,25 @@
             p.n_segs = grid_items;
             p.items_per_frame = grid_items;
             p.seams_per_frame = std::max(1, table->n_seams);
+            if (c->xcc_claim && fused32 && n_frames == 1 && !p.pre && table->claim_slots > 0) {
+                srcnn_ctx::SeamScratch *sc = nullptr;
+                if ((rc = seam_scratch_for_stream(c, &sc))) return rc;
+                const int words = 4 * c->n_cu + 64;
+                if (!sc->claim.p) {
+                    if ((rc = reserve(c, sc->claim, 2 * (size_t)words * sizeof(unsigned)))) return rc;
+                    HIP_TRY(c, hipMemsetAsync(sc->claim.p, 0, 2 * (size_t)words * sizeof(unsigned), c->stream));
+                    sc->claim_words = words;
+                }
+                if (table->claim_slots * kXccCount <= sc->claim_words) {
+                    const int set = sc->claim_flip ^ 1;
+                    p.claim = static_cast<unsigned *>(sc->claim.p) + (size_t)set * sc->claim_words;
+                    p.claim_zero = static_cast<unsigned *>(sc->claim.p) + (size_t)(set ^ 1) * sc->claim_words;
+                    p.claim_items = static_cast<const int *>(table->dev_claim.p);
+                    p.claim_slots = table->claim_slots;
+                    p.claim_words = sc->claim_words;
+                    claim_sc = sc;
+                }
+            }
         }
     }
     if (fused32 && n_frames > 1 && grid_items == 0) {
@@ -241,6 +264,10 @@
         int rc;
         if ((rc = flush_seams(c))) return rc;
         HIP_TRY(c, (c->safe_hazards ? launch_strip_safe : launch_strip)(mode, p, n_frames, c->stream, pad));
+    }
+    if (claim_sc && !split16) {
+        claim_sc->claim_flip ^= 1;
+        c->last_claim = claim_sc;
     }
     static const char *env_merge = SRCNN_DEBUG_ENV("SRCNN_DEBUG_SEAM_MERGE");
     if (defer && !(env_merge && std::atoi(env_merge) == 0)) {
diff --git a/srcnn_cpp_amd/csrc/srcnn_mfma.hip b/srcnn_cpp_amd/csrc/srcnn_mfma.hip
--- a/srcnn_cpp_amd/csrc/srcnn_mfma.hip
+++ b/srcnn_cpp_amd/csrc/srcnn_mfma.hip
@@ -128,6 +128,39 @@
     return mode == MODE_FUSED && !pre;
 }
 
+__device__ __forceinline__ void claim_item(const StripParams &p, int *shared_slot)
+{
+    if (blockIdx.x == 0)
+        for (int i = threadIdx.x; i < p.claim_words; i += NTHREADS) p.claim_zero[i] = 0u;
+    if (threadIdx.x < 64) {
+        const int lane = threadIdx.x;
+        const int x0 = (int)(__builtin_amdgcn_s_getreg((31 << 11) | (0 << 6) | 20) & 7u);
+        const int q0 = (int)(blockIdx.x >> 3);
+        auto take = [&](int slot) {
+            unsigned old = 0u;
+            if (lane == 0) old = atomicAdd(p.claim + slot, 1u);
+            return __builtin_amdgcn_readfirstlane(old) == 0u;
+        };
+        int got = -1;
+        if (q0 < p.claim_items[x0] && take(q0 * 8 + x0)) got = q0 * 8 + x0;
+        for (int k = 0; k < 8 && got < 0; ++k) {
+            const int x = (x0 + k) & 7, len = p.claim_items[x];
+            for (int base = 0; base < len && got < 0; base += 64) {
+                const int q = base + lane;
+                unsigned taken = 1u;
+                if (q < len) taken = __hip_atomic_load(p.claim + (q * 8 + x), __ATOMIC_RELAXED, __HIP_MEMORY_SCOPE_AGENT);
+                unsigned long long free_mask = __ballot(taken == 0u);
+                while (free_mask && got < 0) {
+                    const int slot = (base + (int)__builtin_ctzll(free_mask)) * 8 + x;
+                    free_mask &= free_mask - 1;
+                    if (take(slot)) got = slot;
+                }
+            }
+        }
+        if (lane == 0) *shared_slot = got;
+    }
+}
+
 template <int MODE, bool PRE, int DIAG = 0, bool FIX = false, bool HALO3 = false>
 __device__ __forceinline__ void strip_body(const StripParams &p)
 {
@@ -151,12 +184,48 @@
 
     constexpr int HALO = (MODE == MODE_L12) ? 0 : 2;
 
+    constexpr bool CLAIMS = MODE == MODE_FUSED && !PRE;
+    __shared__ int claimed_slot;
+    const bool claims = CLAIMS && p.claim != nullptr;
+    if constexpr (CLAIMS) {
+        if (claims) claim_item(p, &claimed_slot);
+    }
+
+    const float *wf = p.wfrag + lane;
+    float w1f[2][41], w2f[32], w3f[16];
+    f32x16 b2v = {0};
+    if constexpr (MODE != MODE_L3) {
+#pragma unroll
+        for (int t = 0; t < 2; ++t)
+#pragma unroll
+            for (int s = 0; s < 41; ++s) w1f[t][s] = wf[(t * 41 + s) * 64];
+        constexpr int L2 = (MODE == MODE_L12) ? FRAG_L2U : FRAG_L2, B2 = (MODE == MODE_L12) ? FRAG_B2U : FRAG_B2;
+#pragma unroll
+        for (int q = 0; q < 32; ++q) w2f[q] = wf[(L2 + q) * 64];
+#pragma unroll
+        for (int q = 0; q < 16; ++q) b2v[q] = wf[(B2 + q) * 64];
+    }
+    if constexpr (MODE != MODE_L12) {
+        constexpr int L3 = (MODE == MODE_L3) ? FRAG_L3U : FRAG_L3;
+#pragma unroll
+        for (int q = 0; q < 16; ++q) w3f[q] = wf[(L3 + q) * 64];
+    }
+    const f32x2 ones = {1.0f, 1.0f};
+
     const int W = p.width, H = p.height;
     int bid = blockIdx.x;
     int strip, frame = 0, ys, ye, seam_up = -1, seam_dn = -1;
     if (p.items) {
-        frame = bid / p.items_per_frame;
-        const int *it = p.items + ITEM_INTS * (bid - frame * p.items_per_frame);
+        const int *it;
+        if (claims) {
+            __syncthreads();
+            const int slot = __builtin_amdgcn_readfirstlane(claimed_slot);
+            if (slot < 0) return;
+            it = p.claim_items + CLAIM_LEN_INTS + ITEM_INTS * slot;
+        } else {
+            frame = bid / p.items_per_frame;
+            it = p.items + ITEM_INTS * (bid - frame * p.items_per_frame);
+        }
         strip = it[0];
         ys = it[1];
         ye = it[2];
@@ -192,27 +261,6 @@
     const int f_lo = top_open ? ys : max(ys - HALO, 0);
     const int f_hi = bot_open ? ye : min(ye + HALO, H);
     const int out_lo = top_open ? ys + 2 : ys, out_hi = bot_open ? ye - 2 : ye;
-
-    const float *wf = p.wfrag + lane;
-    float w1f[2][41], w2f[32], w3f[16];
-    f32x16 b2v = {0};
-    if constexpr (MODE != MODE_L3) {
-#pragma unroll
-        for (int t = 0; t < 2; ++t)
-#pragma unroll
-            for (int s = 0; s < 41; ++s) w1f[t][s] = wf[(t * 41 + s) * 64];
-        constexpr int L2 = (MODE == MODE_L12) ? FRAG_L2U : FRAG_L2, B2 = (MODE == MODE_L12) ? FRAG_B2U : FRAG_B2;
-#pragma unroll
-        for (int q = 0; q < 32; ++q) w2f[q] = wf[(L2 + q) * 64];
-#pragma unroll
-        for (int q = 0; q < 16; ++q) b2v[q] = wf[(B2 + q) * 64];
-    }
-    if constexpr (MODE != MODE_L12) {
-        constexpr int L3 = (MODE == MODE_L3) ? FRAG_L3U : FRAG_L3;
-#pragma unroll
-        for (int q = 0; q < 16; ++q) w3f[q] = wf[(L3 + q) * 64];
-    }
-    const f32x2 ones = {1.0f, 1.0f};
 
     const uint8_t *srcf = nullptr;
     int ycol = 0;
diff --git a/srcnn_cpp_amd/csrc/srcnn_plan.cpp b/srcnn_cpp_amd/csrc/srcnn_plan.cpp
--- a/srcnn_cpp_amd/csrc/srcnn_plan.cpp
+++ b/srcnn_cpp_amd/csrc/srcnn_plan.cpp
@@ -34,6 +34,55 @@
 
 double kPairFast = 6.40, kPairSlow = 8.40, kAlone = 3.76, kStartFast = 3.63, kStartSlow = 5.44;
 
+#ifndef SRCNN_XCC_ODD_RATE
+#define SRCNN_XCC_ODD_RATE 0.9906
+#endif
+const double kXccRates[kXccCount] = {1.0, SRCNN_XCC_ODD_RATE, 1.0, SRCNN_XCC_ODD_RATE, 1.0, SRCNN_XCC_ODD_RATE, 1.0, SRCNN_XCC_ODD_RATE};
+
+static std::vector<int> xcc_shares(int n_cu, const double *rates, std::vector<int> *xcc_of)
+{
+    std::vector<int> share((size_t)kXccCount, n_cu / kXccCount);
+    double sum = 0.0;
+    for (int x = 0; x < kXccCount; ++x) sum += rates[x];
+    int total = 0;
+    for (int x = 0; x < kXccCount; ++x) {
+        share[(size_t)x] = std::max(0, (int)std::lround(n_cu * rates[x] / sum));
+        total += share[(size_t)x];
+    }
+    for (int x = 0; total != n_cu; x = (x + 1) % kXccCount) {
+        if (total < n_cu) { ++share[(size_t)x]; ++total; }
+        else if (share[(size_t)x] > 0) { --share[(size_t)x]; --total; }
+    }
+    std::vector<int> left = share;
+    xcc_of->assign((size_t)n_cu, 0);
+    for (int c = 0, x = 0; c < n_cu; ++c, x = (x + 1) % kXccCount) {
+        while (left[(size_t)x] == 0) x = (x + 1) % kXccCount;
+        (*xcc_of)[(size_t)c] = x;
+        --left[(size_t)x];
+    }
+    return share;
+}
+
+static bool rates_usable(int n_cu, const double *rates)
+{
+    if (!rates || n_cu % kXccCount != 0) return false;
+    for (int x = 0; x < kXccCount; ++x)
+        if (!(rates[x] > 0.25 && rates[x] < 4.0)) return false;
+    return true;
+}
+static bool rates_equal(const double *rates)
+{
+    for (int x = 1; x < kXccCount; ++x)
+        if (rates[x] != rates[0]) return false;
+    return true;
+}
+
+static void natural_lists(ItemPlan *plan)
+{
+    for (auto &l : plan->lists) l.clear();
+    for (int i = 0; i < plan->count(); ++i) plan->lists[i % kXccCount].push_back(i);
+}
+
 double cu_finish_estimate(int fast_rows, int slow_rows, double speed)
 {
     static const bool once = [] {
@@ -50,7 +99,7 @@
 }
 
 ItemPlan plan_items_balanced(int n_cu, int n_strips, int row_begin, int row_end, int skew_pct, int extra_top, int extra_bot,
-                             const double *cu_speed = nullptr)
+                             const double *xcc_rates = nullptr, const double *cu_speed = nullptr)
 {
     const ItemPlan none;
     constexpr int kMinRows = 10;
@@ -109,6 +158,19 @@
     std::stable_sort(fi.begin(), fi.end(), [&](int x, int y) { return items[(size_t)x].rows + items[(size_t)x].extra > items[(size_t)y].rows + items[(size_t)y].extra; });
     std::stable_sort(si.begin(), si.end(), [&](int x, int y) { return items[(size_t)x].rows + items[(size_t)x].extra < items[(size_t)y].rows + items[(size_t)y].extra; });
     for (int c = 0; c < n_cu; ++c) items[(size_t)fi[(size_t)c]].cu = items[(size_t)si[(size_t)c]].cu = c;
+    std::vector<double> xcc_speed;
+    std::vector<int> xcc_of;
+    if (rates_usable(n_cu, xcc_rates) && !rates_equal(xcc_rates) && !cu_speed) {
+        const std::vector<int> share = xcc_shares(n_cu, xcc_rates, &xcc_of);
+        double mean = 0.0;
+        for (int x = 0; x < kXccCount; ++x) mean += xcc_rates[x] / kXccCount;
+        xcc_speed.resize((size_t)n_cu);
+        for (int c = 0; c < n_cu; ++c) {
+            const int x = xcc_of[(size_t)c];
+            xcc_speed[(size_t)c] = xcc_rates[x] / mean * (n_cu / kXccCount) / share[(size_t)x];
+        }
+        cu_speed = xcc_speed.data();
+    }
     auto speed = [&](int c) { return cu_speed && cu_speed[c] > 0.5 && cu_speed[c] < 2.0 ? cu_speed[c] : 1.0; };
     auto work = [&](int i) { return items[(size_t)i].rows + items[(size_t)i].extra; };
     auto finish = [&](int c) { return cu_finish_estimate(work(fi[(size_t)c]), work(si[(size_t)c]), speed(c)); };
@@ -284,16 +346,22 @@
     };
     for (int c = 0; c < n_cu; ++c) emit(fi[(size_t)c]);
     for (int c = 0; c < n_cu; ++c) emit(si[(size_t)c]);
+    if (xcc_of.empty()) {
+        natural_lists(&plan);
+    } else {
+        for (int c = 0; c < n_cu; ++c) plan.lists[xcc_of[(size_t)c]].push_back(c);
+        for (int c = 0; c < n_cu; ++c) plan.lists[xcc_of[(size_t)c]].push_back(n_cu + c);
+    }
     return plan;
 }
 
 ItemPlan plan_items_raw(int n_cu, int n_strips, int row_begin, int row_end, int skew_pct, int wgs_per_cu = 2,
-                        bool want_seams = false, int extra_top = 0, int extra_bot = 0)
+                        bool want_seams = false, int extra_top = 0, int extra_bot = 0, const double *xcc_rates = nullptr)
 {
     const ItemPlan none;
     static const char *env_plan = SRCNN_DEBUG_ENV("SRCNN_DEBUG_PLAN");
     if (wgs_per_cu == 2 && want_seams && skew_pct > 0 && !(env_plan && std::atoi(env_plan) == 1)) {
-        const ItemPlan balanced = plan_items_balanced(n_cu, n_strips, row_begin, row_end, skew_pct, extra_top, extra_bot);
+        const ItemPlan balanced = plan_items_balanced(n_cu, n_strips, row_begin, row_end, skew_pct, extra_top, extra_bot, xcc_rates);
         if (balanced.count() > 0) return balanced;
     }
     const int rows = row_end - row_begin;
@@ -356,7 +424,16 @@
     plan.items.reserve(ITEM_INTS * (size_t)slots);
     for (const Item &it : fast) plan.items.insert(plan.items.end(), {it.strip, it.y0, it.y1, it.up, it.dn});
     for (const Item &it : slow) plan.items.insert(plan.items.end(), {it.strip, it.y0, it.y1, it.up, it.dn});
-    return plan.count() == slots ? plan : none;
+    if (plan.count() != slots) return none;
+    if (rates_usable(n_cu, xcc_rates) && *std::max_element(xcc_rates, xcc_rates + kXccCount) >
+                                             1.25 * *std::min_element(xcc_rates, xcc_rates + kXccCount)) {
+        std::vector<int> list_of;
+        xcc_shares(plan.count(), xcc_rates, &list_of);
+        for (int i = 0; i < plan.count(); ++i) plan.lists[list_of[(size_t)i]].push_back(i);
+    } else {
+        natural_lists(&plan);
+    }
+    return plan;
 }
 
 int skew_percent()
@@ -366,9 +443,9 @@
 }
 
 ItemPlan plan_items(int n_cu, int n_strips, int row_begin, int row_end, int skew_pct, int wgs_per_cu, bool want_seams, int extra_top,
-                    int extra_bot)
-{
-    return plan_items_raw(n_cu, n_strips, row_begin, row_end, skew_pct, wgs_per_cu, want_seams, extra_top, extra_bot);
+                    int extra_bot, const double *xcc_rates)
+{
+    return plan_items_raw(n_cu, n_strips, row_begin, row_end, skew_pct, wgs_per_cu, want_seams, extra_top, extra_bot, xcc_rates);
 }
 
 int build_items(srcnn_ctx *c, int n_strips, int row_begin, int row_end, int height, int wgs_per_cu, bool want_seams,
@@ -381,14 +458,15 @@
     const int key[8] = {n_strips, row_begin, row_end, skew_percent(), c->n_cu, wgs_per_cu, want_seams ? 1 : 0, extra_top + 4 * extra_bot};
     srcnn_ctx::ItemTable *victim = &c->item_tables[0];
     for (auto &t : c->item_tables) {
-        if (t.stamp && std::memcmp(key, t.key, sizeof(key)) == 0) {
+        if (t.stamp && std::memcmp(key, t.key, sizeof(key)) == 0 && std::memcmp(c->xcc_rates, t.rates, sizeof(t.rates)) == 0) {
             t.stamp = ++c->item_clock;
             *table = &t;
             return SRCNN_OK;
         }
         if (t.stamp < victim->stamp) victim = &t;
     }
-    const ItemPlan plan = plan_items(c->n_cu, n_strips, row_begin, row_end, key[3], wgs_per_cu, want_seams, extra_top, extra_bot);
+    const ItemPlan plan = plan_items(c->n_cu, n_strips, row_begin, row_end, key[3], wgs_per_cu, want_seams, extra_top, extra_bot,
+                                     c->xcc_rates);
     if (victim->stamp) {
         if (int rc = flush_seams(c)) return rc;
         HIP_TRY(c, hipDeviceSynchronize());
@@ -414,7 +492,27 @@
             }
         }
     }
+    victim->claim_slots = 0;
+    if (plan.count() > 0) {
+        int slots = 0;
+        for (int x = 0; x < kXccCount; ++x) {
+            victim->xcc_len[x] = (int)plan.lists[x].size();
+            slots = std::max(slots, victim->xcc_len[x]);
+        }
+        std::vector<int> tab((size_t)CLAIM_LEN_INTS + (size_t)slots * kXccCount * ITEM_INTS, 0);
+        for (int x = 0; x < kXccCount; ++x) {
+            tab[(size_t)x] = victim->xcc_len[x];
+            for (int q = 0; q < victim->xcc_len[x]; ++q)
+                std::memcpy(&tab[(size_t)CLAIM_LEN_INTS + ((size_t)q * kXccCount + x) * ITEM_INTS],
+                            &plan.items[(size_t)plan.lists[x][(size_t)q] * ITEM_INTS], ITEM_INTS * sizeof(int));
+        }
+        int rc;
+        if ((rc = reserve(c, victim->dev_claim, tab.size() * sizeof(int)))) return rc;
+        HIP_TRY(c, hipMemcpy(victim->dev_claim.p, tab.data(), tab.size() * sizeof(int), hipMemcpyHostToDevice));
+        victim->claim_slots = slots;
+    }
     std::memcpy(victim->key, key, sizeof(key));
+    std::memcpy(victim->rates, c->xcc_rates, sizeof(victim->rates));
     victim->count = plan.count();
     victim->n_seams = plan.n_seams();
     victim->separated = plan.n_seams() > 0 && plan.separated;
@@ -508,6 +606,32 @@
     return SRCNN_OK;
 }
 
+int srcnn_query_plan_xcc(srcnn_ctx *c, int width, int height, int out[8])
+{
+    if (!c || !out || width <= 0 || height <= 0) return SRCNN_ERR_INVALID;
+    for (int x = 0; x < kXccCount; ++x) out[x] = 0;
+    if (!f32_mfma(c) || !c->xcc_claim) return SRCNN_OK;
+    static const char *env_seams = SRCNN_DEBUG_ENV("SRCNN_DEBUG_SEAMS");
+    const int seam_knob = env_seams ? std::atoi(env_seams) : 3;
+    const bool row_seams = (seam_knob & 1) != 0;
+    const int ns_cs = (width + FW - 1) / FW;
+    bool col_seams = (seam_knob & 2) && row_seams && cseam_pays(width);
+    int items_per_cu = 2;
+    auto fits = [&](int n_strips_, int per_cu) { return !plan_items(c->n_cu, n_strips_, 0, height, skew_percent(), per_cu, row_seams).items.empty(); };
+    if (col_seams && !fits(ns_cs, 2)) {
+        if (fits(ns_cs, 1)) items_per_cu = 1;
+        else col_seams = false;
+    }
+    if (!col_seams && row_seams) {
+        const int ns_halo = (width + FW - 5) / (FW - 4);
+        if (!fits(ns_halo, 2) && fits(ns_halo, 1)) items_per_cu = 1;
+    }
+    const Plan pl = make_plan(c, width, height, 1, 2, 2, col_seams ? 0 : -1);
+    const ItemPlan plan = plan_items(c->n_cu, pl.n_strips, 0, height, skew_percent(), items_per_cu, row_seams, 0, 0, c->xcc_rates);
+    for (int x = 0; x < kXccCount; ++x) out[x] = (int)plan.lists[x].size();
+    return SRCNN_OK;
+}
+
 #ifdef SRCNN_TUNING_BUILD
 int srcnn_debug_plan_items(int n_cu, int n_strips, int row_begin, int row_end, int skew_pct, int wgs_per_cu,
                                       int want_seams, int *items, int max_items, int *seams, int max_seams,
@@ -522,6 +646,26 @@
     *n_seams = plan.n_seams();
     return plan.count();
 }
+
+int srcnn_debug_plan_items_xcc(int n_cu, int n_strips, int row_begin, int row_end, int skew_pct, int wgs_per_cu, int want_seams,
+                               const double *rates, int *items, int max_items, int *seams, int max_seams, int *n_seams,
+                               int *lists, int max_list, int *lens)
+{
+    const int extra_top = (wgs_per_cu >> 4) & 15, extra_bot = (wgs_per_cu >> 8) & 15;
+    wgs_per_cu &= 15;
+    if (rates && rates[0] < 0) rates = kXccRates;
+    const ItemPlan plan = plan_items(n_cu, n_strips, row_begin, row_end, skew_pct, wgs_per_cu, want_seams != 0, extra_top, extra_bot, rates);
+    if (plan.count() > max_items || plan.n_seams() > max_seams || !items || !seams || !n_seams || !lists || !lens) return SRCNN_ERR_INVALID;
+    for (int x = 0; x < kXccCount; ++x) {
+        if ((int)plan.lists[x].size() > max_list) return SRCNN_ERR_INVALID;
+        lens[x] = (int)plan.lists[x].size();
+        for (size_t q = 0; q < plan.lists[x].size(); ++q) lists[(size_t)x * max_list + q] = plan.lists[x][q];
+    }
+    if (!plan.items.empty()) std::memcpy(items, plan.items.data(), plan.items.size() * sizeof(int));
+    if (!plan.seams.empty()) std::memcpy(seams, plan.seams.data(), plan.seams.size() * sizeof(int));
+    *n_seams = plan.n_seams();
+    return plan.count();
+}
 #endif
 
 }
```

Measured after the change: 8818 MPix/s (median of 6 runs). Within noise of the previous version (+0.3%).
